# hsp-iit/online-detection

Measured on AMD Instinct MI355X. Metric: FALKON fit+infer samples/sec (N=1e6 D=1024 M=1e4), higher is better.
Workload: dtype f32-accurate K_nM (X Z' as a two-term f16 split on the f16 MFMA, f32 accumulate) stored as 24-bit fixed point (step 2^-24) + f64 solver (preconditioner: K_MM, T and T^-1 in f64; the products of the A factor, which only preconditions, at f32 accuracy on the f16 MFMA)

## Files before the change

include/odx.h:

```cpp
#ifndef ODX_H
#define ODX_H
#include <stdint.h>
#ifdef __cplusplus
extern "C" {
#endif

#define ODX_OK 0
#define ODX_ERR_INVALID (-1)
#define ODX_ERR_HIP (-2)
#define ODX_ERR_UNSUPPORTED (-3)
#define ODX_ERR_WORKSPACE (-4)

typedef void* odx_stream_t;

const char* odx_last_error_string(void);
int odx_version(void);
int odx_device_cus(void);
int odx_set_option(const char* name, int value);
int odx_get_option(const char* name, int* value);
int odx_option_default(const char* name, int* value);
int odx_release_helper_streams(void);
int odx_set_helper_streams(odx_stream_t s0, odx_stream_t s1);
int odx_stream_create_cu_mask(const uint32_t* mask, int words, odx_stream_t* stream);
int odx_stream_destroy(odx_stream_t stream);
// ... 63 lines not shown
int64_t odx_knm_bytes(int64_t n, int64_t M, int fmt);
int odx_gauss_knm_h2_store(const void* PX, int64_t ldpx, const float* metax, const float* xsq, int64_t n,
                           const void* PZ, int64_t ldpz, const float* metaz, const float* zsq, int64_t M, int D,
                           double sigma, int fmt, void* K, int64_t ldk, void* Klo, int64_t ldlo, const double* w,
                           double* ktw, void* workspace, int64_t workspace_bytes, odx_stream_t stream);
int64_t odx_knm_fwd_bwd_q_workspace_bytes(int64_t n, int64_t M, int fmt);
int odx_knm_fwd_bwd_q(const void* K, int64_t ldk, const void* Klo, int64_t ldlo, int fmt, int64_t n, int64_t M,
                      const double* v, const double* w, double* out, void* workspace, int64_t workspace_bytes,
                      odx_stream_t stream);
int64_t odx_knm_fwd_bwd2_q_workspace_bytes(int64_t n, int64_t M, int fmt);
int odx_knm_fwd_bwd2_q(const void* K, int64_t ldk, const void* Klo, int64_t ldlo, int fmt, int64_t n, int64_t M,
                       const double* v, const double* v2, double* out, double* out2, void* workspace,
                       int64_t workspace_bytes, odx_stream_t stream);
int odx_knm_fwd_bwd_q_t(const void* K, int64_t ldk, const void* Klo, int64_t ldlo, int fmt, int64_t n, int64_t M,
                        const double* v, const double* w, double* out, double* t_out, void* workspace,
                        int64_t workspace_bytes, odx_stream_t stream);
int odx_knm_fwd_bwd2_q_t(const void* K, int64_t ldk, const void* Klo, int64_t ldlo, int fmt, int64_t n, int64_t M,
                         const double* v, const double* v2, double* out, double* out2, double* t_out, void* workspace,
                         int64_t workspace_bytes, odx_stream_t stream);
int odx_knm_fwd_bwd_q_cols_t(const void* K, int64_t ldk, const void* Klo, int64_t ldlo, int fmt, int64_t n, int64_t M,
                             const double* v, const double* w, double* out, double* t_out, void* workspace,
                             int64_t workspace_bytes, int64_t Mv, const int32_t* col_of, const int32_t* start,
                             const int32_t* pos, odx_stream_t stream);
int odx_knm_fwd_bwd2_q_cols_t(const void* K, int64_t ldk, const void* Klo, int64_t ldlo, int fmt, int64_t n, int64_t M,
                              const double* v, const double* v2, double* out, double* out2, double* t_out, void* workspace,
                              int64_t workspace_bytes, int64_t Mv, const int32_t* col_of, const int32_t* start,
                              const int32_t* pos, odx_stream_t stream);
int odx_cols_fold_f64(const double* v, int64_t Mv, const int32_t* start, const int32_t* pos, int64_t M, double* out,
                      odx_stream_t stream);
int odx_cols_expand_f64(const double* x, int64_t M, const int32_t* col_of, int64_t Mv, double* out, odx_stream_t stream);
int64_t odx_knm_fwd_bwdn_q_workspace_bytes(int64_t n, int64_t M, int fmt, int nv);
int odx_knm_fwd_bwdn_q(const void* K, int64_t ldk, const void* Klo, int64_t ldlo, int fmt, int64_t n, int64_t M, int nv,
                       const double* V, int64_t ldv, double* out, int64_t ldo, void* workspace, int64_t workspace_bytes,
                       odx_stream_t stream);
int64_t odx_knm_bwdn_q_workspace_bytes(int64_t n, int64_t M, int fmt, int nv);
int odx_knm_bwdn_q(const void* K, int64_t ldk, const void* Klo, int64_t ldlo, int fmt, int64_t n, int64_t M, int nv,
                   const double* W, int64_t ldw, double* out, int64_t ldo, void* workspace, int64_t workspace_bytes,
                   odx_stream_t stream);
int64_t odx_knm_fwdn_q_workspace_bytes(int64_t n, int64_t M, int fmt, int nv);
int odx_knm_fwdn_q(const void* K, int64_t ldk, const void* Klo, int64_t ldlo, int fmt, int64_t n, int64_t M, int nv,
                   const double* V, int64_t ldv, double* T, int64_t ldt, void* workspace, int64_t workspace_bytes,
                   odx_stream_t stream);
int odx_knm_mv(const void* K, int64_t ldk, const void* Klo, int64_t ldlo, int fmt, int64_t n, int64_t M, const double* alpha,
               float* out, int64_t ldo, odx_stream_t stream);
int64_t odx_gauss_ktk_stream_h2_rows(int64_t M, int D);
int64_t odx_gauss_ktk_stream_h2_workspace_bytes(int64_t n, int64_t M, int D);
int odx_gauss_ktk_stream_h2(const void* PX, int64_t ldpx, const float* metax, const float* xsq, int64_t n,
                            const void* PZ, int64_t ldpz, const float* metaz, const float* zsq, int64_t M, int D,
                            double sigma, const double* v, const double* v2, const double* w, double* out, double* out2,
                            void* workspace, int64_t workspace_bytes, odx_stream_t stream);
#define ODX_STREAM_MAX_VECTORS 16
int64_t odx_gauss_ktk_stream_h2n_rows(int64_t M, int D);
int64_t odx_gauss_ktk_stream_h2n_workspace_bytes(int64_t n, int64_t M, int D, int nv);
int odx_gauss_ktk_stream_h2n(const void* PX, int64_t ldpx, const float* metax, const float* xsq, int64_t n,
                             const void* PZ, int64_t ldpz, const float* metaz, const float* zsq, int64_t M, int D,
                             double sigma, int nv, const double* V, int64_t ldv, double* out, int64_t ldo,
                             void* workspace, int64_t workspace_bytes, odx_stream_t stream);

int odx_split_f8(const float* X, int64_t ldx, int64_t n, int D, void* P8, int64_t ldp8, float* meta, float* qsq,
                 odx_stream_t stream);
int odx_gauss_knm_f8_store(const void* PX, int64_t ldpx8, const float* metax, const float* xsq, int64_t n,
                           const void* PZ, int64_t ldpz8, const float* metaz, const float* zsq, int64_t M, int D,
                           double sigma, int fmt, void* K, int64_t ldk, void* Klo, int64_t ldlo, const double* w,
                           double* ktw, void* workspace, int64_t workspace_bytes, odx_stream_t stream);
int odx_gauss_mmv_f8(const void* PX, int64_t ldpx8, const float* metax, const float* xsq, int64_t n,
                     const void* PZ, int64_t ldpz8, const float* metaz, const float* zsq, int64_t max_range, int D,
                     double sigma, const double* V, int64_t ldv, const int32_t* ranges, int T,
                     float* out, int64_t ldo, void* workspace, int64_t workspace_bytes, odx_stream_t stream);

int64_t odx_falkon_precond_workspace_bytes(int64_t M, int D);
int odx_falkon_precond_f64(const float* Z, int64_t ldz, int64_t M, int D, double sigma,
                           double lam, double eps, double* LTi, double* LTit, double* LAi,
                           double* LAit, int64_t ld, int32_t* info,
                           void* workspace, int64_t workspace_bytes, odx_stream_t stream);
int64_t odx_falkon_precond_path_workspace_bytes(int64_t M, int D, int L);
int odx_falkon_precond_path_f64(const float* Z, int64_t ldz, int64_t M, int D, double sigma, const double* lams, int L,
                                double eps, double* LTi, double* LTit, double* LA, int64_t ld, int32_t* info,
                                void* workspace, int64_t workspace_bytes, odx_stream_t stream);
int64_t odx_falkon_precond_batched_workspace_bytes(int64_t Mmax, int D, int B);
int odx_falkon_precond_batched_f64(const float* const* Z, const int64_t* ldz, const int64_t* M, int B,
                                   int64_t Mmax, int D, double sigma, double lam, double eps,
                                   double* out, int64_t ld, int64_t out_stride, int32_t* info,
                                   void* workspace, int64_t workspace_bytes, odx_stream_t stream);

int odx_trmv_f64(const double* Tri, int64_t ld, int64_t M, int uplo, const double* x,
                 double alpha, double beta, const double* z, double* y, odx_stream_t stream);

int odx_trmvn_f64(const double* Tri, int64_t ld, int64_t M, int uplo, int nv, const double* X, int64_t ldx,
                  double alpha, double beta, const double* Z, int64_t ldz, double* Y, int64_t ldy, odx_stream_t stream);

int odx_cg_init(const double* B, double* X, double* R, double* P, double* state, int64_t M,
                odx_stream_t stream);
int odx_cg_step(double* X, double* R, const double* P, const double* AP, double* state,
                double cg_eps, int full_grad, int64_t M, odx_stream_t stream);
int odx_cg_finish(const double* R, double* P, double* state, double cg_eps, double tol,
                  int64_t M, odx_stream_t stream);
int odx_cg_residual(const double* B, const double* AX, const double* AP, const double* state,
                    double* R, int64_t M, odx_stream_t stream);
int odx_cg_scores_axpy_f64(const double* state, const double* t, double* S, int64_t n, odx_stream_t stream);
int odx_cg_scores_store_f32(const double* S, int64_t n, float* out, int64_t ldo, odx_stream_t stream);
int odx_axpby_f64(double a, const double* x, double b, double* y, int64_t M, odx_stream_t stream);

int64_t odx_falkon_cg_workspace_bytes(int64_t n, int64_t M);
int odx_falkon_cg_f64(const float* K, int64_t ldk, int64_t n, int64_t M, const double* LTi, const double* LTit,
                      const double* LAi, const double* LAit, int64_t ldp, const double* b0, double n_total,
                      double lam, int maxiter, int full_gradient_every, double cg_epsilon, double cg_tolerance,
                      double* alpha, void* workspace, int64_t workspace_bytes, odx_stream_t stream);
int64_t odx_falkon_cg_batched_workspace_bytes(int B, const int64_t* n, const int64_t* M);
int odx_falkon_cg_batched_f64(int B, const float* const* K, const int64_t* ldk, const int64_t* n, const int64_t* M,
                              const double* P, int64_t ldp, int64_t p_rows, int64_t p_stride,
                              const double* b0, int64_t vstride, const double* n_total, double lam,
                              int maxiter, int full_gradient_every, double cg_epsilon, double cg_tolerance,
                              double* alpha, void* workspace, int64_t workspace_bytes, odx_stream_t stream);
int64_t odx_falkon_cg_batched_q_workspace_bytes(int B, const int64_t* n, const int64_t* M, int fmt);
int odx_falkon_cg_batched_q_f64(int B, const void* const* Khi, const int64_t* ldk, const void* const* Klo, const int64_t* ldlo,
                                int fmt, const int64_t* n, const int64_t* M, const double* P, int64_t ldp, int64_t p_rows,
                                int64_t p_stride, const double* b0, int64_t vstride, const double* n_total, double lam,
                                int maxiter, int full_gradient_every, double cg_epsilon, double cg_tolerance, double* alpha,
                                void* workspace, int64_t workspace_bytes, odx_stream_t stream);

#define ODX_GEMM_LOWER_ONLY 1
#define ODX_GEMM_A_UPPER 2
#define ODX_GEMM_B_UPPER 4
#define ODX_GEMM_A_LOWER 8
#define ODX_GEMM_B_LOWER 16
#define ODX_GEMM_STORE_T 32
int odx_gemm_nt_f64(const double* A, int64_t lda, const double* B, int64_t ldb, double* C,
                    int64_t ldc, int64_t m, int64_t n, int64_t k, double alpha, double beta,
                    int flags, odx_stream_t stream);
int odx_gemm_nt_f32(const float* A, int64_t lda, const float* B, int64_t ldb, float* C,
                    int64_t ldc, int64_t m, int64_t n, int64_t k, float alpha, float beta,
                    int flags, odx_stream_t stream);
int64_t odx_potrf_workspace_bytes(int64_t M);
int odx_potrf_f64(double* A, int64_t lda, int64_t M, int32_t* info, void* workspace,
                  int64_t workspace_bytes, odx_stream_t stream);
int64_t odx_trtri_workspace_bytes(int64_t M);
int odx_trtri_f64(const double* L, int64_t ldl, int64_t M, double* Li, double* Lit, int64_t ld,
                  void* workspace, int64_t workspace_bytes, odx_stream_t stream);
int odx_convert_f32_f64(const float* src, int64_t lds, double* dst, int64_t ldd, int64_t rows,
                        int64_t cols, odx_stream_t stream);
int odx_convert_f64_f32(const double* src, int64_t lds, float* dst, int64_t ldd, int64_t rows,
                        int64_t cols, odx_stream_t stream);

int64_t odx_rls_gram_workspace_bytes(int64_t nc, int D);
int odx_rls_gram_f64(const float* X, int64_t ldx, int D, const int64_t* idx, int64_t nc,
                     const double* Yt, int64_t ldy, double* G, int64_t ldg, double* XtY,
                     int64_t ldxy, void* workspace, int64_t workspace_bytes, odx_stream_t stream);
int64_t odx_rls_solve_workspace_bytes(int D);
int odx_rls_solve_f64(double* G, int64_t ldg, int D, double lam, const double* XtY, int64_t ldxy,
                      double* W, int64_t ldw, int32_t* info, void* workspace,
                      int64_t workspace_bytes, odx_stream_t stream);

int odx_rls_predict_rows_f64(const float* X, int64_t ldx, int D, const int64_t* idx, int64_t nc,
                             const double* W, int64_t ldw, double* P, int64_t ldp, odx_stream_t stream);
int odx_rls_predict_rows_batched_f64(const float* X, int64_t ldx, int D, const int64_t* idx, const int64_t* seg_start, int C,
                                     int64_t total, const double* W, int64_t ldw, int64_t w_stride, double* P, int64_t ldp,
                                     odx_stream_t stream);

int64_t odx_rls_gram_batched_workspace_bytes(int64_t npad, int D);
int odx_rls_rows_form(const float* X, int64_t ldx, int D);
int odx_rls_xty_batched_f64(const float* X, int64_t ldx, int D, const int64_t* idx_pad, int64_t npad,
                            const int64_t* seg_off, const int64_t* seg_len, int C, const double* Yt, int64_t ldy,
                            double* G, int64_t ldg, int64_t g_stride, double* XtY, int64_t ldxy, int64_t xy_stride,
                            void* workspace, int64_t workspace_bytes, odx_stream_t stream);
int odx_rls_gram_batched_f64(const float* X, int64_t ldx, int D, const int64_t* idx_pad, int64_t npad,
                             const int64_t* seg_off, const int64_t* seg_len, int C,
                             const double* Yt, int64_t ldy, double* G, int64_t ldg, int64_t g_stride,
                             double* XtY, int64_t ldxy, int64_t xy_stride,
                             void* workspace, int64_t workspace_bytes, odx_stream_t stream);
int odx_rls_pad_index(const int64_t* run, int64_t total, const int64_t* seg_off, const int64_t* seg_len, int C, int64_t npad,
                      int64_t* idx_pad, int64_t* gid, int64_t* pos, int64_t* dest, int64_t* lens, odx_stream_t stream);
int odx_rls_gram_raw_batched_f64(const float* X, int64_t ldx, int D, const int64_t* idx_pad, int64_t npad,
                                 const int64_t* seg_off, const int64_t* seg_len, int C, const float* Yraw, int64_t ldyr,
                                 double* G, int64_t ldg, int64_t g_stride, double* O5, int64_t ldo, odx_stream_t stream);
int odx_rls_fold_whitened_f64(const double* O5, int64_t ldo, int D, int C, const double* stats, const double* cnt,
                              double* G, int64_t ldg, int64_t g_stride, double* XtY, int64_t ldxy, int64_t xy_stride,
                              odx_stream_t stream);
int64_t odx_rls_solve_batched_workspace_bytes(int D, int C);
int odx_rls_solve_batched_f64(double* G, int64_t ldg, int64_t g_stride, int D, int C, double lam,
                              const double* XtY, int64_t ldxy, int64_t xy_stride,
                              double* W, int64_t ldw, int64_t w_stride, int32_t* info,
                              void* workspace, int64_t workspace_bytes, odx_stream_t stream);

int odx_roi_align_fwd_f32(const float* feat, int N, int C, int H, int W, const float* rois, int R,
                          float spatial_scale, int PH, int PW, int sampling_ratio, float* out,
                          odx_stream_t stream);
int odx_split_f16_taps3x3(const float* Y, int64_t ldy, int64_t R, int H, int W, int C, void* P, int64_t ldp,
                          float* meta, odx_stream_t stream);
int odx_gemm_h2_f32(const void* PA, int64_t ldpa, const float* metaa, int64_t m, const void* PB, int64_t ldpb,
                    const float* metab, int64_t n, int K, const float* bias, const float* residual, int64_t ldr,
                    int relu, float* out, int64_t ldo, odx_stream_t stream);
int odx_gemm_h2_max_f32(const void* PA, int64_t ldpa, const float* metaa, int64_t m, const void* PB, int64_t ldpb,
                        const float* metab, int64_t n, int K, const float* bias, const float* residual, int64_t ldr,
                        int relu, float* out, int64_t ldo, float* out_meta, odx_stream_t stream);
int odx_split_f16_taps3x3_premax(const float* Y, int64_t ldy, int64_t R, int H, int W, int C, void* P, int64_t ldp,
                                 float* meta, odx_stream_t stream);
int odx_gemm_h2_taps_supported(int64_t m, int64_t n, int C, int64_t ldpy);
int odx_gemm_h2_taps_f32(const void* PY, int64_t ldpy, const float* metay, int64_t R, int H, int W, int C,
                         const void* PB, int64_t ldpb, const float* metab, int64_t n, const float* bias,
                         const float* residual, int64_t ldr, int relu, float* out, int64_t ldo, float* out_meta,
                         void* out_packed, int64_t ldop, float bound_w, float bound_add, const float* residual_meta,
                         odx_stream_t stream);
int odx_upsample_add_rows_f32(float* lat, int64_t ldl, const float* top, int64_t ldt, int B, int H, int W, int Hp, int Wp, int C,
                              float* meta, odx_stream_t stream);
int odx_upsample_add_rows_16(void* lat, int64_t ldl, const void* top, int64_t ldt, int is_bf16, int B, int H, int W, int Hp, int Wp,
                             int C, odx_stream_t stream);
int odx_gemm_h2_chain_f32(const void* PA, int64_t ldpa, const float* metaa, int64_t m, const void* PB, int64_t ldpb,
                          const float* metab, int64_t n, int K, const float* bias, const float* residual, int64_t ldr,
                          int relu, float* out, int64_t ldo, float* out_meta, void* out_packed, int64_t ldop,
                          float bound_w, float bound_add, const float* residual_meta, odx_stream_t stream);
int odx_taps3x3_packed(const void* PY, int64_t ldpy, int64_t R, int H, int W, int C, void* P, int64_t ldp,
                       odx_stream_t stream);
int odx_gemm_b16(const void* A, int64_t lda, int64_t m, const void* B, int64_t ldb, int64_t n, int K, int is_bf16,
                 const float* bias, const void* residual, int64_t ldr, int relu, void* out, int64_t ldo, int out_16,
                 odx_stream_t stream);
int odx_taps3x3_16(const void* Y, int64_t ldy, int64_t R, int H, int W, int C, void* P, int64_t ldp, odx_stream_t stream);
int odx_debug_gemm_h2_mf32(const void* PA, int64_t ldpa, const float* metaa, int64_t m, const void* PB, int64_t ldpb,
                           const float* metab, int64_t n, int K, float* out, int64_t ldo, odx_stream_t stream);
int odx_gemm_b16_taps_supported(int64_t m, int64_t n, int C, int64_t ldy);
int odx_gemm_b16_taps(const void* Y, int64_t ldy, int64_t R, int H, int W, int C, const void* B, int64_t ldb, int64_t n,
                      int is_bf16, const float* bias, const void* residual, int64_t ldr, int relu, void* out, int64_t ldo,
// ... 59 lines not shown
```

online-detection_amd/csrc/api.cpp:

```cpp
#include "odx_common.h"
#include <string.h>

namespace odx {
static thread_local char g_error[512] = "";

void set_error(const char* fmt, ...) {
  va_list ap;
  va_start(ap, fmt);
  vsnprintf(g_error, sizeof(g_error), fmt, ap);
  va_end(ap);
}
}

extern "C" const char* odx_last_error_string(void) { return odx::g_error; }

#include "odx_internal.h"
namespace odx {
struct OptSpec {
  const char* name;
  int def, lo, hi;
};
static const OptSpec g_opt_spec[OPT_COUNT] = {
    {"h2_tile", 0, 0, 256}, {"precond", 0, 0, 2}, {"chain_helpers", -1, -1, 1}, {"rls_force_nt_gram", 0, 0, 1},
    {"rls_force_inverse_solve", 0, 0, 1}};
static int g_opt[OPT_COUNT] = {0, 0, -1, 0, 0};
int lib_option(int which) { return g_opt[which]; }
static int opt_index(const char* name) {
  if (name)
    for (int i = 0; i < OPT_COUNT; ++i)
      if (strcmp(name, g_opt_spec[i].name) == 0) return i;
  return -1;
}
}

extern "C" int odx_set_option(const char* name, int value) {
  const int i = odx::opt_index(name);
  ODX_REQUIRE(i >= 0, "odx_set_option: unknown option '%s'", name ? name : "(null)");
  const odx::OptSpec& sp = odx::g_opt_spec[i];
  ODX_REQUIRE(value >= sp.lo && value <= sp.hi && (i != odx::OPT_H2_TILE || value == 0 || value == 128 || value == 256),
              "odx_set_option: %s = %d out of range", name, value);
  odx::g_opt[i] = value;
  return ODX_OK;
}

extern "C" int odx_get_option(const char* name, int* value) {
  const int i = odx::opt_index(name);
  ODX_REQUIRE(i >= 0 && value, "odx_get_option: unknown option '%s'", name ? name : "(null)");
  *value = odx::g_opt[i];
  return ODX_OK;
}

extern "C" int odx_option_default(const char* name, int* value) {
  const int i = odx::opt_index(name);
  ODX_REQUIRE(i >= 0 && value, "odx_option_default: unknown option '%s'", name ? name : "(null)");
  *value = odx::g_opt_spec[i].def;
  return ODX_OK;
}

extern "C" int odx_version(void) { return 100; }

extern "C" int odx_device_cus(void) {
  int dev = 0;
  if (hipGetDevice(&dev) != hipSuccess) {
    odx::set_error("odx_device_cus: no HIP device");
    return ODX_ERR_HIP;
  }
  int cus = 0;
  if (hipDeviceGetAttribute(&cus, hipDeviceAttributeMultiprocessorCount, dev) != hipSuccess) {
    odx::set_error("odx_device_cus: attribute query failed");
    return ODX_ERR_HIP;
  }
  return cus;
}

extern "C" int odx_stream_create_cu_mask(const uint32_t* mask, int words, odx_stream_t* stream) {
  ODX_REQUIRE(mask && words > 0 && stream, "odx_stream_create_cu_mask: bad argument");
  hipStream_t s = nullptr;
  ODX_CHECK_HIP(hipExtStreamCreateWithCUMask(&s, (uint32_t)words, mask));
  *stream = reinterpret_cast<odx_stream_t>(s);
  return ODX_OK;
}

extern "C" int odx_stream_destroy(odx_stream_t stream) {
  if (stream) ODX_CHECK_HIP(hipStreamDestroy(reinterpret_cast<hipStream_t>(stream)));
  return ODX_OK;
}

namespace odx {
__global__ __launch_bounds__(64) void placement_kernel(int32_t* __restrict__ out, int32_t* __restrict__ counter, int spin) {
  if (threadIdx.x == 0) {
    const unsigned xcc = __builtin_amdgcn_s_getreg((3 << 11) | 20);
    const unsigned hw = __builtin_amdgcn_s_getreg((31 << 11) | 4);
    out[3 * blockIdx.x] = (int32_t)xcc;
    out[3 * blockIdx.x + 1] = (int32_t)hw;
    out[3 * blockIdx.x + 2] = atomicAdd(counter, 1);
    const long long t0 = wall_clock64();
    while (wall_clock64() - t0 < spin) __builtin_amdgcn_s_sleep(8);
  }
}
}

extern "C" int odx_debug_placement(int32_t* out, int blocks, int spin, odx_stream_t stream) {
  ODX_REQUIRE(out && blocks > 0 && spin >= 0, "odx_debug_placement: bad argument");
  hipStream_t s = reinterpret_cast<hipStream_t>(stream);
  ODX_CHECK_HIP(hipMemsetAsync(out, 0, (size_t)(3 * blocks + 1) * sizeof(int32_t), s));
  hipLaunchKernelGGL(odx::placement_kernel, dim3((unsigned)blocks), dim3(64), 0, s, out, out + 3 * blocks, spin);
  ODX_CHECK_LAUNCH("odx_debug_placement");
  return ODX_OK;
// ... 2 lines not shown
```

online-detection_amd/csrc/dense_f64.hip:

```cpp
#include "odx_internal.h"
#include <vector>

namespace odx {

typedef double f64x2 __attribute__((ext_vector_type(2)));
typedef double f64x4v __attribute__((ext_vector_type(4)));

constexpr int DB_NB = POTRF_NB;
constexpr int DB_LD = DB_NB + 1;
constexpr int DB_XLD = 33;
constexpr int DB_NT = 512;
constexpr int DB_PQ = 3072 / DB_NT;

__device__ __forceinline__ double readlane_f64(double v, int src) {
  const long long b = __double_as_longlong(v);
  const unsigned lo = (unsigned)__builtin_amdgcn_readlane((int)(b & 0xffffffffll), src);
  const unsigned hi = (unsigned)__builtin_amdgcn_readlane((int)(b >> 32), src);
  return __longlong_as_double((long long)(((unsigned long long)hi << 32) | lo));
}

__device__ __forceinline__ void chol32_wave(double* s, double* rd, int J, int jb, int32_t* info, int info_base,
                                            int lane) {
  const int l = lane & 31;
  double row[32];
// ... 298 lines not shown
    }
    __builtin_amdgcn_wave_barrier();
#pragma unroll
    for (int q = 0; q < 4; ++q) {
      const int r = wave * 16 + (lane >> 4) + 4 * q;
      T[r * TS_TLD + 32 * J + bc] = y0[q];
      T[r * TS_TLD + 32 * J + 16 + bc] = y1[q];
    }
    __builtin_amdgcn_s_waitcnt(0xC07F);
    __builtin_amdgcn_wave_barrier();
  }
  __syncthreads();
#pragma unroll
  for (int q = 0; q < 16; ++q) {
    const int e = tid + 256 * q, r = e >> 6, c = (e & 63) * 2;
    if (r < rows) *reinterpret_cast<f64x2*>(A21 + (r0 + r) * lda + c) = *reinterpret_cast<const f64x2*>(&T[r * TS_TLD + c]);
  }
}
constexpr int TS_LDS_BYTES = (TS_R * TS_TLD + 10 * 32 * TS_BLD) * (int)sizeof(double);

__global__ __launch_bounds__(256) void transpose_f64_kernel(const double* __restrict__ src, int64_t lds_,
                                                            double* __restrict__ dst, int64_t ldd, int64_t rows,
                                                            int64_t cols, int64_t zstride_src, int64_t zstride_dst) {
  __shared__ double tile[32][33];
  src += (int64_t)blockIdx.z * zstride_src;
  dst += (int64_t)blockIdx.z * zstride_dst;
  const int tx = threadIdx.x & 31, ty = threadIdx.x >> 5;
  const int64_t r0 = (int64_t)blockIdx.y * 32, c0 = (int64_t)blockIdx.x * 32;
#pragma unroll
  for (int q = 0; q < 4; ++q) {
    const int64_t r = r0 + ty + q * 8, c = c0 + tx;
    tile[ty + q * 8][tx] = (r < rows && c < cols) ? src[r * lds_ + c] : 0.0;
  }
  __syncthreads();
#pragma unroll
  for (int q = 0; q < 4; ++q) {
    const int64_t r = c0 + ty + q * 8, c = r0 + tx;
    if (r < cols && c < rows) dst[r * ldd + c] = tile[tx][ty + q * 8];
  }
}

__global__ __launch_bounds__(256) void add_diag_f64_kernel(double* A, int64_t lda, int64_t M, double value,
                                                           int64_t zstride) {
  A += (int64_t)blockIdx.y * zstride;
  const int64_t i = (int64_t)blockIdx.x * 256 + threadIdx.x;
  if (i < M) A[i * lda + i] += value;
}

__global__ __launch_bounds__(256) void fill_f64_kernel(double* A, int64_t lda, int64_t rows, int64_t cols,
                                                       double value) {
  const int64_t c = (int64_t)blockIdx.x * 256 + threadIdx.x;
  const int64_t r = blockIdx.y;
  if (c < cols && r < rows) A[r * lda + c] = value;
}

template <typename S, typename Dt>
__global__ __launch_bounds__(256) void convert_kernel(const S* __restrict__ src, int64_t lds_, Dt* __restrict__ dst,
                                                      int64_t ldd, int64_t rows, int64_t cols) {
  const int64_t c = (int64_t)blockIdx.x * 256 + threadIdx.x;
  const int64_t r = blockIdx.y;
  if (c < cols && r < rows) dst[r * ldd + c] = (Dt)src[r * lds_ + c];
}

__global__ __launch_bounds__(256) void place_diag_inverses_kernel(const double* __restrict__ Dinv, int nb,
                                                                  int64_t M, double* __restrict__ Li,
                                                                  double* __restrict__ Lit, int64_t ld,
                                                                  int64_t zstrideD, int64_t zstrideO) {
  Dinv += (int64_t)blockIdx.z * zstrideD;
  Li += (int64_t)blockIdx.z * zstrideO;
  Lit += (int64_t)blockIdx.z * zstrideO;
  const int b = blockIdx.y;
  const int64_t r0 = (int64_t)b * nb;
  const double* D = Dinv + (int64_t)b * nb * nb;
  for (int e = blockIdx.x * 256 + threadIdx.x; e < nb * nb; e += gridDim.x * 256) {
    const int i = e / nb, j = e % nb;
    if (r0 + i < M && r0 + j < M && j <= i) {
      const double v = D[e];
      Li[(r0 + i) * ld + r0 + j] = v;
      Lit[(r0 + j) * ld + r0 + i] = v;
    }
  }
}

__device__ __forceinline__ void trmv_row(const double* __restrict__ Tri, int64_t ld, int64_t M, int uplo,
                                         const double* __restrict__ x, double alpha, double beta,
                                         const double* __restrict__ z, double* __restrict__ y) {
  const int lane = threadIdx.x & 63;
  int64_t i = (int64_t)blockIdx.x * 4 + (threadIdx.x >> 6);
  if (i >= M) return;
  if (!uplo) i = M - 1 - i;
  const int64_t jlo = uplo ? i : 0, jhi = uplo ? M : i + 1;
  const double* row = Tri + i * ld;
  const int64_t q0 = (jlo + 1) >> 1, q1 = jhi >> 1;
  double s0 = 0.0, s1 = 0.0, s2 = 0.0, s3 = 0.0;
  if (lane == 0) {
    if (jlo & 1) s0 = row[jlo] * x[jlo];
    if (jhi & 1) s1 = row[jhi - 1] * x[jhi - 1];
  }
  int64_t p = q0 + lane;
  for (; p + 192 < q1; p += 256) {
    const f64x2 a0 = *reinterpret_cast<const f64x2*>(row + 2 * p), a1 = *reinterpret_cast<const f64x2*>(row + 2 * (p + 64));
    const f64x2 a2 = *reinterpret_cast<const f64x2*>(row + 2 * (p + 128)), a3 = *reinterpret_cast<const f64x2*>(row + 2 * (p + 192));
    const f64x2 b0 = *reinterpret_cast<const f64x2*>(x + 2 * p), b1 = *reinterpret_cast<const f64x2*>(x + 2 * (p + 64));
    const f64x2 b2 = *reinterpret_cast<const f64x2*>(x + 2 * (p + 128)), b3 = *reinterpret_cast<const f64x2*>(x + 2 * (p + 192));
    s0 = fma(a0[1], b0[1], fma(a0[0], b0[0], s0));
    s1 = fma(a1[1], b1[1], fma(a1[0], b1[0], s1));
    s2 = fma(a2[1], b2[1], fma(a2[0], b2[0], s2));
    s3 = fma(a3[1], b3[1], fma(a3[0], b3[0], s3));
  }
  for (; p < q1; p += 64) {
    const f64x2 a = *reinterpret_cast<const f64x2*>(row + 2 * p);
    const f64x2 b = *reinterpret_cast<const f64x2*>(x + 2 * p);
    s0 = fma(a[1], b[1], fma(a[0], b[0], s0));
  }
  double s = (s0 + s1) + (s2 + s3);
#pragma unroll
  for (int off = 32; off > 0; off >>= 1) s += __shfl_xor(s, off);
  if (lane == 0) {
    double r = alpha * s;
    if (beta != 0.0) r += beta * z[i];
    y[i] = r;
  }
}

__global__ __launch_bounds__(256) void trmv_f64_kernel(const double* __restrict__ Tri, int64_t ld, int64_t M,
                                                       int uplo, const double* __restrict__ x, double alpha,
                                                       double beta, const double* __restrict__ z,
                                                       double* __restrict__ y) {
  trmv_row(Tri, ld, M, uplo, x, alpha, beta, z, y);
}

template <int NV>
__global__ __launch_bounds__(256) void trmvn_f64_kernel(const double* __restrict__ Tri, int64_t ld, int64_t M, int uplo, int nv,
                                                        const double* __restrict__ X, int64_t ldx, double alpha, double beta,
                                                        const double* Z, int64_t ldz, double* Y, int64_t ldy) {
  constexpr int RB = 4, N = RB * NV;
  static_assert((N & (N - 1)) == 0 && N <= 64, "the transposing reduction needs a power-of-two count of sums");
  const int lane = threadIdx.x & 63;
  const int64_t nrb = (M + RB - 1) / RB;
  int64_t rb = (int64_t)blockIdx.x * 4 + (threadIdx.x >> 6);
  if (rb >= nrb) return;
  if (!uplo) rb = nrb - 1 - rb;
  const int64_t i0 = rb * RB, i1 = i0 + RB < M ? i0 + RB : M;
  const int64_t q0 = uplo ? i1 >> 1 : 0, q1 = uplo ? M >> 1 : (i0 + 1) >> 1;
  const double* row[RB];
  const double* xq[NV];
#pragma unroll
  for (int k = 0; k < RB; ++k) row[k] = Tri + (i0 + k < M ? i0 + k : M - 1) * ld;
#pragma unroll
  for (int q = 0; q < NV; ++q) xq[q] = X + (int64_t)(q < nv ? q : nv - 1) * ldx;
  double acc[RB][NV];
#pragma unroll
  for (int k = 0; k < RB; ++k)
#pragma unroll
    for (int q = 0; q < NV; ++q) acc[k][q] = 0.0;
  if (lane < 16) {
    const int64_t j = lane < 8 ? 2 * q1 + lane : 2 * q0 - 1 - (lane - 8);
#pragma unroll
    for (int k = 0; k < RB; ++k) {
      const int64_t i = i0 + k;
      const int64_t jlo = uplo ? i : 0, jhi = uplo ? M : i + 1;
      if (i < M && j >= jlo && j < jhi) {
        const double a = row[k][j];
#pragma unroll
        for (int q = 0; q < NV; ++q) acc[k][q] = a * xq[q][j];
      }
    }
  }
  for (int64_t p = q0 + lane; p < q1; p += 64) {
    f64x2 a[RB];
#pragma unroll
    for (int k = 0; k < RB; ++k) a[k] = *reinterpret_cast<const f64x2*>(row[k] + 2 * p);
#pragma unroll
    for (int q = 0; q < NV; ++q) {
      const f64x2 b = *reinterpret_cast<const f64x2*>(xq[q] + 2 * p);
#pragma unroll
      for (int k = 0; k < RB; ++k) acc[k][q] = fma(a[k][1], b[1], fma(a[k][0], b[0], acc[k][q]));
    }
  }
  double* s = &acc[0][0];
  int off = 32;
#pragma unroll
  for (int half = N / 2; half >= 1; half >>= 1, off >>= 1) {
    const bool up = (lane & off) != 0;
#pragma unroll
    for (int i = 0; i < half; ++i) {
      const double give = up ? s[i] : s[half + i], keep = up ? s[half + i] : s[i];
      s[i] = keep + __shfl_xor(give, off);
    }
  }
#pragma unroll
  for (; off > 0; off >>= 1) s[0] += __shfl_xor(s[0], off);
  int idx = 0, bit = 32;
#pragma unroll
  for (int half = N / 2; half >= 1; half >>= 1, bit >>= 1) idx += (lane & bit) ? half : 0;
  if ((lane & (64 / N - 1)) == 0 || N == 64) {
    const int k = idx / NV, q = idx % NV;
    const int64_t i = i0 + k;
    if (i < M && q < nv) {
      double r = alpha * s[0];
      if (beta != 0.0) r += beta * Z[(int64_t)q * ldz + i];
      Y[(int64_t)q * ldy + i] = r;
    }
  }
}

__global__ __launch_bounds__(256) void trmv_batched_kernel(const double* __restrict__ Tri, int64_t ld, int64_t tri_stride,
                                                           int uplo, VecBatch vb, const double* __restrict__ x,
                                                           int64_t xstride, int scaled, double beta,
                                                           const double* __restrict__ z, int64_t zstride,
                                                           double* __restrict__ y, int64_t ystride) {
  const int b = blockIdx.y;
// ... 177 lines not shown
      double* D = Dinv + (k0 / NB) * NB * NB;
      hipLaunchKernelGGL((potrf_diag_kernel<NB, false>), dim3((unsigned)Z), dim3(DB_NT), 0, stream, A + k0 * lda + k0, lda,
                         jb, D, info, (int)k0, zb.strideA, zb.strideD);
      ODX_CHECK_LAUNCH("potrf_diag");
      const int64_t m = M - k0 - jb;
      if (m <= 0) break;
      double* A21 = A + (k0 + jb) * lda + k0;
      hipLaunchKernelGGL(trsm128_kernel, dim3((unsigned)ceil_div(m, TS_R), (unsigned)Z), dim3(256), TS_LDS_BYTES, stream,
                         A21, lda, m, A + k0 * lda + k0, D + NB * NB - 4096, zb.strideA, zb.strideD);
      ODX_CHECK_LAUNCH("trsm128");
      const int64_t pc = (K0 + kbo) - (k0 + jb);
      if (pc > 0) {
        GemmParams<double> u;
        u.A = A21; u.lda = lda; u.B = A21; u.ldb = lda; u.C = A + (k0 + jb) * lda + (k0 + jb); u.ldc = lda;
        u.m = m; u.n = pc; u.k = jb; u.alpha = -1.0; u.beta = 1.0; u.flags = ODX_GEMM_LOWER_ONLY;
        zgemm(u);
        ODX_PROPAGATE(launch_gemm_f64(u, stream));
      }
    }
    const int64_t mt = M - K0 - kbo;
    if (mt > 0) {
      double* P = A + (K0 + kbo) * lda + K0;
      const int64_t nw = mt < POTRF_NBO ? mt : POTRF_NBO;
      if (pending) {
        ODX_CHECK_HIP(hipStreamWaitEvent(stream, look->join, 0));
        pending = false;
      }
      const int64_t mr = mt - nw;
      double minus1[ODX_MAX_ZBATCH];
      for (int z = 0; z < Z; ++z) minus1[z] = -1.0;
      uint32_t* Pk = pk ? pk + ((K0 / POTRF_NBO) & 1) * pk_buf : nullptr;
      if (Pk) {
        ODX_PROPAGATE(split_f64(P, lda, zb.strideA, mt, kbo, pk_scale, Pk, POTRF_NBO, pk_z, Z, stream));
        ODX_PROPAGATE(gemm_h2_f64(Pk, POTRF_NBO, pk_z, pk_scale, Pk, POTRF_NBO, pk_z, pk_scale, A + (K0 + kbo) * (lda + 1), lda,
                                  zb.strideA, mt, nw, kbo, minus1, 1.0, ODX_GEMM_LOWER_ONLY, Z, stream));
      } else {
        GemmParams<double> u;
        u.A = P; u.lda = lda; u.B = P; u.ldb = lda; u.C = A + (K0 + kbo) * (lda + 1); u.ldc = lda;
        u.m = mt; u.n = nw; u.k = kbo; u.alpha = -1.0; u.beta = 1.0; u.flags = ODX_GEMM_LOWER_ONLY;
        zgemm(u);
        ODX_PROPAGATE(launch_gemm_f64(u, stream));
      }
      if (mr > 0) {
        ODX_CHECK_HIP(hipEventRecord(look->fork, stream));
        ODX_CHECK_HIP(hipStreamWaitEvent(look->stream, look->fork, 0));
        if (Pk) {
          ODX_PROPAGATE(gemm_h2_f64(Pk + nw * POTRF_NBO, POTRF_NBO, pk_z, pk_scale, Pk + nw * POTRF_NBO, POTRF_NBO, pk_z, pk_scale,
                                    A + (K0 + kbo + nw) * (lda + 1), lda, zb.strideA, mr, mr, kbo, minus1, 1.0, ODX_GEMM_LOWER_ONLY, Z,
                                    look->stream));
        } else {
          double* P2 = P + nw * lda;
          GemmParams<double> r;
          r.A = P2; r.lda = lda; r.B = P2; r.ldb = lda; r.C = A + (K0 + kbo + nw) * (lda + 1); r.ldc = lda;
          r.m = mr; r.n = mr; r.k = kbo; r.alpha = -1.0; r.beta = 1.0; r.flags = ODX_GEMM_LOWER_ONLY;
          zgemm(r);
          ODX_PROPAGATE(launch_gemm_f64(r, look->stream));
        }
        ODX_CHECK_HIP(hipEventRecord(look->join, look->stream));
        pending = true;
      }
    }
  }
  if (pending) ODX_CHECK_HIP(hipStreamWaitEvent(stream, look->join, 0));
  hipLaunchKernelGGL(trtri_diag_kernel, dim3((unsigned)ceil_div(M, NB), (unsigned)Z), dim3(DB_NT), 0, stream, A, lda, M,
                     Dinv, zb.strideA, zb.strideD);
  ODX_CHECK_LAUNCH("trtri_diag");
  return ODX_OK;
}

int trmv_batched_f64(const double* Tri, int64_t ld, int64_t tri_stride, int uplo, const VecBatch& vb, const double* x,
                     int64_t xstride, bool scaled, double beta, const double* z, int64_t zstride, double* y,
                     int64_t ystride, hipStream_t stream) {
  int mm = 0;
  for (int b = 0; b < vb.B; ++b) mm = vb.M[b] > mm ? vb.M[b] : mm;
  if (mm <= 0) return ODX_OK;
  hipLaunchKernelGGL(trmv_batched_kernel, dim3((unsigned)ceil_div(mm, 4), (unsigned)vb.B), dim3(256), 0, stream, Tri, ld,
                     tri_stride, uplo, vb, x, xstride, scaled ? 1 : 0, beta, z, zstride, y, ystride);
  ODX_CHECK_LAUNCH("trmv_batched_f64");
  return ODX_OK;
}

int trtri_from_diag_f64(const double* L, int64_t ldl, int64_t M, const double* Dinv, double* Li, double* Lit,
                        int64_t ld, double* WT, hipStream_t stream, const ZBatch& zb, uint32_t* pk, int64_t pk_cap, int64_t pk_z,
                        double bound_l, double bound_inv) {
  constexpr int NB = POTRF_NB;
  ODX_REQUIRE(ld % 2 == 0 && ldl % 2 == 0, "trtri_f64: leading dimensions must be even");
  const int Z = zb.count;
  ODX_REQUIRE(Z >= 1 && Z <= ODX_MAX_ZBATCH && zb.strideA % 2 == 0 && zb.strideO % 2 == 0 && zb.strideW % 2 == 0,
              "trtri_f64: class batch of 1..%d matrices, even strides", ODX_MAX_ZBATCH);
  const int nblk = (int)ceil_div(M, NB);
  hipLaunchKernelGGL(place_diag_inverses_kernel, dim3(16, (unsigned)nblk, (unsigned)Z), dim3(256), 0, stream, Dinv, NB, M,
                     Li, Lit, ld, zb.strideD, zb.strideO);
  ODX_CHECK_LAUNCH("place_diag_inverses");
  for (int64_t s = NB; s < M; s *= 2) {
    const int nb = (int)ceil_div(M, 2 * s);
    const int nbe = (int)ceil_div(M - s, 2 * s);
    const int64_t m2l = M - s - (int64_t)(nbe - 1) * 2 * s;
    const int64_t szr = (int64_t)(nbe - 1) * s * s + (m2l < s ? m2l : s) * s;
    if (pk != nullptr && s >= 512 && 2 * szr + 2 * (int64_t)nbe * s * s <= pk_cap) {
      const float sl = split_scale_for(bound_l), si = split_scale_for(bound_inv), sw = split_scale_for(bound_l * bound_inv);
      uint32_t *pL21 = pk, *pX11 = pL21 + szr, *pX22 = pX11 + (int64_t)nbe * s * s, *pWT = pX22 + szr;
      double one[ODX_MAX_ZBATCH], mone[ODX_MAX_ZBATCH];
      for (int z = 0; z < Z; ++z) { one[z] = 1.0; mone[z] = -1.0; }
      SplitBlocksArgs k1;
      k1.X = L + s * ldl; k1.ldx = ldl; k1.bsx = 2 * s * (ldl + 1); k1.zsx = zb.strideA;
      k1.P = pL21; k1.ldp = s; k1.bsp = s * s; k1.zsp = pk_z; k1.rows = s; k1.cols = s;
      k1.rg_total = M; k1.rg_off = s; k1.rg_step = 2 * s; k1.rows_ragged = 1; k1.nb = nbe; k1.Z = Z; k1.scale = sl;
      ODX_PROPAGATE(split_f64_blocks(k1, stream));
      SplitBlocksArgs k2;
      k2.X = Lit; k2.ldx = ld; k2.bsx = 2 * s * (ld + 1); k2.zsx = zb.strideO;
      k2.P = pX11; k2.ldp = s; k2.bsp = s * s; k2.zsp = pk_z; k2.rows = s; k2.cols = s; k2.nb = nbe; k2.Z = Z; k2.scale = si;
      ODX_PROPAGATE(split_f64_blocks(k2, stream));
      H2F64Args a1;
      a1.PA = pL21; a1.ldpa = s; a1.zsa = pk_z; a1.bsa = s * s; a1.sa = sl;
      a1.PB = pX11; a1.ldpb = s; a1.zsb = pk_z; a1.bsb = s * s; a1.sb = si;
      a1.C = WT; a1.ldc = s; a1.zsc = zb.strideW; a1.bsc = s * s;
      a1.m = s; a1.n = s; a1.k = s; a1.rg_total = M; a1.rg_off = s; a1.rg_step = 2 * s;
      a1.flags = ODX_GEMM_B_UPPER | ODX_GEMM_STORE_T; a1.zcount = Z; a1.nb = nbe; a1.beta = 0.0;
      for (int z = 0; z < Z; ++z) a1.alpha[z] = one[z];
      ODX_PROPAGATE(gemm_h2_f64_ex(a1, stream));
      SplitBlocksArgs k3;
      k3.X = Li + s * (ld + 1); k3.ldx = ld; k3.bsx = 2 * s * (ld + 1); k3.zsx = zb.strideO;
      k3.P = pX22; k3.ldp = s; k3.bsp = s * s; k3.zsp = pk_z; k3.rows = s; k3.cols = s;
      k3.rg_total = M; k3.rg_off = s; k3.rg_step = 2 * s; k3.rows_ragged = 1; k3.cols_ragged = 1; k3.nb = nbe; k3.Z = Z; k3.scale = si;
      ODX_PROPAGATE(split_f64_blocks(k3, stream));
      SplitBlocksArgs k4;
      k4.X = WT; k4.ldx = s; k4.bsx = s * s; k4.zsx = zb.strideW;
      k4.P = pWT; k4.ldp = s; k4.bsp = s * s; k4.zsp = pk_z; k4.rows = s; k4.cols = s;
      k4.rg_total = M; k4.rg_off = s; k4.rg_step = 2 * s; k4.cols_ragged = 1; k4.nb = nbe; k4.Z = Z; k4.scale = sw;
      ODX_PROPAGATE(split_f64_blocks(k4, stream));
      H2F64Args a2;
      a2.PA = pX22; a2.ldpa = s; a2.zsa = pk_z; a2.bsa = s * s; a2.sa = si;
      a2.PB = pWT; a2.ldpb = s; a2.zsb = pk_z; a2.bsb = s * s; a2.sb = sw;
      a2.C = Li + s * ld; a2.ldc = ld; a2.zsc = zb.strideO; a2.bsc = 2 * s * (ld + 1);
      a2.C2 = Lit + s; a2.ldc2 = ld; a2.zsc2 = zb.strideO; a2.bsc2 = 2 * s * (ld + 1);
      a2.m = s; a2.n = s; a2.k = s; a2.rg_total = M; a2.rg_off = s; a2.rg_step = 2 * s; a2.k_is_m = 1;
      a2.flags = ODX_GEMM_A_LOWER; a2.zcount = Z; a2.nb = nbe; a2.beta = 0.0;
      for (int z = 0; z < Z; ++z) a2.alpha[z] = mone[z];
      ODX_PROPAGATE(gemm_h2_f64_ex(a2, stream));
      continue;
    }
    GemmParams<double> g1;
    g1.A = L + s * ldl; g1.lda = ldl;
    g1.B = Lit; g1.ldb = ld;
    g1.C = WT; g1.ldc = s;
    g1.m = s; g1.n = s; g1.k = s; g1.alpha = 1.0; g1.beta = 0.0;
    g1.flags = ODX_GEMM_B_UPPER | ODX_GEMM_STORE_T;
    g1.batches = nb;
    g1.strideA = 2 * s * (ldl + 1); g1.strideB = 2 * s * (ld + 1); g1.strideC = s * s;
    g1.ragged_total = M; g1.ragged_off = s; g1.ragged_step = 2 * s;
    g1.zbatches = Z; g1.zstrideA = zb.strideA; g1.zstrideB = zb.strideO; g1.zstrideC = zb.strideW;
    ODX_PROPAGATE(launch_gemm_f64(g1, stream));
    GemmParams<double> g2;
    g2.A = Li + s * (ld + 1); g2.lda = ld;
    g2.B = WT; g2.ldb = s;
    g2.C = Li + s * ld; g2.ldc = ld;
    g2.C2 = Lit + s; g2.ldc2 = ld;
    g2.m = s; g2.n = s; g2.k = s; g2.alpha = -1.0; g2.beta = 0.0;
    g2.flags = ODX_GEMM_A_LOWER;
    g2.batches = nb;
    g2.strideA = 2 * s * (ld + 1); g2.strideB = s * s; g2.strideC = 2 * s * (ld + 1); g2.strideC2 = 2 * s * (ld + 1);
    g2.ragged_total = M; g2.ragged_off = s; g2.ragged_step = 2 * s; g2.ragged_k_is_m = 1;
    g2.zbatches = Z; g2.zstrideA = zb.strideO; g2.zstrideB = zb.strideW; g2.zstrideC = zb.strideO; g2.zstrideC2 = zb.strideO;
    ODX_PROPAGATE(launch_gemm_f64(g2, stream));
  }
  return ODX_OK;
}

}

using namespace odx;

extern "C" int odx_trmv_f64(const double* Tri, int64_t ld, int64_t M, int uplo, const double* x, double alpha,
                            double beta, const double* z, double* y, odx_stream_t stream) {
  if (M <= 0) return ODX_OK;
  ODX_REQUIRE(Tri && x && y && (beta == 0.0 || z), "odx_trmv_f64: null pointer");
  ODX_REQUIRE(ld % 2 == 0 && ld >= M && aligned16(Tri) && aligned16(x), "odx_trmv_f64: Tri/x must be 16-byte aligned, ld even, ld >= M");
  ODX_REQUIRE(x != y, "odx_trmv_f64: x and y must not alias");
  hipLaunchKernelGGL(trmv_f64_kernel, dim3((unsigned)ceil_div(M, 4)), dim3(256), 0, as_stream(stream), Tri, ld, M,
                     uplo, x, alpha, beta, z, y);
  ODX_CHECK_LAUNCH("odx_trmv_f64");
  return ODX_OK;
}

extern "C" int odx_trmvn_f64(const double* Tri, int64_t ld, int64_t M, int uplo, int nv, const double* X, int64_t ldx, double alpha,
                             double beta, const double* Z, int64_t ldz, double* Y, int64_t ldy, odx_stream_t stream) {
  ODX_REQUIRE(nv >= 1 && nv <= 8, "odx_trmvn_f64: 1 .. 8 vectors per call (got %d)", nv);
  if (M <= 0) return ODX_OK;
  ODX_REQUIRE(Tri && X && Y && (beta == 0.0 || Z), "odx_trmvn_f64: null pointer");
  ODX_REQUIRE(ld % 2 == 0 && ld >= M && aligned16(Tri) && aligned16(X) && ldx % 2 == 0,
              "odx_trmvn_f64: Tri/X must be 16-byte aligned, ld and ldx even, ld >= M");
  ODX_REQUIRE(nv == 1 || (ldx >= M && ldy >= M && (beta == 0.0 || ldz >= M)), "odx_trmvn_f64: rows of X, Z and Y must be M apart or more");
  ODX_REQUIRE(X != Y, "odx_trmvn_f64: X and Y must not alias");
  const dim3 grid((unsigned)ceil_div(ceil_div(M, (int64_t)4), (int64_t)4));
#define ODX_TRMVN(NV_)                                                                                                            \
  hipLaunchKernelGGL(trmvn_f64_kernel<NV_>, grid, dim3(256), 0, as_stream(stream), Tri, ld, M, uplo, nv, X, ldx, alpha, beta, Z, ldz, \
                     Y, ldy)
  if (nv <= 2) ODX_TRMVN(2);
  else if (nv <= 4) ODX_TRMVN(4);
  else ODX_TRMVN(8);
#undef ODX_TRMVN
  ODX_CHECK_LAUNCH("odx_trmvn_f64");
  return ODX_OK;
}

extern "C" int odx_convert_f32_f64(const float* src, int64_t lds_, double* dst, int64_t ldd, int64_t rows,
                                   int64_t cols, odx_stream_t stream) {
  if (rows <= 0 || cols <= 0) return ODX_OK;
  ODX_REQUIRE(src && dst, "odx_convert_f32_f64: null pointer");
  for (int64_t r0 = 0; r0 < rows; r0 += 65535) {
    const int64_t nr = rows - r0 < 65535 ? rows - r0 : 65535;
    hipLaunchKernelGGL((convert_kernel<float, double>), dim3((unsigned)ceil_div(cols, 256), (unsigned)nr), dim3(256),
                       0, as_stream(stream), src + r0 * lds_, lds_, dst + r0 * ldd, ldd, nr, cols);
  }
  ODX_CHECK_LAUNCH("odx_convert_f32_f64");
  return ODX_OK;
}

extern "C" int odx_convert_f64_f32(const double* src, int64_t lds_, float* dst, int64_t ldd, int64_t rows,
                                   int64_t cols, odx_stream_t stream) {
  if (rows <= 0 || cols <= 0) return ODX_OK;
  ODX_REQUIRE(src && dst, "odx_convert_f64_f32: null pointer");
  for (int64_t r0 = 0; r0 < rows; r0 += 65535) {
    const int64_t nr = rows - r0 < 65535 ? rows - r0 : 65535;
    hipLaunchKernelGGL((convert_kernel<double, float>), dim3((unsigned)ceil_div(cols, 256), (unsigned)nr), dim3(256),
                       0, as_stream(stream), src + r0 * lds_, lds_, dst + r0 * ldd, ldd, nr, cols);
  }
  ODX_CHECK_LAUNCH("odx_convert_f64_f32");
  return ODX_OK;
}

extern "C" int64_t odx_potrf_workspace_bytes(int64_t M) {
  if (M <= 0) return 0;
  return ceil_div(M, POTRF_NB) * POTRF_NB * POTRF_NB * (int64_t)sizeof(double);
}

extern "C" int odx_potrf_f64(double* A, int64_t lda, int64_t M, int32_t* info, void* workspace,
                             int64_t workspace_bytes, odx_stream_t stream) {
  if (M <= 0) return ODX_OK;
  ODX_REQUIRE(A && info && workspace, "odx_potrf_f64: null pointer");
  if (workspace_bytes < odx_potrf_workspace_bytes(M)) {
    set_error("odx_potrf_f64: workspace too small");
    return ODX_ERR_WORKSPACE;
  }
  ODX_CHECK_HIP(hipMemsetAsync(info, 0, sizeof(int32_t), as_stream(stream)));
  const int rc = potrf_f64(A, lda, M, static_cast<double*>(workspace), info, as_stream(stream));
  return rc;
}

extern "C" int64_t odx_trtri_workspace_bytes(int64_t M) {
  if (M <= 0) return 0;
  return odx_potrf_workspace_bytes(M) + M * M * (int64_t)sizeof(double);
}

extern "C" int odx_trtri_f64(const double* L, int64_t ldl, int64_t M, double* Li, double* Lit, int64_t ld,
                             void* workspace, int64_t workspace_bytes, odx_stream_t stream) {
  if (M <= 0) return ODX_OK;
  ODX_REQUIRE(L && Li && Lit && workspace, "odx_trtri_f64: null pointer");
  ODX_REQUIRE(ld >= M && ldl >= M && aligned16(L) && aligned16(Li) && aligned16(Lit), "odx_trtri_f64: bad ld / alignment");
  if (workspace_bytes < odx_trtri_workspace_bytes(M)) {
    set_error("odx_trtri_f64: workspace too small");
    return ODX_ERR_WORKSPACE;
  }
  hipStream_t s = as_stream(stream);
  double* Dinv = static_cast<double*>(workspace);
  double* WT = Dinv + ceil_div(M, POTRF_NB) * POTRF_NB * POTRF_NB;
  hipLaunchKernelGGL(trtri_diag_kernel, dim3((unsigned)ceil_div(M, POTRF_NB)), dim3(DB_NT), 0, s, L, ldl, M, Dinv,
                     (int64_t)0, (int64_t)0);
  ODX_CHECK_LAUNCH("trtri_diag");
  ODX_PROPAGATE(fill_f64(Li, ld, M, M, 0.0, s));
  ODX_PROPAGATE(fill_f64(Lit, ld, M, M, 0.0, s));
  return trtri_from_diag_f64(L, ldl, M, Dinv, Li, Lit, ld, WT, s);
}

static int64_t precond_ld(int64_t M) { return round_up(M, 2); }
static int64_t precond_ldz(int D) { const int64_t l = round_up(D, 2); return l % 128 == 0 ? l + 64 : l; }

extern "C" int64_t odx_falkon_precond_workspace_bytes(int64_t M, int D) {
  if (M <= 0 || D <= 0) return 0;
  const int64_t ld = precond_ld(M), ldzd = precond_ldz(D);
  int64_t dbl = M * ldzd + round_up(M, 2) + 4 * M * ld + 2 * ceil_div(M, POTRF_NB) * POTRF_NB * POTRF_NB + precond_split_doubles(M);
  return dbl * (int64_t)sizeof(double);
}

static int falkon_precond_f64_impl(const float* Z, int64_t ldz, int64_t M, int D, double sigma, const double* lams, int L,
                                   double eps, double* LTi, double* LTit, double* const* LAi, double* const* LAit, int64_t ld,
                                   int32_t* info, void* workspace, int64_t workspace_bytes, odx_stream_t stream);

extern "C" int odx_falkon_precond_f64(const float* Z, int64_t ldz, int64_t M, int D, double sigma, double lam,
                                      double eps, double* LTi, double* LTit, double* LAi, double* LAit, int64_t ld,
                                      int32_t* info, void* workspace, int64_t workspace_bytes, odx_stream_t stream) {
  ODX_REQUIRE(LAi && LAit, "odx_falkon_precond_f64: null pointer");
  const int rc = falkon_precond_f64_impl(Z, ldz, M, D, sigma, &lam, 1, eps, LTi, LTit, &LAi, &LAit, ld, info, workspace, workspace_bytes, stream);
  return rc;
}

extern "C" int64_t odx_falkon_precond_path_workspace_bytes(int64_t M, int D, int L) {
  if (M <= 0 || D <= 0 || L <= 0) return 0;
  return round_up(odx_falkon_precond_workspace_bytes(M, D), 16) + (L > 1 ? M * precond_ld(M) * (int64_t)sizeof(double) : 0);
}

extern "C" int odx_falkon_precond_path_f64(const float* Z, int64_t ldz, int64_t M, int D, double sigma, const double* lams, int L,
                                           double eps, double* LTi, double* LTit, double* LA, int64_t ld, int32_t* info,
                                           void* workspace, int64_t workspace_bytes, odx_stream_t stream) {
  ODX_REQUIRE(lams && LA && L >= 1 && L <= ODX_MAX_ZBATCH, "odx_falkon_precond_path_f64: 1 <= L <= %d lambdas, non-null lams / LA",
              ODX_MAX_ZBATCH);
  ODX_REQUIRE(M > 0 && ld >= M, "odx_falkon_precond_path_f64: bad sizes");
  double* lai[ODX_MAX_ZBATCH];
  double* lait[ODX_MAX_ZBATCH];
  for (int l = 0; l < L; ++l) {
    lai[l] = LA + (int64_t)(2 * l) * M * ld;
    lait[l] = lai[l] + M * ld;
  }
  return falkon_precond_f64_impl(Z, ldz, M, D, sigma, lams, L, eps, LTi, LTit, lai, lait, ld, info, workspace, workspace_bytes, stream);
}

static int falkon_precond_f64_impl(const float* Z, int64_t ldz, int64_t M, int D, double sigma, const double* lams, int L,
                                   double eps, double* LTi, double* LTit, double* const* LAi, double* const* LAit, int64_t ld,
                                   int32_t* info, void* workspace, int64_t workspace_bytes, odx_stream_t stream) {
  ODX_REQUIRE(M > 0 && D > 0 && sigma > 0, "odx_falkon_precond_f64: bad sizes");
  ODX_REQUIRE(Z && LTi && LTit && info && workspace, "odx_falkon_precond_f64: null pointer");
  ODX_REQUIRE(ld % 2 == 0 && ld >= M && aligned16(LTi) && aligned16(LTit), "odx_falkon_precond_f64: outputs must be 16-byte aligned with even ld >= M");
  for (int l = 0; l < L; ++l)
    ODX_REQUIRE(LAi[l] && LAit[l] && aligned16(LAi[l]) && aligned16(LAit[l]),
                "odx_falkon_precond_f64: outputs must be 16-byte aligned with even ld >= M");
  ODX_REQUIRE(aligned16(workspace), "odx_falkon_precond_f64: workspace must be 16-byte aligned");
  if (workspace_bytes < odx_falkon_precond_path_workspace_bytes(M, D, L)) {
    set_error("odx_falkon_precond_f64: workspace too small");
    return ODX_ERR_WORKSPACE;
  }
  hipStream_t s = as_stream(stream);
  SideStream* side = nullptr;
  ODX_PROPAGATE(side_stream(&side, 0, s, M));
  hipStream_t s2 = side->stream;
  const int64_t wld = precond_ld(M), ldzd = precond_ldz(D);
  const int64_t dsz = ceil_div(M, POTRF_NB) * POTRF_NB * POTRF_NB;
  double* Zd = static_cast<double*>(workspace);
  double* zsq = Zd + M * ldzd;
  double* W0 = zsq + round_up(M, 2);
  double* W1 = W0 + M * wld;
  double* W2 = W1 + M * wld;
  double* W3 = W2 + M * wld;
  double* DinvT = W3 + M * wld;
  double* DinvA = DinvT + dsz;
  const bool split = precond_split(M);
  const int64_t ldpt = h2_f64_packed_ld(M);
  uint32_t* Tk = reinterpret_cast<uint32_t*>(DinvA + dsz);
  uint32_t* Pk = Tk + precond_pack_units(M);
  double* WA = L > 1 ? static_cast<double*>(workspace) + round_up(odx_falkon_precond_workspace_bytes(M, D), 16) / (int64_t)sizeof(double) : W2;

  ODX_CHECK_HIP(hipMemsetAsync(info, 0, (size_t)L * sizeof(int32_t), s));
  ODX_CHECK_HIP(hipMemsetAsync(Zd, 0, (size_t)(M * ldzd) * sizeof(double), s));
  ODX_PROPAGATE(odx_convert_f32_f64(Z, ldz, Zd, ldzd, M, D, stream));
  ODX_CHECK_HIP(hipMemsetAsync(W0, 0, (size_t)(M * wld) * sizeof(double), s));
  ODX_PROPAGATE(gauss_kmm_f64(Zd, ldzd, M, D, sigma, eps * (double)M, W0, wld, zsq, s));
  ODX_PROPAGATE(potrf_f64(W0, wld, M, DinvT, info, s));
  for (int l = 1; l < L; ++l)
    ODX_CHECK_HIP(hipMemcpyAsync(info + l, info, sizeof(int32_t), hipMemcpyDeviceToDevice, s));
  ODX_CHECK_HIP(hipEventRecord(side->fork, s));
  ODX_CHECK_HIP(hipStreamWaitEvent(s2, side->fork, 0));
  ODX_PROPAGATE(fill_f64(LTi, ld, M, M, 0.0, s2));
  ODX_PROPAGATE(fill_f64(LTit, ld, M, M, 0.0, s2));
  ODX_PROPAGATE(trtri_from_diag_f64(W0, wld, M, DinvT, LTi, LTit, ld, W3, s2));
  ODX_CHECK_HIP(hipEventRecord(side->join, s2));
  ODX_CHECK_HIP(hipMemsetAsync(W1, 0, (size_t)(M * wld) * sizeof(double), s));
  ODX_PROPAGATE(transpose_f64(W0, wld, W1, wld, M, M, s));
  ODX_CHECK_HIP(hipMemsetAsync(W2, 0, (size_t)(M * wld) * sizeof(double), s));
  if (split) {
    const float st = split_scale_for(sqrt(1.0 + eps * 65536.0));
    const double a1 = 1.0 / (double)M;
    ODX_PROPAGATE(split_f64(W1, wld, 0, M, M, st, Tk, ldpt, 0, 1, s));
    ODX_PROPAGATE(gemm_h2_f64(Tk, ldpt, 0, st, Tk, ldpt, 0, st, W2, wld, 0, M, M, M, &a1, 0.0,
                              ODX_GEMM_LOWER_ONLY | ODX_GEMM_A_UPPER | ODX_GEMM_B_UPPER, 1, s));
  } else {
    GemmParams<double> g;
    g.A = W1; g.lda = wld; g.B = W1; g.ldb = wld; g.C = W2; g.ldc = wld;
    g.m = M; g.n = M; g.k = M; g.alpha = 1.0 / (double)M; g.beta = 0.0;
    g.flags = ODX_GEMM_LOWER_ONLY | ODX_GEMM_A_UPPER | ODX_GEMM_B_UPPER;
    ODX_PROPAGATE(launch_gemm_f64(g, s));
  }
  for (int l = 0; l < L; ++l) {
    const double lam = lams[l];
    if (WA != W2) ODX_CHECK_HIP(hipMemcpyAsync(WA, W2, (size_t)(M * wld) * sizeof(double), hipMemcpyDeviceToDevice, s));
    ODX_PROPAGATE(add_diag_f64(WA, wld, M, lam, s));
    if (split) ODX_PROPAGATE(potrf_f64(WA, wld, M, DinvA, info + l, s, ZBatch(), Pk, M * POTRF_NBO, 0, split_scale_for(sqrt(1.0 + eps + lam))));
    else ODX_PROPAGATE(potrf_f64(WA, wld, M, DinvA, info + l, s));
    if (l == 0) ODX_CHECK_HIP(hipStreamWaitEvent(s, side->join, 0));
    ODX_PROPAGATE(fill_f64(LAi[l], ld, M, M, 0.0, s));
    ODX_PROPAGATE(fill_f64(LAit[l], ld, M, M, 0.0, s));
    if (split && eps + lam > 0.0)
      ODX_PROPAGATE(trtri_from_diag_f64(WA, wld, M, DinvA, LAi[l], LAit[l], ld, W1, s, ZBatch(), Tk, precond_pack_units(M), 0,
                                        sqrt(1.0 + eps + lam), 1.0 / sqrt(eps + lam)));
    else
      ODX_PROPAGATE(trtri_from_diag_f64(WA, wld, M, DinvA, LAi[l], LAit[l], ld, W1, s));
  }
  return ODX_OK;
}

extern "C" int64_t odx_falkon_precond_batched_workspace_bytes(int64_t Mmax, int D, int B) {
  if (Mmax <= 0 || D <= 0 || B <= 0) return 0;
  const int64_t ld = precond_ld(Mmax), ldzd = precond_ldz(D);
  const int64_t per = Mmax * ldzd + round_up(Mmax, 2) + 4 * Mmax * ld + 2 * ceil_div(Mmax, POTRF_NB) * POTRF_NB * POTRF_NB +
                      precond_split_doubles(Mmax);
  return per * B * (int64_t)sizeof(double);
}

static int falkon_precond_batched_f64_impl(const float* const* Z, const int64_t* ldz, const int64_t* M, int B,
                                           int64_t Mmax, int D, double sigma, double lam, double eps, double* out,
                                           int64_t ld, int64_t out_stride, int32_t* info, void* workspace,
                                           int64_t workspace_bytes, odx_stream_t stream);

extern "C" int odx_falkon_precond_batched_f64(const float* const* Z, const int64_t* ldz, const int64_t* M, int B,
                                              int64_t Mmax, int D, double sigma, double lam, double eps, double* out,
                                              int64_t ld, int64_t out_stride, int32_t* info, void* workspace,
                                              int64_t workspace_bytes, odx_stream_t stream) {
  const int rc = falkon_precond_batched_f64_impl(Z, ldz, M, B, Mmax, D, sigma, lam, eps, out, ld, out_stride, info, workspace, workspace_bytes, stream);
  return rc;
}

static int falkon_precond_batched_f64_impl(const float* const* Z, const int64_t* ldz, const int64_t* M, int B,
                                           int64_t Mmax, int D, double sigma, double lam, double eps, double* out,
                                           int64_t ld, int64_t out_stride, int32_t* info, void* workspace,
                                           int64_t workspace_bytes, odx_stream_t stream) {
  ODX_REQUIRE(B >= 1 && B <= ODX_MAX_ZBATCH, "odx_falkon_precond_batched_f64: 1 <= B <= %d classes per call", ODX_MAX_ZBATCH);
  ODX_REQUIRE(Z && ldz && M && out && info && workspace && Mmax > 0 && D > 0 && sigma > 0,
              "odx_falkon_precond_batched_f64: null pointer or bad size");
  ODX_REQUIRE(ld % 2 == 0 && ld >= Mmax && aligned16(out) && out_stride % 2 == 0 && out_stride >= 4 * Mmax * ld,
              "odx_falkon_precond_batched_f64: out must be 16-byte aligned, ld even >= Mmax, out_stride >= 4 Mmax ld");
  ODX_REQUIRE(aligned16(workspace), "odx_falkon_precond_batched_f64: workspace must be 16-byte aligned");
  for (int b = 0; b < B; ++b)
    ODX_REQUIRE(Z[b] && M[b] > 0 && M[b] <= Mmax, "odx_falkon_precond_batched_f64: class %d: need 0 < M <= Mmax", b);
  if (workspace_bytes < odx_falkon_precond_batched_workspace_bytes(Mmax, D, B)) {
    set_error("odx_falkon_precond_batched_f64: workspace too small");
    return ODX_ERR_WORKSPACE;
  }
  hipStream_t s = as_stream(stream);
  SideStream* side = nullptr;
  ODX_PROPAGATE(side_stream(&side, 0, s, Mmax));
  hipStream_t s2 = side->stream;
  const int64_t wld = precond_ld(Mmax), ldzd = precond_ldz(D);
  const int64_t dsz = ceil_div(Mmax, POTRF_NB) * POTRF_NB * POTRF_NB;
  const int64_t zper = Mmax * ldzd + round_up(Mmax, 2), wsz = Mmax * wld;
  double* Zd0 = static_cast<double*>(workspace);
  double* W0 = Zd0 + (int64_t)B * zper;
  double* W1 = W0 + (int64_t)B * wsz;
  double* W2 = W1 + (int64_t)B * wsz;
  double* W3 = W2 + (int64_t)B * wsz;
  double* DinvT = W3 + (int64_t)B * wsz;
  double* DinvA = DinvT + (int64_t)B * dsz;
  double* LTi = out, *LTit = out + Mmax * ld, *LAi = out + 2 * Mmax * ld, *LAit = out + 3 * Mmax * ld;
  const bool split = precond_split(Mmax);
  const int64_t ldpt = h2_f64_packed_ld(Mmax);
  uint32_t* Tk = reinterpret_cast<uint32_t*>(DinvA + (int64_t)B * dsz);
  uint32_t* Pk = Tk + (int64_t)B * precond_pack_units(Mmax);

  ODX_CHECK_HIP(hipMemsetAsync(info, 0, (size_t)B * sizeof(int32_t), s));
  ODX_CHECK_HIP(hipMemsetAsync(Zd0, 0, (size_t)((int64_t)B * zper) * sizeof(double), s));
  ODX_CHECK_HIP(hipMemsetAsync(W0, 0, (size_t)(3 * (int64_t)B * wsz) * sizeof(double), s));
  if (out_stride == 4 * Mmax * ld) {
    ODX_CHECK_HIP(hipMemsetAsync(out, 0, (size_t)((int64_t)B * out_stride) * sizeof(double), s));
  } else {
    for (int b = 0; b < B; ++b)
      ODX_CHECK_HIP(hipMemsetAsync(out + (int64_t)b * out_stride, 0, (size_t)(4 * Mmax * ld) * sizeof(double), s));
  }
  VecBatch kb;
  kb.B = B;
  for (int b = 0; b < B; ++b) {
    ODX_PROPAGATE(odx_convert_f32_f64(Z[b], ldz[b], Zd0 + (int64_t)b * zper, ldzd, M[b], D, stream));
    kb.M[b] = (int)M[b];
    kb.scale[b] = eps * (double)M[b];
  }
  ODX_PROPAGATE(gauss_kmm_f64_batched(Zd0, ldzd, zper, Mmax * ldzd, kb, D, sigma, W0, wld, wsz, s));
  for (int b = 0; b < B; ++b)
    if (M[b] < Mmax) ODX_PROPAGATE(add_diag_f64(W0 + (int64_t)b * wsz + M[b] * (wld + 1), wld, Mmax - M[b], 1.0, s));
  ZBatch zt;
  zt.count = B; zt.strideA = wsz; zt.strideD = dsz; zt.strideO = out_stride; zt.strideW = wsz;
  ODX_PROPAGATE(potrf_f64(W0, wld, Mmax, DinvT, info, s, zt));
  ODX_CHECK_HIP(hipEventRecord(side->fork, s));
  ODX_CHECK_HIP(hipStreamWaitEvent(s2, side->fork, 0));
  ODX_PROPAGATE(trtri_from_diag_f64(W0, wld, Mmax, DinvT, LTi, LTit, ld, W3, s2, zt));
  ODX_CHECK_HIP(hipEventRecord(side->join, s2));
  ODX_PROPAGATE(transpose_f64(W0, wld, W1, wld, Mmax, Mmax, s, B, wsz, wsz));
  if (split) {
    const float st = split_scale_for(sqrt(1.0 + eps * 65536.0)), sa = split_scale_for(sqrt(1.0 + eps + lam));
    double a1[ODX_MAX_ZBATCH];
    for (int b = 0; b < B; ++b) a1[b] = 1.0 / (double)M[b];
    ODX_PROPAGATE(split_f64(W1, wld, wsz, Mmax, Mmax, st, Tk, ldpt, precond_pack_units(Mmax), B, s));
    ODX_PROPAGATE(gemm_h2_f64(Tk, ldpt, precond_pack_units(Mmax), st, Tk, ldpt, precond_pack_units(Mmax), st, W2, wld, wsz, Mmax, Mmax, Mmax, a1, 0.0,
                              ODX_GEMM_LOWER_ONLY | ODX_GEMM_A_UPPER | ODX_GEMM_B_UPPER, B, s));
    ODX_PROPAGATE(add_diag_f64(W2, wld, Mmax, lam, s, B, wsz));
    ODX_PROPAGATE(potrf_f64(W2, wld, Mmax, DinvA, info, s, zt, Pk, (int64_t)B * Mmax * POTRF_NBO, Mmax * POTRF_NBO, sa));
  } else {
    GemmParams<double> g;
    g.A = W1; g.lda = wld; g.B = W1; g.ldb = wld; g.C = W2; g.ldc = wld;
    g.m = Mmax; g.n = Mmax; g.k = Mmax; g.beta = 0.0;
    g.flags = ODX_GEMM_LOWER_ONLY | ODX_GEMM_A_UPPER | ODX_GEMM_B_UPPER;
    g.zbatches = B; g.zstrideA = wsz; g.zstrideB = wsz; g.zstrideC = wsz;
    g.zalpha_on = 1;
    for (int b = 0; b < B; ++b) g.zalpha[b] = 1.0 / (double)M[b];
    ODX_PROPAGATE(launch_gemm_f64(g, s));
    ODX_PROPAGATE(add_diag_f64(W2, wld, Mmax, lam, s, B, wsz));
    ODX_PROPAGATE(potrf_f64(W2, wld, Mmax, DinvA, info, s, zt));
  }
  ODX_CHECK_HIP(hipStreamWaitEvent(s, side->join, 0));
  if (split && eps + lam > 0.0)
    return trtri_from_diag_f64(W2, wld, Mmax, DinvA, LAi, LAit, ld, W1, s, zt, Tk, precond_pack_units(Mmax), precond_pack_units(Mmax),
                               sqrt(1.0 + eps + lam), 1.0 / sqrt(eps + lam));
  return trtri_from_diag_f64(W2, wld, Mmax, DinvA, LAi, LAit, ld, W1, s, zt);
}

extern "C" int odx_set_side_stream_cu_mask(const uint32_t* mask, int words) {
  ODX_REQUIRE(words >= 0 && words <= 64 && (words == 0 || mask != nullptr), "odx_set_side_stream_cu_mask: bad argument");
  g_side_mask.assign(mask, mask + words);
  return ODX_OK;
}

extern "C" int odx_set_helper_streams(odx_stream_t s0, odx_stream_t s1) {
  g_given_helper[0] = reinterpret_cast<hipStream_t>(s0);
  g_given_helper[1] = reinterpret_cast<hipStream_t>(s1);
  return ODX_OK;
}

extern "C" int odx_release_helper_streams(void) {
  return odx::release_side_streams(false);
}
```

online-detection_amd/csrc/odx_internal.h:

```cpp
#pragma once
#include "odx_common.h"

namespace odx {
enum LibOpt {
  OPT_H2_TILE = 0,
  OPT_PRECOND,
  OPT_CHAIN_HELPERS,
  OPT_RLS_FORCE_NT_GRAM,
  OPT_RLS_FORCE_INVERSE_SOLVE,
  OPT_COUNT
};
int lib_option(int which);


constexpr int ODX_MAX_ZBATCH = 32;

template <typename T>
struct GemmParams {
  const T* A = nullptr; int64_t lda = 0;
  const T* B = nullptr; int64_t ldb = 0;
  T* C = nullptr; int64_t ldc = 0;
  T* C2 = nullptr; int64_t ldc2 = 0;
  int64_t m = 0, n = 0, k = 0;
  T alpha = T(1), beta = T(0);
  int flags = 0;
  int batches = 1;
  int64_t strideA = 0, strideB = 0, strideC = 0, strideC2 = 0;
  int64_t ragged_total = 0, ragged_off = 0, ragged_step = 0;
  int ragged_k_is_m = 0;
  int vec_epilogue = 0;
  int zbatches = 1;
  int64_t zstrideA = 0, zstrideB = 0, zstrideC = 0, zstrideC2 = 0;
  int zalpha_on = 0;
  T zalpha[ODX_MAX_ZBATCH] = {};
  int zk_on = 0;
  int64_t zkoff[ODX_MAX_ZBATCH] = {};
  int64_t zklen[ODX_MAX_ZBATCH] = {};
};

int launch_gemm_f64(const GemmParams<double>& p, hipStream_t stream);
int launch_gemm_f32(const GemmParams<float>& p, hipStream_t stream);

constexpr int POTRF_NB = 128;
struct ZBatch {
  int count = 1;
  int64_t strideA = 0;
  int64_t strideD = 0;
  int64_t strideO = 0;
  int64_t strideW = 0;
};
int potrf_f64(double* A, int64_t lda, int64_t M, double* Dinv , int32_t* info ,
              hipStream_t stream, const ZBatch& zb = ZBatch(), uint32_t* pk = nullptr, int64_t pk_buf = 0, int64_t pk_z = 0,
              float pk_scale = 1.f);
int trtri_from_diag_f64(const double* L, int64_t ldl, int64_t M, const double* Dinv, double* Li, double* Lit,
                        int64_t ld, double* WT, hipStream_t stream, const ZBatch& zb = ZBatch(), uint32_t* pk = nullptr,
                        int64_t pk_cap = 0, int64_t pk_z = 0, double bound_l = 1.0, double bound_inv = 1.0);
int transpose_f64(const double* src, int64_t lds, double* dst, int64_t ldd, int64_t rows, int64_t cols,
                  hipStream_t stream, int zcount = 1, int64_t zstride_src = 0, int64_t zstride_dst = 0);
int add_diag_f64(double* A, int64_t lda, int64_t M, double value, hipStream_t stream, int zcount = 1, int64_t zstride = 0);
int fill_f64(double* A, int64_t lda, int64_t rows, int64_t cols, double value, hipStream_t stream);

int slab_reduce_f64(const double* slab, int64_t slab_ld, int nslab, int64_t M, double* out, hipStream_t stream);
int slab_reduce2_f64(const double* slab, int64_t slab_ld, int nslab, int64_t M, double* out, double* out2, hipStream_t stream);

int slab_reduce_cols_f64(const double* slab, int64_t slab_ld, int nslab, int nv, int64_t M, int64_t Mv, const int* col_of, double* out,
                         double* out2, hipStream_t stream);

int slab_reduce_batched_f64(int B, const int64_t* M, const int* nslab, const double* slab, int64_t slab_ld, int64_t slab_stride,
                            double* out, int64_t ostride, hipStream_t stream);
int64_t knm_passq_batched_workspace_bytes(int B, const int64_t* n, const int64_t* M, int fmt);
int knm_passq_batched(int B, const void* const* Khi, const int64_t* ldk, const void* const* Klo, const int64_t* ldlo, int fmt,
                      const int64_t* n, const int64_t* M, const double* v, int64_t vstride, double* out, int64_t ostride,
                      void* workspace, int64_t workspace_bytes, hipStream_t stream);

int pass_cus();
int check_q_block(const char* who, const void* K, int64_t ldk, const void* Klo, int64_t ldlo, int fmt, int64_t M);

bool knm_pass_batch_cfg(int B, const int64_t* M, int* nt, int* ch, int* r);
int64_t knm_pass_batched_workspace_bytes(int B, const int64_t* n, const int64_t* M);
int knm_pass_batched(int B, const float* const* K, const int64_t* ldk, const int64_t* n, const int64_t* M, const double* v,
                     int64_t vstride, double* out, int64_t ostride, void* workspace, int64_t workspace_bytes,
                     hipStream_t stream);

struct VecBatch {
  int B = 1;
  int M[ODX_MAX_ZBATCH] = {};
  double scale[ODX_MAX_ZBATCH] = {};
};
int trmv_batched_f64(const double* Tri, int64_t ld, int64_t tri_stride, int uplo, const VecBatch& vb, const double* x,
                     int64_t xstride, bool scaled, double beta, const double* z, int64_t zstride, double* y,
                     int64_t ystride, hipStream_t stream);
int cg_init_batched(const VecBatch& vb, const double* Bv, double* X, double* R, double* P, double* state, int64_t vstride,
                    hipStream_t stream);
int cg_step_batched(const VecBatch& vb, double* X, double* R, const double* P, const double* AP, double* state,
                    double cg_eps, int full_grad, int64_t vstride, hipStream_t stream);
int cg_finish_batched(const VecBatch& vb, const double* R, double* P, double* state, double cg_eps, double tol,
                      int64_t vstride, hipStream_t stream);
int cg_full_residual_batched(const VecBatch& vb, const double* Bv, const double* AX, double* R, int64_t vstride,
                             hipStream_t stream);

int64_t h2_f64_packed_ld(int64_t cols);
int split_f64(const double* X, int64_t ldx, int64_t zsx, int64_t rows, int64_t cols, float scale, uint32_t* P, int64_t ldp,
              int64_t zsp, int z, hipStream_t stream);
struct SplitBlocksArgs {
  const double* X = nullptr; int64_t ldx = 0, bsx = 0, zsx = 0;
  uint32_t* P = nullptr; int64_t ldp = 0, bsp = 0, zsp = 0;
  int64_t rows = 0, cols = 0;
  int64_t rg_total = 0, rg_off = 0, rg_step = 0;
  int rows_ragged = 0, cols_ragged = 0, nb = 1, Z = 1;
  float scale = 1.f;
};
int split_f64_blocks(const SplitBlocksArgs& a, hipStream_t stream);
struct H2F64Args {
  const uint32_t* PA = nullptr; int64_t ldpa = 0, zsa = 0, bsa = 0; float sa = 1.f;
  const uint32_t* PB = nullptr; int64_t ldpb = 0, zsb = 0, bsb = 0; float sb = 1.f;
  double* C = nullptr; int64_t ldc = 0, zsc = 0, bsc = 0;
  double* C2 = nullptr; int64_t ldc2 = 0, zsc2 = 0, bsc2 = 0;
  int64_t m = 0, n = 0, k = 0;
  int64_t rg_total = 0, rg_off = 0, rg_step = 0;
  int k_is_m = 0, flags = 0, zcount = 1, nb = 1;
  double beta = 0.0;
  double alpha[ODX_MAX_ZBATCH] = {};
};
int gemm_h2_f64_ex(const H2F64Args& a, hipStream_t stream);
int gemm_h2_f64(const uint32_t* PA, int64_t ldpa, int64_t zsa, float sa, const uint32_t* PB, int64_t ldpb, int64_t zsb, float sb,
                double* C, int64_t ldc, int64_t zsc, int64_t m, int64_t n, int64_t k, const double* alpha, double beta, int flags,
                int zcount, hipStream_t stream);

int gauss_kmm_f64(const double* Zd, int64_t ldz, int64_t M, int D, double sigma, double diag_add, double* Kmm,
                  int64_t ldk, double* zsq , hipStream_t stream);

int gauss_kmm_f64_batched(const double* Zd, int64_t ldz, int64_t z_stride, int64_t zsq_off, const VecBatch& vb, int D,
                          double sigma, double* Kmm, int64_t ldk, int64_t k_stride, hipStream_t stream);

}
```

online-detection_amd/odx/backend.py:

```python
import ctypes
import os

import torch

from . import hip
from .knm_path import PathOps, _p


class Features:
    __slots__ = ("X", "sq", "n", "D", "ld", "P", "meta", "own_pack", "P8", "meta8", "sq8", "zero_row", "cmap")

    def __init__(self, X, sq, D, P=None, meta=None):
        self.X, self.sq, self.n, self.D, self.ld = X, sq, X.shape[0], D, X.stride(0) if X.shape[0] else X.shape[1]
        self.P, self.meta = P, meta
        self.zero_row = False
        self.own_pack = P is None
        self.P8 = self.meta8 = self.sq8 = None
        self.cmap = None


class Rows16:
    __slots__ = ("buf", "n", "K", "zero_row")

    def __init__(self, buf, K, zero_row=False):
        self.buf, self.n, self.K = buf, buf.shape[0], K
        self.zero_row = zero_row

    @property
    def dense(self):
        return self.buf[:, :self.K]


class PackedRows:
    __slots__ = ("X", "n", "D", "P", "meta", "zero_row")

    def __init__(self, X, n, D, P, meta, zero_row=False):
        self.X, self.n, self.D, self.P, self.meta, self.zero_row = X, n, D, P, meta, zero_row


class Precond:
    __slots__ = ("LTi", "LTit", "LAi", "LAit", "M", "ld", "info", "block_rows")


class Knm:
    __slots__ = ("K", "n", "M", "ld", "fmt", "lo", "cmap", "Mv")

    def __init__(self):
        self.fmt, self.lo, self.cmap, self.Mv = "f32", None, None, None

    def dense(self):
        if self.fmt == "f32":
            return self.K[:, :self.M]
        if self.fmt == "u24":
            q = ((self.K[:, :self.M].to(torch.int32) & 0xFFFF) << 8) | self.lo[:, :self.M].to(torch.int32)
            return q.to(torch.float32) * (2.0 ** -24)
        return ((self.K[:, :self.M].to(torch.int32) & 0xFFFF) << 16).view(torch.float32)

    def rows(self, lo, hi):
        sub = Knm()
        sub.n, sub.M, sub.ld, sub.fmt = hi - lo, self.M, self.ld, self.fmt
        sub.K = self.K[lo:hi]
        sub.lo = self.lo[lo:hi] if self.lo is not None else None
        sub.cmap, sub.Mv = self.cmap, self.Mv
        return sub


class KnmStream:
    __slots__ = ("F", "Zf", "sigma", "n", "M", "ring", "K", "fmt", "lo")

    def __init__(self, F, Zf, sigma, ring=None):
        self.F, self.Zf, self.sigma, self.n, self.M, self.ring = F, Zf, float(sigma), F.n, Zf.n, ring
        self.K, self.fmt, self.lo = F.P, "stream", None


class HipBackend(PathOps):
    name = "hip-gfx950"
    shared_mmv_min = 2

    def __init__(self, device=None):
        self.lib = hip.require_gpu()
        self.device = torch.device("cuda", torch.cuda.current_device()) if device is None else torch.device(device)
        self._ws = {}
        self._meta_pools = {}
        self._capture_meta_pool = None
        from . import options as _options
        opts = _options.load()
        self.gauss = opts.gauss
        self.knm_storage = opts.knm_storage
        _options.apply()
        self.helper_streams = []
        try:
            from . import streams as _streams
            own = _streams.of_default(3, self.device)
            if len(own) >= 3:
                self.helper_streams = own[1:3]
                hip.check(self.lib.odx_set_helper_streams(ctypes.c_void_p(own[1].cuda_stream), ctypes.c_void_p(own[2].cuda_stream)),
                          "odx_set_helper_streams")
        except hip.OdxError:
            raise
        except Exception:
            pass

    def _stream(self):
        return ctypes.c_void_p(torch.cuda.current_stream(self.device).cuda_stream)

    def _workspace(self, key, nbytes):
        nbytes = max(int(nbytes), 16)
        if torch.cuda.is_current_stream_capturing():
            return torch.empty(nbytes, dtype=torch.uint8, device=self.device)
        cur = torch.cuda.current_stream(self.device)
        if cur != torch.cuda.default_stream(self.device):
            key = (key, cur.cuda_stream)
        buf = self._ws.get(key)
        if buf is None or buf.numel() < nbytes:
            buf = None
            self._ws.pop(key, None)
            buf = torch.empty(nbytes, dtype=torch.uint8, device=self.device)
            self._ws[key] = buf
        return buf

    def release_workspaces(self):
        self._ws.clear()
        self.release_helper_streams()

# ... 68 lines not shown

    def _meta_slot(self):
        if torch.cuda.is_current_stream_capturing():
            pool = self._capture_meta_pool
            if pool is None or pool[1] + 2 > pool[0].numel():
                pool = self._capture_meta_pool = [torch.zeros(1024, dtype=torch.float32, device=self.device), 0]
            at = pool[1]
            pool[1] = at + 4
            return pool[0][at:at + 2]
        cur = torch.cuda.current_stream(self.device)
        key = cur.cuda_stream
        pool = self._meta_pools.get(key)
        if pool is None or pool[1] + 2 > pool[0].numel():
            pool = self._meta_pools[key] = [torch.zeros(8192, dtype=torch.float32, device=self.device), 0]
        at = pool[1]
        pool[1] = at + 4
        return pool[0][at:at + 2]

    def reset_capture_pools(self):
        self._capture_meta_pool = None

    def rows(self, F, idx):
        idx = torch.as_tensor(idx, dtype=torch.int64, device=self.device).reshape(-1)
        ld = (F.D + 3) // 4 * 4
        buf = torch.zeros((idx.numel(), ld), dtype=torch.float32, device=self.device)
        buf[:, :F.D] = F.X.index_select(0, idx)
        P = F.P.index_select(0, idx) if F.P is not None else None
        Z = Features(buf[:, :F.D], F.sq.index_select(0, idx), F.D, P, F.meta if P is not None else None)
        if F.P8 is not None:
            Z.P8, Z.meta8, Z.sq8 = F.P8.index_select(0, idx), F.meta8, F.sq8.index_select(0, idx)
        return Z

    def pack8(self, F):
        if F.P8 is None:
            ldp8 = (F.D + 127) // 128 * 128
            F.P8 = torch.empty((F.n, ldp8), dtype=torch.uint8, device=self.device)
            F.meta8 = torch.zeros(2, dtype=torch.float32, device=self.device)
            F.sq8 = torch.empty(F.n, dtype=torch.float32, device=self.device)
            hip.check(self.lib.odx_split_f8(_p(F.X), F.ld, F.n, F.D, _p(F.P8), ldp8, _p(F.meta8), _p(F.sq8), self._stream()),
                      "odx_split_f8")
        return F

    def pack(self, F, zero_row=False):
        if F.P is not None and zero_row and not F.zero_row:
            if not F.own_pack:
                raise ValueError("pack(zero_row=True): the packed rows were gathered from another matrix and have no zero row behind them")
            F.P = None
        if F.P is None:
            ldp = (F.D + 63) // 64 * 64
            if zero_row:
                buf = torch.empty((F.n + 1, ldp), dtype=torch.int32, device=self.device)
                buf[F.n].zero_()
                F.P = buf[:F.n]
                F.zero_row = True
            else:
                F.P = torch.empty((F.n, ldp), dtype=torch.int32, device=self.device)
            if F.meta is not None and F.n:
                hip.check(self.lib.odx_split_f16_premax(_p(F.X), F.ld, F.n, F.D, _p(F.P), ldp, _p(F.meta), self._stream()),
                          "odx_split_f16_premax")
            else:
                F.meta = torch.zeros(2, dtype=torch.float32, device=self.device)
                hip.check(self.lib.odx_split_f16(_p(F.X), F.ld, F.n, F.D, _p(F.P), ldp, _p(F.meta), self._stream()),
                          "odx_split_f16")
        return F

    def precond(self, Zf, sigma, lam, eps, out=None, ws_key="precond"):
        M, D = Zf.n, Zf.D
        ld = (M + 1) // 2 * 2
        P = Precond()
        P.M, P.ld = M, ld
        mats = out if out is not None else torch.empty((4, M, ld), dtype=torch.float64, device=self.device)
        P.LTi, P.LTit, P.LAi, P.LAit = mats[0], mats[1], mats[2], mats[3]
        P.block_rows = M
        P.info = torch.zeros(1, dtype=torch.int32, device=self.device)
        nbytes = self.lib.odx_falkon_precond_workspace_bytes(M, D)
        ws = self._workspace(ws_key, nbytes)
        hip.check(self.lib.odx_falkon_precond_f64(_p(Zf.X), Zf.ld, M, D, float(sigma), float(lam), float(eps),
                                                  _p(P.LTi), _p(P.LTit), _p(P.LAi), _p(P.LAit), ld, _p(P.info),
                                                  _p(ws), ws.numel(), self._stream()), "odx_falkon_precond_f64")
        return P

    MAX_CLASS_BATCH = 32

    def precond_batched(self, Zfs, sigma, lam, eps, out=None, ws_key="precond_batched", Mmax=None):
        B = len(Zfs)
        if not 1 <= B <= self.MAX_CLASS_BATCH:
            raise ValueError("precond_batched: 1..%d classes per call, got %d" % (self.MAX_CLASS_BATCH, B))
        D = Zfs[0].D
        if any(z.D != D for z in Zfs):
            raise ValueError("precond_batched: every class needs the same feature dimension")
        Ms = [int(z.n) for z in Zfs]
        if Mmax is not None and int(Mmax) < max(Ms):
            raise ValueError("precond_batched: Mmax (%d) below the largest class (%d)" % (int(Mmax), max(Ms)))
        Mmax = max(Ms) if Mmax is None else int(Mmax)
        ld = (Mmax + 1) // 2 * 2
        if out is None:
            out = torch.empty((B, 4, Mmax, ld), dtype=torch.float64, device=self.device)
        if out.dtype != torch.float64 or out.dim() != 4 or out.shape[0] < B or tuple(out.shape[1:]) != (4, Mmax, ld) or not out.is_contiguous():
            raise ValueError("precond_batched: out must be a contiguous (>= %d, 4, %d, %d) f64 tensor" % (B, Mmax, ld))
        info = torch.zeros(B, dtype=torch.int32, device=self.device)
        ws = self._workspace(ws_key, self.lib.odx_falkon_precond_batched_workspace_bytes(Mmax, D, B))
        zp = (ctypes.c_void_p * B)(*[z.X.data_ptr() for z in Zfs])
        zl = (ctypes.c_int64 * B)(*[int(z.ld) for z in Zfs])
        zm = (ctypes.c_int64 * B)(*Ms)
        hip.check(self.lib.odx_falkon_precond_batched_f64(zp, zl, zm, B, Mmax, D, float(sigma), float(lam), float(eps), _p(out), ld,
                                                          4 * Mmax * ld, _p(info), _p(ws), ws.numel(), self._stream()),
                  "odx_falkon_precond_batched_f64")
        Ps = []
        for b, M in enumerate(Ms):
            P = Precond()
            P.M, P.ld = M, ld
            P.LTi, P.LTit, P.LAi, P.LAit = (out[b, k, :M] for k in range(4))
            P.info = info[b:b + 1]
            P.block_rows = Mmax
            Ps.append(P)
        return Ps

    def check_precond(self, P):
        self.check_info(P.info)

    def check_info(self, info):
        info = int(info.item())
        if info != 0:
            raise hip.OdxError("FALKON preconditioner: non-positive pivot at index %d (Cholesky failed)" % (info - 1))

    def knm_format(self, n, M):
        if self.knm_storage == "stream":
            if self.gauss != "h2":
                raise ValueError("knm_storage 'stream' needs gauss 'h2' (the streamed pass recomputes K on the split-f16 tile core); "
                                 "gauss is %r" % (self.gauss,))
            return "stream"
        if self.gauss not in ("h2", "f8") or n <= 0 or M <= 0:
            return "f32"
        if self.knm_storage in ("u24", "bf16"):
            return self.knm_storage if self.lib.odx_knm_fwd_bwd_q_workspace_bytes(n, M, hip.KNM_CODE[self.knm_storage]) >= 0 else "f32"
        if self.knm_storage == "auto" and n * M >= (1 << 27) and M >= 1024 and (self.gauss == "f8" or self.lib.odx_gauss_h2_tile(n, M) == 256) \
                and self.lib.odx_knm_fwd_bwd_q_workspace_bytes(n, M, hip.KNM_U24) >= 0:
            return "u24"
        return "f32"

    def knm_bytes(self, n, M, D=None):
        if self.knm_format(n, M) == "stream":
            return max(0, int(self._stream_bytes(max(n, 1), M, 64 if D is None else D)))
        return int(self.lib.odx_knm_bytes(max(n, 0), M, hip.KNM_CODE[self.knm_format(n, M)]))

    def _knm_block(self, n, M, fmt, out):
        K = Knm()
        K.n, K.M, K.fmt = n, M, fmt
        K.ld = ld = int(self.lib.odx_knm_ld(M, hip.KNM_CODE[fmt]))
        per = {"f32": 4, "u24": 3, "bf16": 2}[fmt]
        need = n * ld * per
        if out is not None:
            raw = out.view(-1).view(torch.uint8)
            if raw.numel() < need or raw.data_ptr() % 16:
                raise ValueError("knm: out buffer too small (%d < %d bytes) or not 16-byte aligned" % (raw.numel(), need))
        else:
            raw = torch.empty(max(need, 16), dtype=torch.uint8, device=self.device)
        if fmt == "f32":
            K.K = raw[: n * ld * 4].view(torch.float32).view(n, ld)
        else:
            K.K = raw[: n * ld * 2].view(torch.int16).view(n, ld)
            if fmt == "u24":
                K.lo = raw[n * ld * 2: n * ld * 3].view(n, ld)
        return K

    def knm(self, F, Zf, sigma, out=None):
        n, M = F.n, Zf.n
        fmt = self.knm_format(n, M)
        if fmt == "stream":
            raise ValueError("knm: knm_storage 'stream' stores no K_nM block (knm_rhs hands out a streamed shard)")
        if fmt != "f32" or self.gauss == "f8":
            return self._knm_store(F, Zf, sigma, fmt, None, out, None)[0]
        K = self._knm_block(n, M, "f32", out)
        ld = K.ld
        if self.direct_small(n, M, F.D):
            hip.check(self.lib.odx_gauss_knm_direct_f32(_p(F.X), F.ld, n, _p(Zf.X), Zf.ld, M, F.D, float(sigma), _p(K.K), ld,
                                                        self._stream()), "odx_gauss_knm_direct_f32")
            return K
        if self.gauss == "h2":
            self.pack(F), self.pack(Zf)
            hip.check(self.lib.odx_gauss_knm_h2(_p(F.P), F.P.stride(0), _p(F.meta), _p(F.sq), n, _p(Zf.P), Zf.P.stride(0),
                                                _p(Zf.meta), _p(Zf.sq), M, F.D, float(sigma), _p(K.K), ld, self._stream()),
                      "odx_gauss_knm_h2")
        else:
            hip.check(self.lib.odx_gauss_knm_f32(_p(F.X), F.ld, _p(F.sq), n, _p(Zf.X), Zf.ld, _p(Zf.sq), M, F.D,
                                                 float(sigma), _p(K.K), ld, self._stream()), "odx_gauss_knm_f32")
        return K

    DIRECT_MAX_MACS = 1 << 24

    def direct_small(self, n, M, D):
        from . import options as _options
        return (self.gauss == "h2" and _options.current().h2_tile == 0 and n > 0 and M > 0 and self.knm_storage in ("auto", "f32")
                and int(n) * int(M) * int(D) <= self.DIRECT_MAX_MACS)

    def _knm_store(self, F, Zf, sigma, fmt, w, out, rhs_out):
        n, M = F.n, Zf.n
        K = self._knm_block(n, M, fmt, out)
        f8 = self.gauss == "f8"
        (self.pack8(F), self.pack8(Zf)) if f8 else (self.pack(F), self.pack(Zf))
        ws = None
        if w is not None:
            w = w.to(dtype=torch.float64, device=self.device).contiguous()
            if rhs_out is None:
                rhs_out = torch.empty(M, dtype=torch.float64, device=self.device)
            ws = self._workspace("knm_rhs", self.lib.odx_gauss_knm_h2_rhs_workspace_bytes(n, M))
        fn, PX, mx, PZ, mz = ((self.lib.odx_gauss_knm_f8_store, F.P8, F.meta8, Zf.P8, Zf.meta8) if f8 else
                              (self.lib.odx_gauss_knm_h2_store, F.P, F.meta, Zf.P, Zf.meta))
        sqx, sqz = (F.sq8, Zf.sq8) if f8 else (F.sq, Zf.sq)
        hip.check(fn(_p(PX), PX.stride(0), _p(mx), _p(sqx), n, _p(PZ), PZ.stride(0), _p(mz), _p(sqz), M, F.D, float(sigma),
                     hip.KNM_CODE[fmt], _p(K.K), K.ld, _p(K.lo), K.ld, _p(w), _p(rhs_out if w is not None else None), _p(ws),
                     ws.numel() if ws is not None else 0, self._stream()), "odx_gauss_knm_f8_store" if f8 else "odx_gauss_knm_h2_store")
        return K, rhs_out

    def knm_rhs(self, F, Zf, sigma, w, out=None, rhs_out=None):
        n, M = F.n, Zf.n
        if rhs_out is None:
            rhs_out = torch.empty(M, dtype=torch.float64, device=self.device)
        fmt = self.knm_format(n, M)
        if fmt == "stream":
            self.pack(F), self.pack(Zf)
            ring = None
            if out is not None:
                raw = out.view(-1).view(torch.uint8)
                if raw.numel() >= self._stream_bytes(max(n, 1), M, F.D) and raw.data_ptr() % 16 == 0:
                    ring = raw
            K = KnmStream(F, Zf, sigma, ring)
            w = None if w is None else w.to(dtype=torch.float64, device=self.device).contiguous()
            return K, self.ktk(K, w=w, out=rhs_out)
        cmap = getattr(Zf, "cmap", None)
        if cmap is not None and fmt in ("u24", "bf16") and n > 0:
            self.pack8(Zf) if self.gauss == "f8" else self.pack(Zf)
            first, col_of = cmap.on(self.device)[:2]
            K, b_d = self._knm_store(F, self.rows(Zf, first), sigma, fmt, w, out, None)
            K.cmap, K.Mv = cmap, M
            if w is not None:
                self._call("odx_cols_expand_f64", _p(b_d), K.M, _p(col_of), M, _p(rhs_out))
            return K, rhs_out
        if (fmt != "f32" or self.gauss == "f8") and n > 0:
            return self._knm_store(F, Zf, sigma, fmt, w, out, rhs_out)
        if not (self.gauss == "h2" and n > 0 and self.lib.odx_gauss_h2_tile(n, M) == 256) or self.direct_small(n, M, F.D):
            K = self.knm(F, Zf, sigma, out=out)
            return K, self.ktk(K, w=w, out=rhs_out)
        return self._knm_store(F, Zf, sigma, "f32", w, out, rhs_out)

    def pin_gauss_tile(self, tile):
        from . import options as _options
        _options.set(h2_tile=int(tile))

    def reserve_cus_during_passes(self, cus):
        hip.check(self.lib.odx_set_pass_reserved_cus(int(cus)), "odx_set_pass_reserved_cus")

    def cg_residual(self, B, AX, AP, state, R):
        hip.check(self.lib.odx_cg_residual(_p(B), _p(AX), _p(AP), _p(state), _p(R), R.numel(), self._stream()), "odx_cg_residual")

    def cg_scores_axpy(self, state, t, S):
        if S.dtype != torch.float64 or t.dtype != torch.float64 or S.numel() != t.numel() or not (S.is_contiguous() and t.is_contiguous()):
            raise ValueError("cg_scores_axpy: t and S must be contiguous f64 vectors of the same length")
        hip.check(self.lib.odx_cg_scores_axpy_f64(_p(state), _p(t), _p(S), S.numel(), self._stream()), "odx_cg_scores_axpy_f64")

    def cg_scores_store(self, S, out):
        if out.dtype != torch.float32 or out.shape[0] != S.numel() or (out.dim() == 2 and out.shape[1] != 1) or S.dtype != torch.float64:
            raise ValueError("cg_scores_store: S must be (n,) f64 and out an (n,) or (n, 1) f32 tensor")
        hip.check(self.lib.odx_cg_scores_store_f32(_p(S), S.numel(), _p(out), out.stride(0), self._stream()), "odx_cg_scores_store_f32")
        return out

    def cg_solve(self, K, P, b0, n_total, lam, maxiter, opt):
        if K.fmt != "f32":
            raise hip.OdxError("cg_solve: the one-call CG loop needs an f32-stored K_nM block, got %r" % K.fmt)
        alpha = torch.empty(K.M, dtype=torch.float64, device=self.device)
        nbytes = self.lib.odx_falkon_cg_workspace_bytes(max(K.n, 1), K.M)
        if nbytes < 0:
            raise hip.OdxError("odx_falkon_cg_f64: M = %d is outside the supported range" % K.M)
        ws = self._workspace("cg_solve", nbytes)
        hip.check(self.lib.odx_falkon_cg_f64(_p(K.K), K.ld, K.n, K.M, _p(P.LTi), _p(P.LTit), _p(P.LAi), _p(P.LAit), P.ld, _p(b0),
                                             float(n_total), float(lam), int(maxiter), int(opt.cg_full_gradient_every),
                                             float(opt.cg_epsilon), float(opt.cg_tolerance), _p(alpha), _p(ws), ws.numel(),
                                             self._stream()), "odx_falkon_cg_f64")
        return alpha

    def cg_batched_supported(self, ns, Ms, fmt="f32"):
        B = len(ns)
        if not 1 <= B <= self.MAX_CLASS_BATCH or fmt == "stream":
            return False
        n = (ctypes.c_int64 * B)(*[int(v) for v in ns])
        M = (ctypes.c_int64 * B)(*[int(v) for v in Ms])
        if fmt == "f32":
            return self.lib.odx_falkon_cg_batched_workspace_bytes(B, n, M) >= 0
        return self.lib.odx_falkon_cg_batched_q_workspace_bytes(B, n, M, hip.KNM_CODE[fmt]) >= 0

    def cg_solve_batched(self, Ks, Ps, b0s, n_totals, lam, maxiter, opt):
        B = len(Ks)
        fmt = Ks[0].fmt
        if fmt == "stream" or any(k.fmt != fmt for k in Ks):
            return None
        n = (ctypes.c_int64 * B)(*[int(k.n) for k in Ks])
        M = (ctypes.c_int64 * B)(*[int(k.M) for k in Ks])
        if fmt == "f32":
            nbytes = self.lib.odx_falkon_cg_batched_workspace_bytes(B, n, M)
        else:
            nbytes = self.lib.odx_falkon_cg_batched_q_workspace_bytes(B, n, M, hip.KNM_CODE[fmt])
        if nbytes < 0:
            return None
        base = Ps[0].LTi
        p_rows, ldp = Ps[0].block_rows, Ps[0].ld
        p_stride = 4 * p_rows * ldp
        for b, P in enumerate(Ps):
            if P.LTi.data_ptr() != base.data_ptr() + b * p_stride * 8 or P.ld != ldp:
                raise ValueError("cg_solve_batched: the preconditioners must be consecutive members of one precond_batched block")
        kp = (ctypes.c_void_p * B)(*[k.K.data_ptr() for k in Ks])
        kl = (ctypes.c_int64 * B)(*[int(k.ld) for k in Ks])
        nt = (ctypes.c_double * B)(*[float(x) for x in n_totals])
        alpha = torch.zeros_like(b0s)
        ws = self._workspace("cg_solve_batched", nbytes)
        if fmt != "f32":
            lp = (ctypes.c_void_p * B)(*[(k.lo.data_ptr() if k.lo is not None else 0) for k in Ks])
            hip.check(self.lib.odx_falkon_cg_batched_q_f64(B, kp, kl, lp, kl, hip.KNM_CODE[fmt], n, M, _p(base), ldp, p_rows, p_stride, _p(b0s),
                                                           b0s.stride(0), nt, float(lam), int(maxiter), int(opt.cg_full_gradient_every),
                                                           float(opt.cg_epsilon), float(opt.cg_tolerance), _p(alpha), _p(ws), ws.numel(),
                                                           self._stream()), "odx_falkon_cg_batched_q_f64")
            return alpha
        hip.check(self.lib.odx_falkon_cg_batched_f64(B, kp, kl, n, M, _p(base), ldp, p_rows, p_stride, _p(b0s), b0s.stride(0), nt,
                                                     float(lam), int(maxiter), int(opt.cg_full_gradient_every), float(opt.cg_epsilon),
                                                     float(opt.cg_tolerance), _p(alpha), _p(ws), ws.numel(), self._stream()),
                  "odx_falkon_cg_batched_f64")
        return alpha

    _TRI = {"LTi": 0, "LTit": 1, "LAi": 0, "LAit": 1}

    def trmv(self, P, name, x, alpha=1.0, beta=0.0, z=None, out=None):
        if out is None:
            out = torch.empty(P.M, dtype=torch.float64, device=self.device)
        hip.check(self.lib.odx_trmv_f64(_p(getattr(P, name)), P.ld, P.M, self._TRI[name], _p(x), float(alpha),
                                        float(beta), _p(z), _p(out), self._stream()), "odx_trmv_f64")
        return out

    def cg_init(self, B, X, R, Pv, state):
        hip.check(self.lib.odx_cg_init(_p(B), _p(X), _p(R), _p(Pv), _p(state), B.numel(), self._stream()), "odx_cg_init")

    def cg_step(self, X, R, Pv, AP, state, cg_eps, full_grad):
        hip.check(self.lib.odx_cg_step(_p(X), _p(R), _p(Pv), _p(AP), _p(state), float(cg_eps), int(bool(full_grad)),
                                       X.numel(), self._stream()), "odx_cg_step")

    def cg_finish(self, R, Pv, state, cg_eps, tol):
        hip.check(self.lib.odx_cg_finish(_p(R), _p(Pv), _p(state), float(cg_eps), float(tol), R.numel(),
                                         self._stream()), "odx_cg_finish")

    def axpby(self, a, x, b, y):
        hip.check(self.lib.odx_axpby_f64(float(a), _p(x), float(b), _p(y), y.numel(), self._stream()), "odx_axpby_f64")

    def mmv(self, F, Zf, sigma, V, ranges=None, out=None, max_range=None):
        V = V.to(device=self.device, dtype=torch.float64)
        if V.dim() == 1:
            V = V[:, None]
        Vs = V
        V = V.contiguous()
        Mtot, T = V.shape
        if Mtot != Zf.n:
            raise ValueError("mmv: V has %d rows but there are %d centres" % (Mtot, Zf.n))
        shared = ranges is None and self.gauss == "h2" and self.shared_mmv_min is not None and T >= self.shared_mmv_min
        if shared and F.n > 0 and T > 0 and Mtot > 0:
            if out is None:
                out = torch.empty((F.n, T), dtype=torch.float32, device=self.device)
            self.pack(F), self.pack(Zf)
            if Vs.stride(1) == 1 and Vs.stride(0) >= T:
                V = Vs
            ws = self._workspace("mmv", self.lib.odx_gauss_mmvn_h2_workspace_bytes(F.n, Mtot, T))
            hip.check(self.lib.odx_gauss_mmvn_h2(_p(F.P), F.P.stride(0), _p(F.meta), _p(F.sq), F.n, _p(Zf.P), Zf.P.stride(0),
                                                 _p(Zf.meta), _p(Zf.sq), Mtot, F.D, float(sigma), _p(V), V.stride(0), T,
                                                 _p(out), out.stride(0), _p(ws), ws.numel(), self._stream()), "odx_gauss_mmvn_h2")
            return out
        if ranges is None:
            key = ("dense_ranges", Mtot, T)
            ranges = self._ws.get(key)
            if ranges is None:
                ranges = self._ws[key] = torch.tensor([[0, Mtot]] * T, dtype=torch.int32, device=self.device)
        ranges = ranges.to(device=self.device, dtype=torch.int32).contiguous()
        if out is None:
            out = torch.empty((F.n, T), dtype=torch.float32, device=self.device)
        if F.n == 0 or T == 0:
            return out
        if Mtot == 0:
            return out.zero_()
        if self.gauss == "f8":
            self.pack8(F), self.pack8(Zf)
            mr = Mtot if max_range is None else max(1, min(int(max_range), Mtot))
            ws = self._workspace("mmv", self.lib.odx_gauss_mmv_h2_workspace_bytes(F.n, mr, T))
            hip.check(self.lib.odx_gauss_mmv_f8(_p(F.P8), F.P8.stride(0), _p(F.meta8), _p(F.sq8), F.n, _p(Zf.P8), Zf.P8.stride(0),
                                                _p(Zf.meta8), _p(Zf.sq8), mr, F.D, float(sigma), _p(V), V.stride(0), _p(ranges), T,
                                                _p(out), out.stride(0), _p(ws), ws.numel(), self._stream()), "odx_gauss_mmv_f8")
        elif self.gauss == "h2":
            self.pack(F), self.pack(Zf)
            mr = Mtot if max_range is None else max(1, min(int(max_range), Mtot))
            ws = self._workspace("mmv", self.lib.odx_gauss_mmv_h2_workspace_bytes(F.n, mr, T))
            hip.check(self.lib.odx_gauss_mmv_h2(_p(F.P), F.P.stride(0), _p(F.meta), _p(F.sq), F.n, _p(Zf.P), Zf.P.stride(0),
                                                _p(Zf.meta), _p(Zf.sq), mr, F.D, float(sigma), _p(V), V.stride(0), _p(ranges), T,
                                                _p(out), out.stride(0), _p(ws), ws.numel(), self._stream()), "odx_gauss_mmv_h2")
        else:
            hip.check(self.lib.odx_gauss_mmv_f32(_p(F.X), F.ld, _p(F.sq), F.n, _p(Zf.X), Zf.ld, _p(Zf.sq), F.D,
                                                 float(sigma), _p(V), V.stride(0), _p(ranges), T, _p(out), out.stride(0),
                                                 self._stream()), "odx_gauss_mmv_f32")
        return out

    def rls_gram(self, F, idx, Yt, G, XtY):
        nc = idx.numel()
        if nc == 0:
            return
        nbytes = self.lib.odx_rls_gram_workspace_bytes(nc, F.D)
        ws = self._workspace("rls_gram", nbytes)
        hip.check(self.lib.odx_rls_gram_f64(_p(F.X), F.ld, F.D, _p(idx), nc, _p(Yt), Yt.stride(0), _p(G), G.stride(0),
                                            _p(XtY), XtY.stride(0), _p(ws), ws.numel(), self._stream()),
                  "odx_rls_gram_f64")

    def rls_solve(self, G, D, lam, XtY):
        D1 = D + 1
# ... 595 lines not shown
```

online-detection_amd/odx/hip.py:

```python
import ctypes
import os

_LIB = None
_LIB_PATH = os.environ.get("ODX_LIB_PATH") or os.path.join(os.path.dirname(os.path.abspath(__file__)), "lib", "libodx.so")

ODX_OK = 0
KNM_F32, KNM_U24, KNM_BF16 = 0, 1, 2
KNM_CODE = {"f32": KNM_F32, "u24": KNM_U24, "bf16": KNM_BF16}
STREAM_MAX_VECTORS = 16
GEMM_LOWER_ONLY, GEMM_A_UPPER, GEMM_B_UPPER, GEMM_A_LOWER, GEMM_B_LOWER, GEMM_STORE_T = 1, 2, 4, 8, 16, 32


class OdxUnavailable(RuntimeError):
    pass


class OdxError(RuntimeError):
    pass


_vp, _i64, _i32, _f64, _f32 = ctypes.c_void_p, ctypes.c_int64, ctypes.c_int, ctypes.c_double, ctypes.c_float

SIGNATURES = {
    "odx_last_error_string": (ctypes.c_char_p, []),
# ... 9 lines not shown
    "odx_stream_destroy": (_i32, [_vp]),
    "odx_set_pass_cus": (_i32, [_i32]),
    "odx_set_side_stream_cu_mask": (_i32, [_vp, _i32]),
    "odx_debug_placement": (_i32, [_vp, _i32, _i32, _vp]),
    "odx_row_sqnorm_f32": (_i32, [_vp, _i64, _i64, _i32, _vp, _vp]),
    "odx_row_sqnorm_absmax_f32": (_i32, [_vp, _i64, _i64, _i32, _vp, _vp, _vp]),
    "odx_split_f16_premax": (_i32, [_vp, _i64, _i64, _i32, _vp, _i64, _vp, _vp]),
    "odx_gauss_knm_f32": (_i32, [_vp, _i64, _vp, _i64, _vp, _i64, _vp, _i64, _i32, _f64, _vp, _i64, _vp]),
    "odx_gauss_knm_direct_f32": (_i32, [_vp, _i64, _i64, _vp, _i64, _i64, _i32, _f64, _vp, _i64, _vp]),
    "odx_gauss_mmv_f32": (_i32, [_vp, _i64, _vp, _i64, _vp, _i64, _vp, _i32, _f64, _vp, _i64, _vp, _i32, _vp, _i64, _vp]),
    "odx_split_f16": (_i32, [_vp, _i64, _i64, _i32, _vp, _i64, _vp, _vp]),
    "odx_gauss_h2_tile": (_i32, [_i64, _i64]),
    "odx_set_h2_tile": (_i32, [_i32]),
    "odx_gauss_knm_h2": (_i32, [_vp, _i64, _vp, _vp, _i64, _vp, _i64, _vp, _vp, _i64, _i32, _f64, _vp, _i64, _vp]),
    "odx_gauss_knm_h2_rhs_workspace_bytes": (_i64, [_i64, _i64]),
    "odx_gauss_knm_h2_rhs": (_i32, [_vp, _i64, _vp, _vp, _i64, _vp, _i64, _vp, _vp, _i64, _i32, _f64, _vp, _i64, _vp, _vp, _vp, _i64,
                                    _vp]),
    "odx_gauss_mmv_h2_workspace_bytes": (_i64, [_i64, _i64, _i32]),
    "odx_gauss_mmv_h2": (_i32, [_vp, _i64, _vp, _vp, _i64, _vp, _i64, _vp, _vp, _i64, _i32, _f64, _vp, _i64, _vp, _i32, _vp, _i64,
                                _vp, _i64, _vp]),
    "odx_gauss_mmvn_h2_workspace_bytes": (_i64, [_i64, _i64, _i32]),
    "odx_gauss_mmvn_h2": (_i32, [_vp, _i64, _vp, _vp, _i64, _vp, _i64, _vp, _vp, _i64, _i32, _f64, _vp, _i64, _i32, _vp, _i64,
                                 _vp, _i64, _vp]),
    "odx_falkon_cg_workspace_bytes": (_i64, [_i64, _i64]),
    "odx_falkon_cg_f64": (_i32, [_vp, _i64, _i64, _i64, _vp, _vp, _vp, _vp, _i64, _vp, _f64, _f64, _i32, _i32, _f64, _f64, _vp, _vp,
                                 _i64, _vp]),
    "odx_falkon_cg_batched_workspace_bytes": (_i64, [_i32, _vp, _vp]),
    "odx_falkon_cg_batched_f64": (_i32, [_i32, _vp, _vp, _vp, _vp, _vp, _i64, _i64, _i64, _vp, _i64, _vp, _f64, _i32, _i32, _f64, _f64,
                                         _vp, _vp, _i64, _vp]),
    "odx_falkon_cg_batched_q_workspace_bytes": (_i64, [_i32, _vp, _vp, _i32]),
    "odx_falkon_cg_batched_q_f64": (_i32, [_i32, _vp, _vp, _vp, _vp, _i32, _vp, _vp, _vp, _i64, _i64, _i64, _vp, _i64, _vp, _f64, _i32, _i32,
                                           _f64, _f64, _vp, _vp, _i64, _vp]),
    "odx_knm_fwd_bwd_workspace_bytes": (_i64, [_i64, _i64]),
    "odx_set_pass_reserved_cus": (_i32, [_i32]),
    "odx_knm_fwd_bwd": (_i32, [_vp, _i64, _i64, _i64, _vp, _vp, _vp, _vp, _i64, _vp]),
    "odx_knm_fwd_bwd2_workspace_bytes": (_i64, [_i64, _i64]),
    "odx_knm_fwd_bwd2": (_i32, [_vp, _i64, _i64, _i64, _vp, _vp, _vp, _vp, _vp, _i64, _vp]),
    "odx_knm_ld": (_i64, [_i64, _i32]),
    "odx_knm_bytes": (_i64, [_i64, _i64, _i32]),
    "odx_gauss_knm_h2_store": (_i32, [_vp, _i64, _vp, _vp, _i64, _vp, _i64, _vp, _vp, _i64, _i32, _f64, _i32, _vp, _i64, _vp, _i64,
                                      _vp, _vp, _vp, _i64, _vp]),
    "odx_knm_fwd_bwd_t": (_i32, [_vp, _i64, _i64, _i64, _vp, _vp, _vp, _vp, _vp, _i64, _vp]),
    "odx_knm_fwd_bwd2_t": (_i32, [_vp, _i64, _i64, _i64, _vp, _vp, _vp, _vp, _vp, _vp, _i64, _vp]),
    "odx_knm_fwd_bwd_q_t": (_i32, [_vp, _i64, _vp, _i64, _i32, _i64, _i64, _vp, _vp, _vp, _vp, _vp, _i64, _vp]),
    "odx_knm_fwd_bwd2_q_t": (_i32, [_vp, _i64, _vp, _i64, _i32, _i64, _i64, _vp, _vp, _vp, _vp, _vp, _vp, _i64, _vp]),
    "odx_knm_fwd_bwd_q_cols_t": (_i32, [_vp, _i64, _vp, _i64, _i32, _i64, _i64, _vp, _vp, _vp, _vp, _vp, _i64, _i64, _vp, _vp, _vp, _vp]),
    "odx_knm_fwd_bwd2_q_cols_t": (_i32, [_vp, _i64, _vp, _i64, _i32, _i64, _i64, _vp, _vp, _vp, _vp, _vp, _vp, _i64, _i64, _vp, _vp, _vp,
                                         _vp]),
    "odx_cols_fold_f64": (_i32, [_vp, _i64, _vp, _vp, _i64, _vp, _vp]),
    "odx_cols_expand_f64": (_i32, [_vp, _i64, _vp, _i64, _vp, _vp]),
    "odx_cg_scores_axpy_f64": (_i32, [_vp, _vp, _vp, _i64, _vp]),
    "odx_cg_scores_store_f32": (_i32, [_vp, _i64, _vp, _i64, _vp]),
    "odx_knm_fwd_bwd_q_workspace_bytes": (_i64, [_i64, _i64, _i32]),
    "odx_knm_fwd_bwd_q": (_i32, [_vp, _i64, _vp, _i64, _i32, _i64, _i64, _vp, _vp, _vp, _vp, _i64, _vp]),
    "odx_knm_fwd_bwd2_q_workspace_bytes": (_i64, [_i64, _i64, _i32]),
    "odx_knm_fwd_bwd2_q": (_i32, [_vp, _i64, _vp, _i64, _i32, _i64, _i64, _vp, _vp, _vp, _vp, _vp, _i64, _vp]),
    "odx_knm_fwd_bwdn_q_workspace_bytes": (_i64, [_i64, _i64, _i32, _i32]),
    "odx_knm_fwd_bwdn_q": (_i32, [_vp, _i64, _vp, _i64, _i32, _i64, _i64, _i32, _vp, _i64, _vp, _i64, _vp, _i64, _vp]),
    "odx_knm_bwdn_q_workspace_bytes": (_i64, [_i64, _i64, _i32, _i32]),
    "odx_knm_bwdn_q": (_i32, [_vp, _i64, _vp, _i64, _i32, _i64, _i64, _i32, _vp, _i64, _vp, _i64, _vp, _i64, _vp]),
    "odx_knm_fwdn_q_workspace_bytes": (_i64, [_i64, _i64, _i32, _i32]),
    "odx_knm_fwdn_q": (_i32, [_vp, _i64, _vp, _i64, _i32, _i64, _i64, _i32, _vp, _i64, _vp, _i64, _vp, _i64, _vp]),
    "odx_knm_mv": (_i32, [_vp, _i64, _vp, _i64, _i32, _i64, _i64, _vp, _vp, _i64, _vp]),
    "odx_gauss_ktk_stream_h2_rows": (_i64, [_i64, _i32]),
    "odx_gauss_ktk_stream_h2_workspace_bytes": (_i64, [_i64, _i64, _i32]),
    "odx_gauss_ktk_stream_h2": (_i32, [_vp, _i64, _vp, _vp, _i64, _vp, _i64, _vp, _vp, _i64, _i32, _f64, _vp, _vp, _vp, _vp, _vp, _vp,
                                       _i64, _vp]),
    "odx_gauss_ktk_stream_h2n_rows": (_i64, [_i64, _i32]),
    "odx_gauss_ktk_stream_h2n_workspace_bytes": (_i64, [_i64, _i64, _i32, _i32]),
    "odx_gauss_ktk_stream_h2n": (_i32, [_vp, _i64, _vp, _vp, _i64, _vp, _i64, _vp, _vp, _i64, _i32, _f64, _i32, _vp, _i64, _vp, _i64,
                                        _vp, _i64, _vp]),
    "odx_split_f8": (_i32, [_vp, _i64, _i64, _i32, _vp, _i64, _vp, _vp, _vp]),
    "odx_gauss_knm_f8_store": (_i32, [_vp, _i64, _vp, _vp, _i64, _vp, _i64, _vp, _vp, _i64, _i32, _f64, _i32, _vp, _i64, _vp, _i64,
                                      _vp, _vp, _vp, _i64, _vp]),
    "odx_gauss_mmv_f8": (_i32, [_vp, _i64, _vp, _vp, _i64, _vp, _i64, _vp, _vp, _i64, _i32, _f64, _vp, _i64, _vp, _i32, _vp, _i64,
                                _vp, _i64, _vp]),
    "odx_cg_residual": (_i32, [_vp, _vp, _vp, _vp, _vp, _i64, _vp]),
    "odx_falkon_precond_workspace_bytes": (_i64, [_i64, _i32]),
    "odx_falkon_precond_f64": (_i32, [_vp, _i64, _i64, _i32, _f64, _f64, _f64, _vp, _vp, _vp, _vp, _i64, _vp, _vp, _i64, _vp]),
    "odx_falkon_precond_path_workspace_bytes": (_i64, [_i64, _i32, _i32]),
    "odx_falkon_precond_path_f64": (_i32, [_vp, _i64, _i64, _i32, _f64, _vp, _i32, _f64, _vp, _vp, _vp, _i64, _vp, _vp, _i64, _vp]),
    "odx_falkon_precond_batched_workspace_bytes": (_i64, [_i64, _i32, _i32]),
    "odx_falkon_precond_batched_f64": (_i32, [_vp, _vp, _vp, _i32, _i64, _i32, _f64, _f64, _f64, _vp, _i64, _i64, _vp, _vp, _i64, _vp]),
    "odx_trmv_f64": (_i32, [_vp, _i64, _i64, _i32, _vp, _f64, _f64, _vp, _vp, _vp]),
    "odx_trmvn_f64": (_i32, [_vp, _i64, _i64, _i32, _i32, _vp, _i64, _f64, _f64, _vp, _i64, _vp, _i64, _vp]),
    "odx_cg_init": (_i32, [_vp, _vp, _vp, _vp, _vp, _i64, _vp]),
    "odx_cg_step": (_i32, [_vp, _vp, _vp, _vp, _vp, _f64, _i32, _i64, _vp]),
    "odx_cg_finish": (_i32, [_vp, _vp, _vp, _f64, _f64, _i64, _vp]),
    "odx_axpby_f64": (_i32, [_f64, _vp, _f64, _vp, _i64, _vp]),
    "odx_gemm_nt_f64": (_i32, [_vp, _i64, _vp, _i64, _vp, _i64, _i64, _i64, _i64, _f64, _f64, _i32, _vp]),
    "odx_gemm_nt_f32": (_i32, [_vp, _i64, _vp, _i64, _vp, _i64, _i64, _i64, _i64, _f32, _f32, _i32, _vp]),
    "odx_potrf_workspace_bytes": (_i64, [_i64]),
    "odx_potrf_f64": (_i32, [_vp, _i64, _i64, _vp, _vp, _i64, _vp]),
    "odx_trtri_workspace_bytes": (_i64, [_i64]),
    "odx_trtri_f64": (_i32, [_vp, _i64, _i64, _vp, _vp, _i64, _vp, _i64, _vp]),
    "odx_convert_f32_f64": (_i32, [_vp, _i64, _vp, _i64, _i64, _i64, _vp]),
    "odx_convert_f64_f32": (_i32, [_vp, _i64, _vp, _i64, _i64, _i64, _vp]),
    "odx_rls_gram_workspace_bytes": (_i64, [_i64, _i32]),
    "odx_rls_gram_f64": (_i32, [_vp, _i64, _i32, _vp, _i64, _vp, _i64, _vp, _i64, _vp, _i64, _vp, _i64, _vp]),
    "odx_rls_solve_workspace_bytes": (_i64, [_i32]),
    "odx_rls_solve_f64": (_i32, [_vp, _i64, _i32, _f64, _vp, _i64, _vp, _i64, _vp, _vp, _i64, _vp]),
    "odx_rls_gram_batched_workspace_bytes": (_i64, [_i64, _i32]),
    "odx_rls_gram_batched_f64": (_i32, [_vp, _i64, _i32, _vp, _i64, _vp, _vp, _i32, _vp, _i64, _vp, _i64, _i64, _vp, _i64, _i64, _vp, _i64, _vp]),
    "odx_rls_pad_index": (_i32, [_vp, _i64, _vp, _vp, _i32, _i64, _vp, _vp, _vp, _vp, _vp, _vp]),
    "odx_rls_gram_raw_batched_f64": (_i32, [_vp, _i64, _i32, _vp, _i64, _vp, _vp, _i32, _vp, _i64, _vp, _i64, _i64, _vp, _i64, _vp]),
    "odx_rls_fold_whitened_f64": (_i32, [_vp, _i64, _i32, _i32, _vp, _vp, _vp, _i64, _i64, _vp, _i64, _i64, _vp]),
    "odx_rls_xty_batched_f64": (_i32, [_vp, _i64, _i32, _vp, _i64, _vp, _vp, _i32, _vp, _i64, _vp, _i64, _i64, _vp, _i64, _i64, _vp, _i64, _vp]),
    "odx_rls_rows_form": (_i32, [_vp, _i64, _i32]),
    "odx_rls_solve_batched_workspace_bytes": (_i64, [_i32, _i32]),
    "odx_rls_solve_batched_f64": (_i32, [_vp, _i64, _i64, _i32, _i32, _f64, _vp, _i64, _i64, _vp, _i64, _i64, _vp, _vp, _i64, _vp]),
    "odx_rls_predict_rows_f64": (_i32, [_vp, _i64, _i32, _vp, _i64, _vp, _i64, _vp, _i64, _vp]),
    "odx_rls_predict_rows_batched_f64": (_i32, [_vp, _i64, _i32, _vp, _vp, _i32, _i64, _vp, _i64, _i64, _vp, _i64, _vp]),
    "odx_roi_align_fwd_f32": (_i32, [_vp, _i32, _i32, _i32, _i32, _vp, _i32, _f32, _i32, _i32, _i32, _vp, _vp]),
    "odx_split_f16_taps3x3": (_i32, [_vp, _i64, _i64, _i32, _i32, _i32, _vp, _i64, _vp, _vp]),
    "odx_gemm_b16": (_i32, [_vp, _i64, _i64, _vp, _i64, _i64, _i32, _i32, _vp, _vp, _i64, _i32, _vp, _i64, _i32, _vp]),
    "odx_taps3x3_16": (_i32, [_vp, _i64, _i64, _i32, _i32, _i32, _vp, _i64, _vp]),
    "odx_gemm_h2_f32": (_i32, [_vp, _i64, _vp, _i64, _vp, _i64, _vp, _i64, _i32, _vp, _vp, _i64, _i32, _vp, _i64, _vp]),
    "odx_roi_align_rows_f32": (_i32, [_vp, _i32, _i32, _i32, _i32, _vp, _i32, _f32, _i32, _i32, _i32, _i32, _vp, _vp]),
    "odx_roi_align_rows_nhwc_f32": (_i32, [_vp, _i64, _i32, _i32, _i32, _i32, _vp, _i32, _f32, _i32, _i32, _i32, _i32, _vp, _vp]),
    "odx_gemm_h2_max_f32": (_i32, [_vp, _i64, _vp, _i64, _vp, _i64, _vp, _i64, _i32, _vp, _vp, _i64, _i32, _vp, _i64, _vp, _vp]),
    "odx_split_f16_taps3x3_premax": (_i32, [_vp, _i64, _i64, _i32, _i32, _i32, _vp, _i64, _vp, _vp]),
    "odx_gemm_h2_taps_supported": (_i32, [_i64, _i64, _i32, _i64]),
    "odx_gemm_h2_taps_f32": (_i32, [_vp, _i64, _vp, _i64, _i32, _i32, _i32, _vp, _i64, _vp, _i64, _vp, _vp, _i64, _i32, _vp, _i64, _vp,
                                    _vp, _i64, _f32, _f32, _vp, _vp]),
    "odx_gemm_h2_chain_f32": (_i32, [_vp, _i64, _vp, _i64, _vp, _i64, _vp, _i64, _i32, _vp, _vp, _i64, _i32, _vp, _i64, _vp,
                                     _vp, _i64, _f32, _f32, _vp, _vp]),
    "odx_taps3x3_packed": (_i32, [_vp, _i64, _i64, _i32, _i32, _i32, _vp, _i64, _vp]),
    "odx_rpn_label_f32": (_i32, [_vp, _i32, _vp, _vp, _i32, _i32, _f32, _f32, _vp, _vp, _vp, _vp, _vp, _vp, _vp, _vp]),
    "odx_det_label_f32": (_i32, [_vp, _vp, _i32, _vp, _i32, _i32, _f32, _f32, _f32, _f32, _vp, _i32, _vp, _vp, _vp, _vp, _vp, _vp]),
    "odx_box_targets_f32": (_i32, [_vp, _vp, _i64, _vp, _vp]),
    "odx_debug_gemm_h2_mf32": (_i32, [_vp, _i64, _vp, _i64, _vp, _i64, _vp, _i64, _i32, _vp, _i64, _vp]),
    "odx_gemm_b16_taps_supported": (_i32, [_i64, _i64, _i32, _i64]),
    "odx_gemm_b16_taps": (_i32, [_vp, _i64, _i64, _i32, _i32, _i32, _vp, _i64, _i64, _i32, _vp, _vp, _i64, _i32, _vp, _i64, _i32, _vp]),
    "odx_roi_align_fpn_f32": (_i32, [_vp, _vp, _vp, _vp, _i32, _i32, _i32, _vp, _i32, _i32, _i32, _i32, _vp, _vp, _vp]),
    "odx_roi_align_fpn_nhwc_f32": (_i32, [_vp, _vp, _vp, _vp, _i32, _i32, _i32, _vp, _i32, _i32, _i32, _i32, _vp, _vp, _vp]),
    "odx_stem_pool_rows_f32": (_i32, [_vp, _vp, _i32, _i32, _i32, _i32, _vp, _i64, _vp, _vp]),
    "odx_stem_pool_rows_16": (_i32, [_vp, _vp, _i32, _i32, _i32, _i32, _i32, _vp, _i64, _vp]),
    "odx_upsample_add_rows_f32": (_i32, [_vp, _i64, _vp, _i64, _i32, _i32, _i32, _i32, _i32, _i32, _vp, _vp]),
    "odx_upsample_add_rows_16": (_i32, [_vp, _i64, _vp, _i64, _i32, _i32, _i32, _i32, _i32, _i32, _i32, _vp]),
    "odx_roi_align_fpn_nhwc_16": (_i32, [_vp, _i32, _vp, _vp, _vp, _i32, _i32, _i32, _vp, _i32, _i32, _i32, _i32, _vp, _vp, _vp]),
    "odx_nms_workspace_bytes": (_i64, [_i32]),
    "odx_nms_f32": (_i32, [_vp, _i32, _f32, _vp, _vp, _i64, _vp]),
    "odx_nms_first_f32": (_i32, [_vp, _i32, _f32, _i32, _vp, _vp, _i64, _vp]),
    "odx_nms_batched_workspace_bytes": (_i64, [_i32, _i32]),
    "odx_nms_batched_f32": (_i32, [_vp, _vp, _i32, _i32, _f32, _vp, _vp, _i64, _vp]),
    "odx_rpn_topk_decode_f32": (_i32, [_vp, _vp, _vp, _i32, _i32, _i32, _i32, _i32, _f32, _f32, _f32, _vp, _vp, _vp, _vp]),
    "odx_nms_compact_f32": (_i32, [_vp, _vp, _vp, _i32, _i32, _i32, _vp, _vp, _vp]),
    "odx_nms_batched_first_f32": (_i32, [_vp, _vp, _i32, _i32, _f32, _i32, _vp, _vp, _i64, _vp]),
    "odx_paste_masks_u8": (_i32, [_vp, _vp, _i32, _i32, _i32, _i32, _f32, _i32, _vp, _vp]),
    "odx_bias_act_nchw_f32": (_i32, [_vp, _vp, _vp, _i64, _i32, _i64, _i32, _vp]),
    "odx_bias_act_nchw_16": (_i32, [_vp, _vp, _vp, _i32, _i64, _i32, _i64, _i32, _vp]),
}


def lib_path():
    return _LIB_PATH


def load():
    global _LIB
    if _LIB is not None:
        return _LIB
    if not os.path.exists(_LIB_PATH):
        raise OdxUnavailable(
            "libodx.so not found at %s — build it with `make -C online-detection_amd/csrc` "
            "(or __graft_entry__.build()); there is no CPU fallback." % _LIB_PATH)
    lib = ctypes.CDLL(_LIB_PATH)
    for name, (res, args) in SIGNATURES.items():
        fn = getattr(lib, name)
        fn.restype = res
        fn.argtypes = args
    _LIB = lib
    return lib


def check(rc, what=""):
    if rc != ODX_OK:
        msg = load().odx_last_error_string().decode("utf-8", "replace")
# ... 9 lines not shown
```

online-detection_amd/odx/job.py:

```python
import contextlib

import torch

from . import cols as _cols
from . import plan as _plan
from . import solver
from .dist import RowShard


class _Side:

    def __init__(self, device, be=None, cus=0, index=0):
        self.cuda = torch.device(device).type == "cuda"
        self.stream = None
        if self.cuda and cus > 0 and be is not None and hasattr(be, "masked_stream"):
            self.stream = be.masked_stream(cus)
        elif self.cuda:
            from . import streams as _streams
            own = _streams.distinct(index + 1, device)
            self.stream = own[index] if len(own) > index else torch.cuda.Stream(device=device)

    def after_current(self):
        if self.cuda:
            self.stream.wait_stream(torch.cuda.current_stream())

    def __enter__(self):
        self._ctx = torch.cuda.stream(self.stream) if self.cuda else contextlib.nullcontext()
        return self._ctx.__enter__()

    def __exit__(self, *exc):
        return self._ctx.__exit__(*exc)

    def mark(self):
        if not self.cuda:
            return None
        ev = torch.cuda.Event()
        ev.record(self.stream)
        return ev


def _wait(ev):
    if ev is not None:
        torch.cuda.current_stream().wait_event(ev)


class _OnStream:

    def __init__(self, stream, inner):
        self.stream, self.inner = stream, inner

    def __enter__(self):
        self.cur = torch.cuda.current_stream()
        self.stream.wait_stream(self.cur)
        self.ctx = torch.cuda.stream(self.stream)
        self.ctx.__enter__()
        return self.inner.__enter__()

    def __exit__(self, *exc):
        r = self.inner.__exit__(*exc)
        self.ctx.__exit__(*exc)
        self.cur.wait_stream(self.stream)
        return r


precond_groups = _plan.precond_groups


class LockstepClassJob:

    def __init__(self, be, X, n_total, M, labels, centre_idx, sigma, lam, maxiter=20, opt=None, shard=None,
                 precond_batch=0, precond_depth=2, precond_after_fit=False, classes=None, precond_cus=0, batch=0,
                 hbm_bytes=None, exchange="lockstep", gauss_on_complement=False, precond_lookahead=1, precond_cus_full_only=False,
                 score_from_knm=True, scores_from_cg=True, distinct_columns="auto"):
        if exchange not in ("lockstep", "allreduce"):
            raise ValueError("LockstepClassJob: exchange must be 'lockstep' or 'allreduce', got %r" % (exchange,))
        self.exchange = exchange
        self.score_from_knm = bool(score_from_knm)
        self.scores_from_cg = bool(scores_from_cg) and self.score_from_knm
        if distinct_columns not in ("auto", False, "force"):
            raise ValueError("LockstepClassJob: distinct_columns must be 'auto', False or 'force', got %r" % (distinct_columns,))
        self.distinct_columns = distinct_columns
        if exchange == "allreduce":
            batch = 1
        self.be, self.X, self.N, self.M = be, X, int(n_total), int(M)
        self.labels, self.cidx = labels, centre_idx
        self.sigma, self.lam, self.maxiter = sigma, lam, maxiter
        self.opt = opt or solver.SolverOptions(check_pivots=False)
        self.shard = shard if shard is not None else RowShard()
        self.world, self.rank = self.shard.world, self.shard.rank
        self.lo, self.hi = self.shard.bounds(self.N)
        self.n_loc = self.hi - self.lo
        dev = X.device
        self.C = len(centre_idx) if classes is None else int(classes)
        self.ldk = (self.M + 3) // 4 * 4
        D = int(X.shape[1]) if X.dim() == 2 else 0
        self.plan = _plan.plan_lockstep(
            self.N, D, self.M, self.C, self.world, batch=batch, chain=precond_batch,
            hbm_bytes=hbm_bytes if hbm_bytes is not None else (_plan.device_hbm_bytes(dev) if dev.type == "cuda" else _plan.HBM_BYTES_MI355X),
            knm_format=(be.knm_format if hasattr(be, "knm_format") else None),
            knm_bytes=(be.knm_bytes if hasattr(be, "knm_bytes") else None), gauss=getattr(be, "gauss", "h2"),
            lookahead=max(1, int(precond_lookahead)), chain_sides=2 if (precond_cus_full_only and precond_cus > 0) else 1)
        if not self.plan.feasible:
            raise MemoryError("LockstepClassJob: this job does not fit %d rank(s): %s" % (self.world, self.plan.summary()))
        self.b, self.G = self.plan.b, self.plan.g
        self.R = self.world // self.b
        kbytes = (be.knm_bytes(self.n_loc, self.M, D) if self.plan.knm_format == "stream" else be.knm_bytes(self.n_loc, self.M)) \
            if hasattr(be, "knm_bytes") else self.n_loc * self.ldk * 4
        self.kbufs = [torch.empty(max(kbytes, 16), dtype=torch.uint8, device=dev) for _ in range(self.b)]
        self.scores = torch.empty((self.n_loc, self.C), dtype=torch.float32, device=dev)
        self.sbuf = (torch.empty(self.n_loc, dtype=torch.float64, device=dev)
                     if self.scores_from_cg and (self.shard.world == 1 or exchange == "allreduce") and hasattr(be, "cg_scores_axpy")
                     else None)
        self.depth = precond_depth if precond_depth > 0 else 2
        self.after_fit = bool(precond_after_fit)
        self.ld_p = (self.M + 1) // 2 * 2
        self.nslot = self.depth + 1
        self.sides = [_Side(dev, be, precond_cus, index=k) for k in range(self.nslot)] if self.G == 1 else []
        self.lookahead = max(1, int(precond_lookahead))
        self.precond_cus, self.full_only = int(precond_cus), bool(precond_cus_full_only and precond_cus > 0)
        grouped = self.G > 1 or exchange == "allreduce"
        self.gside = _Side(dev, be, 0 if self.full_only else precond_cus) if grouped else None
        self.cside = _Side(dev, be, precond_cus, index=1) if (grouped and self.full_only) else None
        self._cplans = {}
        self._cmaps = {}
        self.gauss_stream = (be.masked_stream(precond_cus, complement=True)
                             if gauss_on_complement and precond_cus > 0 and dev.type == "cuda" and hasattr(be, "masked_stream") else None)
        self.pbuf, self.pgroup = [], []
        self.trace = []
        if self.world > 1 and not getattr(self.shard, "emulated", False):
            for idx in self.cidx[:self.C]:
                if torch.is_tensor(idx):
                    self._centre_plan(idx)
        if (distinct_columns and hasattr(be, "knm_format") and be.knm_format(self.n_loc, self.M) in ("u24", "bf16")
                and (distinct_columns == "force" or self.n_loc * self.M >= 2 ** 27)):
            for idx in self.cidx[:self.C]:
                if torch.is_tensor(idx):
                    cmap = _cols.column_map(idx)
                    if cmap is not None:
                        cmap.on(dev)
                        self._cmaps[self._idx_key(idx)] = cmap
        if self.G > 1 and hasattr(be, "precond_batched") and hasattr(be, "lib") and dev.type == "cuda":
            while len(self.pgroup) < self.lookahead + 1:
                self.pgroup.append(torch.empty((self.G, 4, self.M, self.ld_p), dtype=torch.float64, device=dev))
            for side in (self.gside, self.cside):
                if side is not None:
                    with side:
                        be._workspace("precond_group", be.lib.odx_falkon_precond_batched_workspace_bytes(self.M, D, self.G))

    def release(self):
        self.kbufs, self.pbuf, self.pgroup, self.scores, self.sbuf = [], [], [], None, None

    @staticmethod
    def _idx_key(idx):
        return (idx.data_ptr(), int(idx.numel()))

    def _with_map(self, Zf, idx):
        cmap = self._cmaps.get(self._idx_key(idx)) if self._cmaps else None
        if cmap is not None:
            Zf.cmap = cmap
        return Zf

    def _centre_plan(self, idx):
        key = (idx.data_ptr(), int(idx.numel()))
        plan = self._cplans.get(key)
        if plan is None:
            from .dist import shard_bounds
            ih = idx.detach().cpu().to(torch.int64)
            los = torch.tensor([shard_bounds(self.N, self.world, r)[0] for r in range(self.world)], dtype=torch.int64)
            owner = torch.bucketize(ih, los, right=True) - 1
            counts = torch.bincount(owner, minlength=self.world)
            cmax = max(int(counts.max()), 1)
            order = torch.argsort(owner, stable=True)
            starts = torch.cumsum(counts, 0) - counts
            within = torch.empty_like(ih)
            within[order] = torch.arange(ih.numel(), dtype=torch.int64) - starts[owner[order]]
            mine = ih[owner == self.rank] - self.lo
            dev = self.X.device
            plan = (mine.to(dev), cmax, (owner * cmax + within).to(dev), int(counts[self.rank]))
            self._cplans[key] = plan
        return plan

    def gather_centres(self, idx):
        be, X = self.be, self.X
        if self.world == 1:
            return self._with_map(be.features(X.index_select(0, idx)), idx)
        if getattr(self.shard, "emulated", False):
            Z = X.index_select(0, idx - self.lo)
            self.shard._count("centre_gather", Z)
            return self._with_map(be.features(Z), idx)
        mine, cmax, slot, n_mine = self._centre_plan(idx)
        blk = torch.zeros((cmax, X.shape[1]), dtype=X.dtype, device=X.device)
        if n_mine:
            torch.index_select(X, 0, mine, out=blk[:n_mine])
        allb = torch.empty((self.world, cmax, X.shape[1]), dtype=X.dtype, device=X.device)
        self.shard.gather_blocks(blk, allb)
        return self._with_map(be.features(allb.view(self.world * cmax, X.shape[1]).index_select(0, slot)), idx)

    def _score(self, ph, F, Z, K, alpha, c, summed=False):
        be = self.be
        if summed:
            be.knm_mv(K, alpha, out=self.scores[:, c:c + 1], summed=self.sbuf)
        elif (self.score_from_knm and K is not None and hasattr(be, "knm_mv") and getattr(be, "gauss", None) == "h2"
                and getattr(K, "fmt", None) in ("u24", "f32")):
            with ph("ktk"):
                be.knm_mv(K, alpha, out=self.scores[:, c:c + 1])
        else:
            with ph("mmv"):
                be.mmv(F, Z, self.sigma, alpha, None, out=self.scores[:, c:c + 1])

    def _prepare(self, batch, owners, slot, ph, infos):
        be, dev = self.be, self.X.device
        while len(self.pbuf) < self.nslot:
            self.pbuf.append(torch.empty((4, self.M, self.ld_p), dtype=torch.float64, device=dev))
        Zs = [self.gather_centres(self.cidx[c]) for c in batch]
        P, ev = None, None
        if self.rank in owners:
            pos = owners.index(self.rank)
            side = self.sides[slot]
            side.after_current()
            with side:
                with ph("precond"):
                    kw = {"out": self.pbuf[slot], "ws_key": "precond%d" % slot} if hasattr(be, "precond_batched") else {}
                    P = be.precond(Zs[pos], self.sigma, self.lam, self.opt.pc_epsilon, **kw)
                ev = side.mark()
            if infos is not None and hasattr(P, "info"):
                infos.append(P.info)
            self.trace.append(("precond", (batch[pos],)))
        return Zs, P, ev

    def _prepare_group(self, group, slot, ph, infos):
        be, dev = self.be, self.X.device
        Zs_all = [[self.gather_centres(self.cidx[c]) for c in batch] for batch, _ in group]
        own = [(k, owners.index(self.rank)) for k, (_, owners) in enumerate(group) if self.rank in owners]
        Ps, ev = {}, None
        if own:
            confined = self.cside is not None and len(own) >= self.G
            side = self.cside if confined else self.gside
            if self.precond_cus > 0 and hasattr(be, "set_helper_cus"):
                be.set_helper_cus(self.precond_cus if (confined or not self.full_only) else 0)
            side.after_current()
            with side:
                with ph("precond"):
                    zf = [Zs_all[k][pos] for k, pos in own]
                    if hasattr(be, "precond_batched"):
                        while len(self.pgroup) < self.lookahead + 1:
                            self.pgroup.append(torch.empty((self.G, 4, self.M, self.ld_p), dtype=torch.float64, device=dev))
                        plist = be.precond_batched(zf, self.sigma, self.lam, self.opt.pc_epsilon,
                                                   out=self.pgroup[slot][:len(own)], ws_key="precond_group")
                    else:
                        plist = [be.precond(z, self.sigma, self.lam, self.opt.pc_epsilon) for z in zf]
                ev = side.mark()
            Ps = dict(zip((k for k, _ in own), plist))
            if infos is not None:
                infos.extend(p.info for p in plist if hasattr(p, "info"))
            self.trace.append(("precond", tuple(group[k][0][pos] for k, pos in own)))
        return [(Zs_all[k], Ps.get(k), ev) for k in range(len(group))]

    def _run_replicated(self, F, classes, ph, phases, infos, alphas_out):
        be, dev = self.be, self.X.device
        groups = precond_groups(len(classes), max(self.G, 1))

        def prepare(gi):
            cls = [classes[k] for k in groups[gi]]
            Zs = [self.gather_centres(self.cidx[c]) for c in cls]
            self.gside.after_current()
            with self.gside:
                with ph("precond"):
                    if hasattr(be, "precond_batched") and len(cls) > 1:
                        g = max(self.G, len(cls))
                        while len(self.pgroup) < 2:
                            self.pgroup.append(torch.empty((g, 4, self.M, self.ld_p), dtype=torch.float64, device=dev))
                        plist = be.precond_batched(Zs, self.sigma, self.lam, self.opt.pc_epsilon,
                                                   out=self.pgroup[gi % 2][:len(cls)], ws_key="precond_group")
                    else:
                        plist = [be.precond(z, self.sigma, self.lam, self.opt.pc_epsilon) for z in Zs]
                ev = self.gside.mark()
            if infos is not None:
                infos.extend(p.info for p in plist if hasattr(p, "info"))
            self.trace.append(("precond", tuple(cls)))
            return {c: (z, p, ev) for c, z, p in zip(cls, Zs, plist)}

        ready = prepare(0) if groups else {}
        first_of = {grp[0]: gi for gi, grp in enumerate(groups)}
        out = None
        for k, c in enumerate(classes):
            gi = first_of.get(k)
            if gi is not None and gi + 1 < len(groups):
                ready.update(prepare(gi + 1))
            Z, P, ev = ready.pop(c)
            self.trace.append(("fit", (c,)))
            Ks = []
            alpha = solver.falkon_fit(be, F, self.labels(c), Z, self.sigma, self.lam, self.maxiter, self.opt, n_total=self.N,
                                      shard=self.shard, owner=None, knm_out=self.kbufs[0],
                                      phase=(lambda name: phases[name]) if phases is not None else None,
                                      precond=P, precond_ready=(lambda ev=ev: _wait(ev)), knm_blocks=Ks, scores_out=self.sbuf)
            self.trace.extend(("distinct", (c, K.M)) for K in Ks if getattr(K, "cmap", None) is not None)
            if alphas_out is not None:
                alphas_out[c] = alpha
            self._score(ph, F, Z, Ks[0] if Ks else None, alpha, c,
                        summed=self.sbuf is not None and bool(Ks) and solver.scores_from_cg(be, Ks[0]))
            out = (alpha, Z)
        if hasattr(be, "release_helper_streams"):
            be.release_helper_streams()
        return out

    def run(self, F, classes=None, phases=None, infos=None, alphas_out=None):
        be, world, rank = self.be, self.world, self.rank
        classes = list(range(self.C)) if classes is None else list(classes)
        base = (lambda name: phases[name]) if phases is not None else (lambda name: contextlib.nullcontext())
        if self.gauss_stream is not None:
            ph = lambda name: _OnStream(self.gauss_stream, base(name)) if name in ("knm", "mmv") else base(name)
        else:
            ph = base
        if self.exchange == "allreduce":
            return self._run_replicated(F, classes, ph, phases, infos, alphas_out)
        sched = _plan.lockstep_batches(classes, world, self.b)
        out = None
        if self.G > 1:
            n_rounds = (len(sched) + self.R - 1) // self.R
            groups = [[bi for r in grp for bi in range(r * self.R, min((r + 1) * self.R, len(sched)))]
                      for grp in precond_groups(n_rounds, self.G)]
            first_of = {grp[0]: gi for gi, grp in enumerate(groups)}
            L, nb = self.lookahead, self.lookahead + 1
            ready = {}
            for g0 in range(min(L, len(groups))):
                ready.update(zip(groups[g0], self._prepare_group([sched[bi] for bi in groups[g0]], g0 % nb, ph, infos)))
        else:
            ready = {bi: self._prepare(*sched[bi], bi % self.nslot, ph, infos) for bi in range(min(self.depth, len(sched)))}
        for bi, (batch, owners) in enumerate(sched):
            if self.G > 1:
                gi = first_of.get(bi)
                if gi is not None and gi + L < len(groups):
                    ready.update(zip(groups[gi + L], self._prepare_group([sched[k] for k in groups[gi + L]], (gi + L) % nb, ph, infos)))
            elif not self.after_fit and bi + self.depth < len(sched):
                ready[bi + self.depth] = self._prepare(*sched[bi + self.depth], (bi + self.depth) % self.nslot, ph, infos)
            Zs, P, ev = ready.pop(bi)
            ys = [self.labels(c) for c in batch]
            mine = rank in owners
            self.trace.append(("fit", tuple(batch)))
            Ks = []
            alphas = solver.falkon_fit_lockstep(be, F, ys, Zs, self.sigma, self.lam, self.maxiter, self.opt, n_total=self.N,
                                                shard=self.shard, knm_outs=self.kbufs[:len(batch)],
                                                phase=ph if (phases is not None or self.gauss_stream is not None) else None,
                                                precond=P if mine else None,
                                                precond_ready=(lambda: _wait(ev)) if mine else None, owners=owners, knm_blocks=Ks,
                                                scores_out=[self.sbuf] if (self.sbuf is not None and len(batch) == 1) else None)
            if self.G == 1 and self.after_fit and bi + self.depth < len(sched):
                ready[bi + self.depth] = self._prepare(*sched[bi + self.depth], (bi + self.depth) % self.nslot, ph, infos)
            self.trace.extend(("distinct", (c, K.M)) for c, K in zip(batch, Ks) if getattr(K, "cmap", None) is not None)
            if alphas_out is not None:
                alphas_out.update((c, alphas[pos]) for pos, c in enumerate(batch))
            summed = self.sbuf is not None and len(batch) == 1 and len(Ks) == 1 and solver.scores_from_cg(be, Ks[0])
            for pos, c in enumerate(batch):
                self._score(ph, F, Zs[pos], Ks[pos] if pos < len(Ks) else None, alphas[pos], c, summed=summed)
            out = (alphas[-1], Zs[-1])
        if hasattr(be, "release_helper_streams"):
# ... 3 lines not shown
```

online-detection_amd/odx/knm_path.py:

```python
import ctypes

import torch

from . import hip


def _p(t):
    return ctypes.c_void_p(t.data_ptr()) if t is not None else ctypes.c_void_p(0)


def _compact(K):
    return K.fmt in hip.KNM_CODE and K.fmt != "f32"


def _qblock(K):
    return _p(K.K), K.ld, _p(K.lo), K.ld, hip.KNM_CODE[K.fmt]


def _mapped(K):
    return getattr(K, "cmap", None)


def _vlen(K):
    return K.Mv if _mapped(K) is not None else K.M
# ... 146 lines not shown
                l += g
        while l < L:
            g = min(width, L - l)
            plan.append(("nv" if g >= 3 else "pair" if g == 2 and self.can_ktk2(K) else "single", l, g))
            l += g
        return plan

    def ktkn_reads(self, K, L):
        if K.fmt == "stream":
            return -(-L // self.ktkn_span(K))
        return sum({"nv": 1, "wide": 2, "pair": 1, "single": g}[kind] for kind, _, g in self._ktkn_plan(K, L))

    def _nv_call(self, entry, key, K, g, A, B):
        nbytes = self._pass_bytes(entry, max(K.n, 1), K.M, hip.KNM_CODE[K.fmt], g)
        ws = self._workspace(key, nbytes) if key else None
        self._call(entry, *_qblock(K), K.n, K.M, g, _p(A[0]), A.stride(0), _p(B[0]), B.stride(0), _p(ws), ws.numel() if key else 0)

    def kvn(self, K, V, out=None):
        if not _compact(K):
            raise ValueError("kvn: compact stored blocks only (u24 / bf16), got %r" % (K.fmt,))
        _no_map("kvn", K)
        L, M, n = V.shape[0], K.M, K.n
        if out is None:
            out = torch.zeros((L, (n + 1) // 2 * 2), dtype=torch.float64, device=self.device)
        _check_matrix("kvn", "V", V, L, M)
        _check_matrix("kvn", "out", out, L, n)
        _check_aligned("kvn", V=V, out=out)
        for l, g in _groups(L if n > 0 else 0, self.WIDE_PASS_MAX):
            self._nv_call("odx_knm_fwdn_q", None, K, g, V[l:], out[l:])
        return out

    def _ktkn_wide(self, K, V, out, l, g):
        ldt = (max(K.n, 1) + 1) // 2 * 2
        T = self._workspace("ktkn_t", g * ldt * 8)[:g * ldt * 8].view(torch.float64).view(g, ldt)
        self.kvn(K, V[l:l + g], out=T)
        self._nv_call("odx_knm_bwdn_q", "ktk", K, g, T, out[l:])

    def ktkn(self, K, V, out=None):
        _no_map("ktkn", K)
        L, M = V.shape[0], K.M
        if out is None:
            out = torch.zeros((L, (M + 1) // 2 * 2), dtype=torch.float64, device=self.device)
        _check_matrix("ktkn", "V", V, L, M)
        _check_matrix("ktkn", "out", out, L, M)
        if K.fmt == "stream":
            for l, g in _groups(L, self.ktkn_span(K)):
                if g == 1:
                    self.ktk(K, v=V[l, :M], out=out[l, :M])
                    continue
                _check_aligned("ktkn", V=V, out=out)
                self._ktkn_stream(K, V, out, l, g)
            return out
        for kind, l, g in self._ktkn_plan(K, L):
            if kind in ("nv", "wide"):
                _check_aligned("ktkn", V=V, out=out)
            if kind == "wide":
                self._ktkn_wide(K, V, out, l, g)
            elif kind == "nv":
                self._nv_call("odx_knm_fwd_bwdn_q", "ktk", K, g, V[l:], out[l:])
            elif kind == "pair":
                self.ktk2(K, V[l, :M], V[l + 1, :M], out1=out[l, :M], out2=out[l + 1, :M])
            else:
                for j in range(l, l + g):
                    self.ktk(K, v=V[j, :M], out=out[j, :M])
        return out

    def ktwn(self, K, W, out=None):
        _no_map("ktwn", K)
        T, M, n = W.shape[0], K.M, K.n
        if out is None:
            out = torch.zeros((T, (M + 1) // 2 * 2), dtype=torch.float64, device=self.device)
        _check_matrix("ktwn", "W", W, T, n)
        _check_matrix("ktwn", "out", out, T, M)
        for l, g in _groups(T, self.WIDE_PASS_MAX if _compact(K) else 1):
            if g == 1:
                self.ktk(K, w=W[l, :n], out=out[l, :M])
                continue
            _check_aligned("ktwn", W=W, out=out)
            self._nv_call("odx_knm_bwdn_q", "ktk", K, g, W[l:], out[l:])
        return out

    def trmvn(self, P, name, X, alpha=1.0, beta=0.0, Z=None, out=None):
        T, M = X.shape[0], P.M
        if out is None:
            out = torch.zeros((T, P.ld), dtype=torch.float64, device=self.device)
        for nm, t in (("X", X), ("out", out)) + (() if Z is None else (("Z", Z),)):
            _check_matrix("trmvn", nm, t, T, M)
        if beta != 0.0 and Z is None:
            raise ValueError("trmvn: beta needs Z")
        for l, g in _groups(T, 8):
            if g == 1:
                self.trmv(P, name, X[l], alpha=alpha, beta=beta, z=None if Z is None else Z[l], out=out[l])
                continue
            _check_aligned("trmvn", X=X)
            self._call("odx_trmvn_f64", _p(getattr(P, name)), P.ld, M, self._TRI[name], g, _p(X[l]), X.stride(0), float(alpha),
                       float(beta), _p(None if Z is None else Z[l]), 0 if Z is None else Z.stride(0), _p(out[l]), out.stride(0))
        return out

    def knm_mv(self, K, alpha, out=None, summed=None):
        if K.fmt not in hip.KNM_CODE:
            raise ValueError("knm_mv: needs a stored K_nM block, got %r (a streamed shard is scored by mmv)" % (K.fmt,))
        if summed is not None:
            if summed.numel() != K.n:
                raise ValueError("knm_mv: summed has %d entries but the block has %d rows" % (summed.numel(), K.n))
            if out is None:
                out = torch.empty((K.n, 1), dtype=torch.float32, device=self.device)
            return self.cg_scores_store(summed, out)
        alpha = alpha.to(device=self.device, dtype=torch.float64).contiguous()
        if alpha.numel() != _vlen(K):
            raise ValueError("knm_mv: alpha has %d entries but the block has %d columns" % (alpha.numel(), _vlen(K)))
        if _mapped(K) is not None:
            _, start, pos = _cols(K, self.device)[1:]
            folded = torch.empty(K.M, dtype=torch.float64, device=self.device)
            self._call("odx_cols_fold_f64", _p(alpha), K.Mv, start, pos, K.M, _p(folded))
            alpha = folded
        if out is None:
            out = torch.empty((K.n, 1), dtype=torch.float32, device=self.device)
        if out.dtype != torch.float32 or out.shape[0] != K.n or (out.dim() == 2 and out.shape[1] != 1):
            raise ValueError("knm_mv: out must be an (n,) or (n, 1) f32 tensor")
        self._call("odx_knm_mv", *_qblock(K), K.n, K.M, _p(alpha), _p(out), out.stride(0))
        return out

    def precond_path(self, Zf, sigma, lams, eps, out=None, ws_key="precond"):
        from .backend import Precond
        lams = [float(x) for x in lams]
        L, M, D = len(lams), Zf.n, Zf.D
        if not 1 <= L <= self.MAX_CLASS_BATCH:
            raise ValueError("precond_path: 1..%d lambdas per call, got %d" % (self.MAX_CLASS_BATCH, L))
        ld = (M + 1) // 2 * 2
        shape = (2 + 2 * L, M, ld)
        mats = out if out is not None else torch.empty(shape, dtype=torch.float64, device=self.device)
        if mats.dtype != torch.float64 or tuple(mats.shape) != shape or not mats.is_contiguous():
            raise ValueError("precond_path: out must be a contiguous %r f64 tensor" % (shape,))
        info = torch.zeros(L, dtype=torch.int32, device=self.device)
        ws = self._workspace(ws_key, self.lib.odx_falkon_precond_path_workspace_bytes(M, D, L))
        hip.check(self.lib.odx_falkon_precond_path_f64(_p(Zf.X), Zf.ld, M, D, float(sigma), (ctypes.c_double * L)(*lams), L, float(eps),
                                                       _p(mats[0]), _p(mats[1]), _p(mats[2]), ld, _p(info), _p(ws), ws.numel(),
                                                       self._stream()), "odx_falkon_precond_path_f64")
        members = []
        for l in range(L):
            P = Precond()
            P.M, P.ld = M, ld
            P.LTi, P.LTit, P.LAi, P.LAit = mats[0], mats[1], mats[2 + 2 * l], mats[3 + 2 * l]
            P.block_rows = None
            P.info = info[l:l + 1]
            members.append(P)
        return members
```

online-detection_amd/odx/solver.py:

```python
import math
from dataclasses import dataclass

import torch


@dataclass
class SolverOptions:
    pc_epsilon: float = 1e-5
    cg_epsilon: float = 1e-7
    cg_tolerance: float = 1e-7
    cg_full_gradient_every: int = 10
    check_pivots: bool = True


_DEFERRED = None


class deferred_pivot_checks:

    def __enter__(self):
        global _DEFERRED
        self._prev, self.items = _DEFERRED, []
        _DEFERRED = self.items
        return self
# ... 111 lines not shown
    def W1(*pairs, rows=False):
        k = len(pairs)
        for j, (s, _) in enumerate(pairs):
            for c in cgs:
                be.trmv(c.P, "LAit", getattr(c, s), out=c.v[j])
                be.trmv(c.P, "LTit", c.v[j], out=c.io[k - 1][j][0])
        exchange(k, rows)
        for j, (_, out) in enumerate(pairs):
            for c in cgs:
                u = be.trmv(c.P, "LTi", c.io[k - 1][j][1], alpha=1.0 / n, beta=c.lam, z=c.v[j])
                be.trmv(c.P, "LAi", u, out=getattr(c, out))

    W = W1 if sh is None else Wn
    tol = opt.cg_tolerance ** 2
    for it in range(maxiter):
        full = (it + 1) % opt.cg_full_gradient_every == 0
        fold = can_fold and full and it != maxiter - 1
        if fold:
            W(("Pv", "AP"), ("X", "AX"), rows=acc)
        else:
            W(("Pv", "AP"), rows=acc)
        for c in cgs:
            be.cg_step(c.X, c.R, c.Pv, c.AP, c.state, opt.cg_epsilon, full)
        for c in cgs:
            if c.scores is not None:
                be.cg_scores_axpy(c.state, c.tk, c.scores)
        if it == maxiter - 1:
            break
        if fold:
            for c in cgs:
                be.cg_residual(c.B, c.AX, c.AP, c.state, c.R)
        elif full:
            W(("X", "AP"))
            for c in cgs:
                c.R.copy_(c.B)
                be.axpby(-1.0, c.AP, 1.0, c.R)
        for c in cgs:
            be.cg_finish(c.R, c.Pv, c.state, opt.cg_epsilon, tol)
    if sh is not None:
        be.trmvn(P, "LTit", be.trmvn(P, "LAit", sh.X, out=sh.U), out=sh.alpha)
        for l, c in enumerate(cgs):
            c.alpha = sh.alpha[l, :P.M]
    else:
        for c in cgs:
            c.alpha = be.trmv(c.P, "LTit", be.trmv(c.P, "LAit", c.X), out=c.alpha)
    if opt.check_pivots:
        for c in (cgs[:1] if sh is not None else cgs):
            _check_pivots(be, c.P)


def falkon_fit(be, F, y, Zf, sigma, lam, maxiter=20, opt=None, n_total=None, allreduce=None, knm_out=None,
               return_knm=False, phase=None, precond=None, shard=None, owner=None, precond_ready=None, knm_blocks=None,
               scores_out=None):
    opt = opt or SolverOptions()
    n = float(F.n if n_total is None else n_total)
    M = Zf.n
    if shard is not None and allreduce is None:
        allreduce = shard.allreduce
    ar = allreduce if allreduce is not None else (lambda v: v)
    ph = phase if phase is not None else (lambda name: _NoPhase())
    owned = shard is None or owner is None or shard.rank == owner
    bcast = (lambda v: shard.broadcast(v, src=owner)) if (shard is not None and owner is not None) else (lambda v: v)

    P = precond
    if owned and P is None:
        with ph("precond"):
            P = be.precond(Zf, sigma, lam, opt.pc_epsilon)
    yn = y * (1.0 / n)
    with ph("knm"):
        K, b0 = be.knm_rhs(F, Zf, sigma, yn, out=knm_out)
    if knm_blocks is not None:
        knm_blocks.append(K)
    acc = scores_out is not None and (shard is None or owner is None) and scores_from_cg(be, K)
    tk = None
    if acc:
        scores_out.zero_()
        tk = torch.empty_like(scores_out)
    if shard is not None:
        can_fold = _can_fold(be, K, M, int(n) // shard.world)
    else:
        can_fold = allreduce is None and _can_fold(be, K, M, int(n))

    b0 = ar(b0)
    one_call = shard is None and allreduce is None and phase is None and hasattr(be, "cg_solve") and not acc
    if one_call and getattr(K, "fmt", "f32") != "f32":
        one_call = bool(hasattr(be, "cg_batched_supported") and getattr(P, "block_rows", None) is not None
                        and getattr(K, "cmap", None) is None
                        and be.cg_batched_supported([K.n], [K.M], K.fmt))
    if one_call:
        if precond_ready is not None:
            precond_ready()
            precond_ready = None
        if K.fmt != "f32":
            b0s = be.zeros((M + 1) // 2 * 2).view(1, -1)
            b0s[0, :M].copy_(b0)
            got = be.cg_solve_batched([K], [P], b0s, [n], lam, maxiter, opt)
            alpha = None if got is None else got[0, :M].clone()
        else:
            alpha = be.cg_solve(K, P, b0, n, lam, maxiter, opt)
    if one_call and alpha is not None:
        if opt.check_pivots:
            _check_pivots(be, P)
        return (alpha, K) if return_knm else alpha

    k, Mp = 2 if can_fold else 1, (M + 1) // 2 * 2
    TT, CC = be.zeros(k * Mp).view(k, Mp), be.zeros(k * Mp).view(k, Mp)

    def exchange(k, rows):
        bcast(TT if k == 2 else TT[0, :M])
        _pass(be, ph, K, TT[:k], CC[:k], M, tk if rows else None)
        _sum(ar, CC if k == 2 else CC[0, :M])

    alpha = be.zeros(M)
    cgs = []
    if owned:
        if precond_ready is not None:
            precond_ready()
        cgs.append(_cg_state(be, P, lam, b0, M, _slots(TT, CC, M), can_fold, alpha, tk, scores_out if acc else None))
    _cg_run(be, cgs, exchange, n, maxiter, opt, can_fold)
    bcast(alpha)
    return (alpha, K) if return_knm else alpha


def falkon_fit_path(be, F, y, Zf, sigma, lams, maxiter=20, opt=None, n_total=None, allreduce=None, phase=None, knm_out=None,
                    knm_blocks=None):
    opt = opt or SolverOptions()
    lams = [float(x) for x in lams]
    if not lams or any(not (math.isfinite(x) and x > 0.0) for x in lams):
        raise ValueError("falkon_fit_path: lams must be a non-empty sequence of finite positive penalties, got %r" % (lams,))
    L = len(lams)
    n = float(F.n if n_total is None else n_total)
    M = Zf.n
    ar = allreduce if allreduce is not None else (lambda v: v)
    ph = phase if phase is not None else (lambda name: _NoPhase())

    with ph("precond"):
        if hasattr(be, "precond_path"):
            Ps = be.precond_path(Zf, sigma, lams, opt.pc_epsilon)
        else:
            Ps = [be.precond(Zf, sigma, lam, opt.pc_epsilon) for lam in lams]
    with ph("knm"):
        K, b0 = be.knm_rhs(F, Zf, sigma, y * (1.0 / n), out=knm_out)
    if knm_blocks is not None:
        knm_blocks.append(K)
    b0 = ar(b0)

    return _fit_members(be, K, [(P, lam, b0) for P, lam in zip(Ps, lams)], M, n, maxiter, opt, ar, ph)


def _fit_members(be, K, members, M, n, maxiter, opt, ar, ph, B0=None):
    L = len(members)
    Mp = (M + 1) // 2 * 2
    can_fold = bool(getattr(K, "fmt", None) == "stream" and hasattr(be, "ktkn") and hasattr(be, "ktkn_span")
                    and hasattr(be, "cg_residual") and 2 * L <= be.ktkn_span(K))
    rows = 2 * L if can_fold else L
    TT = be.zeros(rows * Mp).view(rows, Mp)
    CC = be.zeros(rows * Mp).view(rows, Mp)

    def exchange(k, rows):
        TTr, CCr = TT[:k * L], CC[:k * L]
        with ph("ktkn"):
            if hasattr(be, "ktkn"):
                be.ktkn(K, TTr, out=CCr)
            else:
                for l in range(k * L):
                    be.ktk(K, v=TTr[l, :M], out=CCr[l, :M])
        _sum(ar, CCr)
# ... 128 lines not shown
```

Before: 186,000.

## Stop T-inverse recursion early and apply blocked triangular solves in CG

After: 190,900, median of 6. 2.6% higher.

```diff
diff --git a/include/odx.h b/include/odx.h
--- a/include/odx.h
+++ b/include/odx.h
@@ -169,9 +169,18 @@
                                    int64_t Mmax, int D, double sigma, double lam, double eps,
                                    double* out, int64_t ld, int64_t out_stride, int32_t* info,
                                    void* workspace, int64_t workspace_bytes, odx_stream_t stream);
+int odx_falkon_precond_batched_partial_f64(const float* const* Z, const int64_t* ldz, const int64_t* M, int B,
+                                           int64_t Mmax, int D, double sigma, double lam, double eps, int64_t t_stop,
+                                           double* out, int64_t ld, int64_t out_stride, int32_t* info,
+                                           void* workspace, int64_t workspace_bytes, odx_stream_t stream);
 
 int odx_trmv_f64(const double* Tri, int64_t ld, int64_t M, int uplo, const double* x,
                  double alpha, double beta, const double* z, double* y, odx_stream_t stream);
+
+int64_t odx_tri_blocked_mv_workspace_bytes(int64_t M);
+int odx_tri_blocked_mv_f64(const double* Tri, int64_t ld, int64_t M, int uplo, const int64_t* bounds, int nblocks,
+                           const double* x, double alpha, double beta, const double* z, double* y,
+                           void* workspace, int64_t workspace_bytes, odx_stream_t stream);
 
 int odx_trmvn_f64(const double* Tri, int64_t ld, int64_t M, int uplo, int nv, const double* X, int64_t ldx,
                   double alpha, double beta, const double* Z, int64_t ldz, double* Y, int64_t ldy, odx_stream_t stream);
@@ -224,6 +233,8 @@
 int64_t odx_trtri_workspace_bytes(int64_t M);
 int odx_trtri_f64(const double* L, int64_t ldl, int64_t M, double* Li, double* Lit, int64_t ld,
                   void* workspace, int64_t workspace_bytes, odx_stream_t stream);
+int odx_trtri_partial_f64(const double* L, int64_t ldl, int64_t M, int64_t stop, double* Li, double* Lit, int64_t ld,
+                          void* workspace, int64_t workspace_bytes, odx_stream_t stream);
 int odx_convert_f32_f64(const float* src, int64_t lds, double* dst, int64_t ldd, int64_t rows,
                         int64_t cols, odx_stream_t stream);
 int odx_convert_f64_f32(const double* src, int64_t lds, float* dst, int64_t ldd, int64_t rows,
diff --git a/online-detection_amd/csrc/api.cpp b/online-detection_amd/csrc/api.cpp
--- a/online-detection_amd/csrc/api.cpp
+++ b/online-detection_amd/csrc/api.cpp
@@ -20,10 +20,11 @@
   const char* name;
   int def, lo, hi;
 };
+constexpr int T_INVERSE_UNMERGED_DEFAULT = 2;
 static const OptSpec g_opt_spec[OPT_COUNT] = {
     {"h2_tile", 0, 0, 256}, {"precond", 0, 0, 2}, {"chain_helpers", -1, -1, 1}, {"rls_force_nt_gram", 0, 0, 1},
-    {"rls_force_inverse_solve", 0, 0, 1}};
-static int g_opt[OPT_COUNT] = {0, 0, -1, 0, 0};
+    {"rls_force_inverse_solve", 0, 0, 1}, {"t_inverse_unmerged", T_INVERSE_UNMERGED_DEFAULT, 0, 2}, {"t_inverse_force_stop", 0, 0, 1 << 20}};
+static int g_opt[OPT_COUNT] = {0, 0, -1, 0, 0, T_INVERSE_UNMERGED_DEFAULT, 0};
 int lib_option(int which) { return g_opt[which]; }
 static int opt_index(const char* name) {
   if (name)
diff --git a/online-detection_amd/csrc/dense_f64.hip b/online-detection_amd/csrc/dense_f64.hip
--- a/online-detection_amd/csrc/dense_f64.hip
+++ b/online-detection_amd/csrc/dense_f64.hip
@@ -404,15 +404,34 @@
   }
 }
 
-__device__ __forceinline__ void trmv_row(const double* __restrict__ Tri, int64_t ld, int64_t M, int uplo,
-                                         const double* __restrict__ x, double alpha, double beta,
-                                         const double* __restrict__ z, double* __restrict__ y) {
-  const int lane = threadIdx.x & 63;
-  int64_t i = (int64_t)blockIdx.x * 4 + (threadIdx.x >> 6);
-  if (i >= M) return;
-  if (!uplo) i = M - 1 - i;
-  const int64_t jlo = uplo ? i : 0, jhi = uplo ? M : i + 1;
-  const double* row = Tri + i * ld;
+__global__ __launch_bounds__(256) void place_factor_blocks_kernel(const double* __restrict__ L, int64_t ldl, int64_t M,
+                                                                  int64_t stop, double* __restrict__ Li,
+                                                                  double* __restrict__ Lit, int64_t ld, int64_t zstrideA,
+                                                                  int64_t zstrideO) {
+  __shared__ double tile[32][33];
+  const int64_t r0 = stop + (int64_t)blockIdx.y * 32, c0 = (int64_t)blockIdx.x * 32;
+  if (c0 >= r0 / stop * stop) return;
+  L += (int64_t)blockIdx.z * zstrideA;
+  Li += (int64_t)blockIdx.z * zstrideO;
+  Lit += (int64_t)blockIdx.z * zstrideO;
+  const int tx = threadIdx.x & 31, ty = threadIdx.x >> 5;
+#pragma unroll
+  for (int q = 0; q < 4; ++q) {
+    const int64_t r = r0 + ty + q * 8, c = c0 + tx;
+    const double v = r < M ? L[r * ldl + c] : 0.0;
+    tile[ty + q * 8][tx] = v;
+    if (r < M) Li[r * ld + c] = v;
+  }
+  __syncthreads();
+#pragma unroll
+  for (int q = 0; q < 4; ++q) {
+    const int64_t r = c0 + ty + q * 8, c = r0 + tx;
+    if (c < M) Lit[r * ld + c] = tile[tx][ty + q * 8];
+  }
+}
+
+__device__ __forceinline__ double row_dot(const double* __restrict__ row, const double* __restrict__ x, int64_t jlo, int64_t jhi,
+                                          int lane) {
   const int64_t q0 = (jlo + 1) >> 1, q1 = jhi >> 1;
   double s0 = 0.0, s1 = 0.0, s2 = 0.0, s3 = 0.0;
   if (lane == 0) {
@@ -438,10 +457,22 @@
   double s = (s0 + s1) + (s2 + s3);
 #pragma unroll
   for (int off = 32; off > 0; off >>= 1) s += __shfl_xor(s, off);
+  return s;
+}
+
+__device__ __forceinline__ void trmv_row(const double* __restrict__ Tri, int64_t ld, int64_t M, int uplo,
+                                         const double* __restrict__ x, double alpha, double beta,
+                                         const double* __restrict__ z, double* __restrict__ y, double* __restrict__ yraw = nullptr) {
+  const int lane = threadIdx.x & 63;
+  int64_t i = (int64_t)blockIdx.x * 4 + (threadIdx.x >> 6);
+  if (i >= M) return;
+  if (!uplo) i = M - 1 - i;
+  const double s = row_dot(Tri + i * ld, x, uplo ? i : 0, uplo ? M : i + 1, lane);
   if (lane == 0) {
     double r = alpha * s;
     if (beta != 0.0) r += beta * z[i];
     y[i] = r;
+    if (yraw) yraw[i] = s;
   }
 }
 
@@ -450,6 +481,23 @@
                                                        double beta, const double* __restrict__ z,
                                                        double* __restrict__ y) {
   trmv_row(Tri, ld, M, uplo, x, alpha, beta, z, y);
+}
+
+__global__ __launch_bounds__(256) void trmv_block_f64_kernel(const double* __restrict__ Tri, int64_t ld, int64_t M,
+                                                             int uplo, const double* __restrict__ x, double alpha,
+                                                             double beta, const double* __restrict__ z,
+                                                             double* __restrict__ y, double* __restrict__ yraw) {
+  trmv_row(Tri, ld, M, uplo, x, alpha, beta, z, y, yraw);
+}
+
+__global__ __launch_bounds__(256) void rect_dot_f64_kernel(const double* __restrict__ A, int64_t ld, int64_t r0, int64_t r1,
+                                                           int64_t c0, int64_t c1, const double* __restrict__ t,
+                                                           const double* __restrict__ x, double* __restrict__ u) {
+  const int lane = threadIdx.x & 63;
+  const int64_t i = r0 + (int64_t)blockIdx.x * 4 + (threadIdx.x >> 6);
+  if (i >= r1) return;
+  const double s = row_dot(A + i * ld, t, c0, c1, lane);
+  if (lane == 0) u[i] = x[i] - s;
 }
 
 template <int NV>
@@ -793,9 +841,11 @@
 
 int trtri_from_diag_f64(const double* L, int64_t ldl, int64_t M, const double* Dinv, double* Li, double* Lit,
                         int64_t ld, double* WT, hipStream_t stream, const ZBatch& zb, uint32_t* pk, int64_t pk_cap, int64_t pk_z,
-                        double bound_l, double bound_inv) {
+                        double bound_l, double bound_inv, int64_t stop) {
   constexpr int NB = POTRF_NB;
   ODX_REQUIRE(ld % 2 == 0 && ldl % 2 == 0, "trtri_f64: leading dimensions must be even");
+  ODX_REQUIRE(stop == 0 || (stop >= NB && stop % NB == 0 && (stop / NB & (stop / NB - 1)) == 0),
+              "trtri_f64: the stop level must be %d 2^k", NB);
   const int Z = zb.count;
   ODX_REQUIRE(Z >= 1 && Z <= ODX_MAX_ZBATCH && zb.strideA % 2 == 0 && zb.strideO % 2 == 0 && zb.strideW % 2 == 0,
               "trtri_f64: class batch of 1..%d matrices, even strides", ODX_MAX_ZBATCH);
@@ -804,6 +854,12 @@
                      Li, Lit, ld, zb.strideD, zb.strideO);
   ODX_CHECK_LAUNCH("place_diag_inverses");
   for (int64_t s = NB; s < M; s *= 2) {
+    if (stop > 0 && s >= stop) {
+      hipLaunchKernelGGL(place_factor_blocks_kernel, dim3((unsigned)ceil_div(M, 32), (unsigned)ceil_div(M - stop, 32), (unsigned)Z),
+                         dim3(256), 0, stream, L, ldl, M, stop, Li, Lit, ld, zb.strideA, zb.strideO);
+      ODX_CHECK_LAUNCH("place_factor_blocks");
+      break;
+    }
     const int nb = (int)ceil_div(M, 2 * s);
     const int nbe = (int)ceil_div(M - s, 2 * s);
     const int64_t m2l = M - s - (int64_t)(nbe - 1) * 2 * s;
@@ -964,13 +1020,13 @@
   return odx_potrf_workspace_bytes(M) + M * M * (int64_t)sizeof(double);
 }
 
-extern "C" int odx_trtri_f64(const double* L, int64_t ldl, int64_t M, double* Li, double* Lit, int64_t ld,
-                             void* workspace, int64_t workspace_bytes, odx_stream_t stream) {
+static int trtri_f64_impl(const char* who, const double* L, int64_t ldl, int64_t M, int64_t stop, double* Li, double* Lit,
+                          int64_t ld, void* workspace, int64_t workspace_bytes, odx_stream_t stream) {
   if (M <= 0) return ODX_OK;
-  ODX_REQUIRE(L && Li && Lit && workspace, "odx_trtri_f64: null pointer");
-  ODX_REQUIRE(ld >= M && ldl >= M && aligned16(L) && aligned16(Li) && aligned16(Lit), "odx_trtri_f64: bad ld / alignment");
+  ODX_REQUIRE(L && Li && Lit && workspace, "%s: null pointer", who);
+  ODX_REQUIRE(ld >= M && ldl >= M && aligned16(L) && aligned16(Li) && aligned16(Lit), "%s: bad ld / alignment", who);
   if (workspace_bytes < odx_trtri_workspace_bytes(M)) {
-    set_error("odx_trtri_f64: workspace too small");
+    set_error("%s: workspace too small", who);
     return ODX_ERR_WORKSPACE;
   }
   hipStream_t s = as_stream(stream);
@@ -981,7 +1037,54 @@
   ODX_CHECK_LAUNCH("trtri_diag");
   ODX_PROPAGATE(fill_f64(Li, ld, M, M, 0.0, s));
   ODX_PROPAGATE(fill_f64(Lit, ld, M, M, 0.0, s));
-  return trtri_from_diag_f64(L, ldl, M, Dinv, Li, Lit, ld, WT, s);
+  return trtri_from_diag_f64(L, ldl, M, Dinv, Li, Lit, ld, WT, s, ZBatch(), nullptr, 0, 0, 1.0, 1.0, stop);
+}
+
+extern "C" int odx_trtri_f64(const double* L, int64_t ldl, int64_t M, double* Li, double* Lit, int64_t ld,
+                             void* workspace, int64_t workspace_bytes, odx_stream_t stream) {
+  return trtri_f64_impl("odx_trtri_f64", L, ldl, M, 0, Li, Lit, ld, workspace, workspace_bytes, stream);
+}
+
+extern "C" int odx_trtri_partial_f64(const double* L, int64_t ldl, int64_t M, int64_t stop, double* Li, double* Lit, int64_t ld,
+                                     void* workspace, int64_t workspace_bytes, odx_stream_t stream) {
+  return trtri_f64_impl("odx_trtri_partial_f64", L, ldl, M, stop, Li, Lit, ld, workspace, workspace_bytes, stream);
+}
+
+extern "C" int64_t odx_tri_blocked_mv_workspace_bytes(int64_t M) {
+  return M <= 0 ? 0 : 2 * round_up(M, 2) * (int64_t)sizeof(double);
+}
+
+extern "C" int odx_tri_blocked_mv_f64(const double* Tri, int64_t ld, int64_t M, int uplo, const int64_t* bounds, int nblocks,
+                                      const double* x, double alpha, double beta, const double* z, double* y, void* workspace,
+                                      int64_t workspace_bytes, odx_stream_t stream) {
+  if (M <= 0) return ODX_OK;
+  ODX_REQUIRE(Tri && x && y && bounds && workspace && (beta == 0.0 || z), "odx_tri_blocked_mv_f64: null pointer");
+  ODX_REQUIRE(ld % 2 == 0 && ld >= M && aligned16(Tri) && aligned16(x) && aligned16(workspace),
+              "odx_tri_blocked_mv_f64: Tri/x/workspace must be 16-byte aligned, ld even, ld >= M");
+  ODX_REQUIRE(x != y, "odx_tri_blocked_mv_f64: x and y must not alias");
+  ODX_REQUIRE(nblocks >= 1 && bounds[0] == 0 && bounds[nblocks] == M, "odx_tri_blocked_mv_f64: bounds must run from 0 to M");
+  for (int b = 0; b < nblocks; ++b)
+    ODX_REQUIRE(bounds[b] < bounds[b + 1] && bounds[b] % 2 == 0, "odx_tri_blocked_mv_f64: bounds must ascend, interior ones even");
+  if (workspace_bytes < odx_tri_blocked_mv_workspace_bytes(M)) {
+    set_error("odx_tri_blocked_mv_f64: workspace too small");
+    return ODX_ERR_WORKSPACE;
+  }
+  hipStream_t s = as_stream(stream);
+  double* t = static_cast<double*>(workspace);
+  double* u = t + round_up(M, 2);
+  for (int k = 0; k < nblocks; ++k) {
+    const int b = uplo ? nblocks - 1 - k : k;
+    const int64_t r0 = bounds[b], r1 = bounds[b + 1];
+    if (k > 0) {
+      hipLaunchKernelGGL(rect_dot_f64_kernel, dim3((unsigned)ceil_div(r1 - r0, 4)), dim3(256), 0, s, Tri, ld, r0, r1,
+                         uplo ? r1 : (int64_t)0, uplo ? M : r0, t, x, u);
+      ODX_CHECK_LAUNCH("odx_tri_blocked_mv_f64 (rect)");
+    }
+    hipLaunchKernelGGL(trmv_block_f64_kernel, dim3((unsigned)ceil_div(r1 - r0, 4)), dim3(256), 0, s, Tri + r0 * (ld + 1), ld,
+                       r1 - r0, uplo, (k > 0 ? u : x) + r0, alpha, beta, z ? z + r0 : nullptr, y + r0, t + r0);
+    ODX_CHECK_LAUNCH("odx_tri_blocked_mv_f64 (block)");
+  }
+  return ODX_OK;
 }
 
 static int64_t precond_ld(int64_t M) { return round_up(M, 2); }
@@ -1117,7 +1220,7 @@
 }
 
 static int falkon_precond_batched_f64_impl(const float* const* Z, const int64_t* ldz, const int64_t* M, int B,
-                                           int64_t Mmax, int D, double sigma, double lam, double eps, double* out,
+                                           int64_t Mmax, int D, double sigma, double lam, double eps, int64_t t_stop, double* out,
                                            int64_t ld, int64_t out_stride, int32_t* info, void* workspace,
                                            int64_t workspace_bytes, odx_stream_t stream);
 
@@ -1125,12 +1228,20 @@
                                               int64_t Mmax, int D, double sigma, double lam, double eps, double* out,
                                               int64_t ld, int64_t out_stride, int32_t* info, void* workspace,
                                               int64_t workspace_bytes, odx_stream_t stream) {
-  const int rc = falkon_precond_batched_f64_impl(Z, ldz, M, B, Mmax, D, sigma, lam, eps, out, ld, out_stride, info, workspace, workspace_bytes, stream);
+  const int rc = falkon_precond_batched_f64_impl(Z, ldz, M, B, Mmax, D, sigma, lam, eps, 0, out, ld, out_stride, info, workspace, workspace_bytes, stream);
   return rc;
 }
 
+extern "C" int odx_falkon_precond_batched_partial_f64(const float* const* Z, const int64_t* ldz, const int64_t* M, int B,
+                                                      int64_t Mmax, int D, double sigma, double lam, double eps, int64_t t_stop,
+                                                      double* out, int64_t ld, int64_t out_stride, int32_t* info, void* workspace,
+                                                      int64_t workspace_bytes, odx_stream_t stream) {
+  ODX_REQUIRE(t_stop >= 0, "odx_falkon_precond_batched_partial_f64: negative stop level");
+  return falkon_precond_batched_f64_impl(Z, ldz, M, B, Mmax, D, sigma, lam, eps, t_stop, out, ld, out_stride, info, workspace, workspace_bytes, stream);
+}
+
 static int falkon_precond_batched_f64_impl(const float* const* Z, const int64_t* ldz, const int64_t* M, int B,
-                                           int64_t Mmax, int D, double sigma, double lam, double eps, double* out,
+                                           int64_t Mmax, int D, double sigma, double lam, double eps, int64_t t_stop, double* out,
                                            int64_t ld, int64_t out_stride, int32_t* info, void* workspace,
                                            int64_t workspace_bytes, odx_stream_t stream) {
   ODX_REQUIRE(B >= 1 && B <= ODX_MAX_ZBATCH, "odx_falkon_precond_batched_f64: 1 <= B <= %d classes per call", ODX_MAX_ZBATCH);
@@ -1189,7 +1300,7 @@
   ODX_PROPAGATE(potrf_f64(W0, wld, Mmax, DinvT, info, s, zt));
   ODX_CHECK_HIP(hipEventRecord(side->fork, s));
   ODX_CHECK_HIP(hipStreamWaitEvent(s2, side->fork, 0));
-  ODX_PROPAGATE(trtri_from_diag_f64(W0, wld, Mmax, DinvT, LTi, LTit, ld, W3, s2, zt));
+  ODX_PROPAGATE(trtri_from_diag_f64(W0, wld, Mmax, DinvT, LTi, LTit, ld, W3, s2, zt, nullptr, 0, 0, 1.0, 1.0, t_stop));
   ODX_CHECK_HIP(hipEventRecord(side->join, s2));
   ODX_PROPAGATE(transpose_f64(W0, wld, W1, wld, Mmax, Mmax, s, B, wsz, wsz));
   if (split) {
diff --git a/online-detection_amd/csrc/odx_internal.h b/online-detection_amd/csrc/odx_internal.h
--- a/online-detection_amd/csrc/odx_internal.h
+++ b/online-detection_amd/csrc/odx_internal.h
@@ -8,6 +8,8 @@
   OPT_CHAIN_HELPERS,
   OPT_RLS_FORCE_NT_GRAM,
   OPT_RLS_FORCE_INVERSE_SOLVE,
+  OPT_T_INVERSE_UNMERGED,
+  OPT_T_INVERSE_FORCE_STOP,
   OPT_COUNT
 };
 int lib_option(int which);
@@ -54,7 +56,7 @@
               float pk_scale = 1.f);
 int trtri_from_diag_f64(const double* L, int64_t ldl, int64_t M, const double* Dinv, double* Li, double* Lit,
                         int64_t ld, double* WT, hipStream_t stream, const ZBatch& zb = ZBatch(), uint32_t* pk = nullptr,
-                        int64_t pk_cap = 0, int64_t pk_z = 0, double bound_l = 1.0, double bound_inv = 1.0);
+                        int64_t pk_cap = 0, int64_t pk_z = 0, double bound_l = 1.0, double bound_inv = 1.0, int64_t stop = 0);
 int transpose_f64(const double* src, int64_t lds, double* dst, int64_t ldd, int64_t rows, int64_t cols,
                   hipStream_t stream, int zcount = 1, int64_t zstride_src = 0, int64_t zstride_dst = 0);
 int add_diag_f64(double* A, int64_t lda, int64_t M, double value, hipStream_t stream, int zcount = 1, int64_t zstride = 0);
diff --git a/online-detection_amd/odx/backend.py b/online-detection_amd/odx/backend.py
--- a/online-detection_amd/odx/backend.py
+++ b/online-detection_amd/odx/backend.py
@@ -39,7 +39,15 @@
 
 
 class Precond:
-    __slots__ = ("LTi", "LTit", "LAi", "LAit", "M", "ld", "info", "block_rows")
+    __slots__ = ("LTi", "LTit", "LAi", "LAit", "M", "ld", "info", "block_rows", "blocks")
+
+    def __init__(self):
+        self.blocks = ()
+
+
+def require_merged(P, who):
+    if getattr(P, "blocks", ()):
+        raise ValueError("%s: this preconditioner holds a partial inverse of T (blocks %r); only trmv multiplies by it" % (who, P.blocks))
 
 
 class Knm:
@@ -274,7 +282,7 @@
 
     MAX_CLASS_BATCH = 32
 
-    def precond_batched(self, Zfs, sigma, lam, eps, out=None, ws_key="precond_batched", Mmax=None):
+    def precond_batched(self, Zfs, sigma, lam, eps, out=None, ws_key="precond_batched", Mmax=None, t_stop=0):
         B = len(Zfs)
         if not 1 <= B <= self.MAX_CLASS_BATCH:
             raise ValueError("precond_batched: 1..%d classes per call, got %d" % (self.MAX_CLASS_BATCH, B))
@@ -295,9 +303,15 @@
         zp = (ctypes.c_void_p * B)(*[z.X.data_ptr() for z in Zfs])
         zl = (ctypes.c_int64 * B)(*[int(z.ld) for z in Zfs])
         zm = (ctypes.c_int64 * B)(*Ms)
-        hip.check(self.lib.odx_falkon_precond_batched_f64(zp, zl, zm, B, Mmax, D, float(sigma), float(lam), float(eps), _p(out), ld,
-                                                          4 * Mmax * ld, _p(info), _p(ws), ws.numel(), self._stream()),
-                  "odx_falkon_precond_batched_f64")
+        t_stop = int(t_stop) if int(t_stop) < Mmax else 0
+        if t_stop:
+            hip.check(self.lib.odx_falkon_precond_batched_partial_f64(zp, zl, zm, B, Mmax, D, float(sigma), float(lam), float(eps), t_stop,
+                                                                      _p(out), ld, 4 * Mmax * ld, _p(info), _p(ws), ws.numel(),
+                                                                      self._stream()), "odx_falkon_precond_batched_partial_f64")
+        else:
+            hip.check(self.lib.odx_falkon_precond_batched_f64(zp, zl, zm, B, Mmax, D, float(sigma), float(lam), float(eps), _p(out), ld,
+                                                              4 * Mmax * ld, _p(info), _p(ws), ws.numel(), self._stream()),
+                      "odx_falkon_precond_batched_f64")
         Ps = []
         for b, M in enumerate(Ms):
             P = Precond()
@@ -305,6 +319,8 @@
             P.LTi, P.LTit, P.LAi, P.LAit = (out[b, k, :M] for k in range(4))
             P.info = info[b:b + 1]
             P.block_rows = Mmax
+            if t_stop and M > t_stop:
+                P.blocks = tuple(range(0, M, t_stop)) + (M,)
             Ps.append(P)
         return Ps
 
@@ -458,6 +474,7 @@
         return out
 
     def cg_solve(self, K, P, b0, n_total, lam, maxiter, opt):
+        require_merged(P, "cg_solve")
         if K.fmt != "f32":
             raise hip.OdxError("cg_solve: the one-call CG loop needs an f32-stored K_nM block, got %r" % K.fmt)
         alpha = torch.empty(K.M, dtype=torch.float64, device=self.device)
@@ -483,6 +500,8 @@
 
     def cg_solve_batched(self, Ks, Ps, b0s, n_totals, lam, maxiter, opt):
         B = len(Ks)
+        for P in Ps:
+            require_merged(P, "cg_solve_batched")
         fmt = Ks[0].fmt
         if fmt == "stream" or any(k.fmt != fmt for k in Ks):
             return None
@@ -519,10 +538,20 @@
         return alpha
 
     _TRI = {"LTi": 0, "LTit": 1, "LAi": 0, "LAit": 1}
+    _bounds = {}
 
     def trmv(self, P, name, x, alpha=1.0, beta=0.0, z=None, out=None):
         if out is None:
             out = torch.empty(P.M, dtype=torch.float64, device=self.device)
+        if P.blocks and name in ("LTi", "LTit"):
+            bounds = self._bounds.get(P.blocks)
+            if bounds is None:
+                bounds = self._bounds[P.blocks] = (ctypes.c_int64 * len(P.blocks))(*P.blocks)
+            ws = self._workspace("tri_blocked_mv", self.lib.odx_tri_blocked_mv_workspace_bytes(P.M))
+            hip.check(self.lib.odx_tri_blocked_mv_f64(_p(getattr(P, name)), P.ld, P.M, self._TRI[name], bounds, len(P.blocks) - 1,
+                                                      _p(x), float(alpha), float(beta), _p(z), _p(out), _p(ws), ws.numel(),
+                                                      self._stream()), "odx_tri_blocked_mv_f64")
+            return out
         hip.check(self.lib.odx_trmv_f64(_p(getattr(P, name)), P.ld, P.M, self._TRI[name], _p(x), float(alpha),
                                         float(beta), _p(z), _p(out), self._stream()), "odx_trmv_f64")
         return out
diff --git a/online-detection_amd/odx/hip.py b/online-detection_amd/odx/hip.py
--- a/online-detection_amd/odx/hip.py
+++ b/online-detection_amd/odx/hip.py
@@ -115,6 +115,9 @@
     "odx_falkon_precond_path_f64": (_i32, [_vp, _i64, _i64, _i32, _f64, _vp, _i32, _f64, _vp, _vp, _vp, _i64, _vp, _vp, _i64, _vp]),
     "odx_falkon_precond_batched_workspace_bytes": (_i64, [_i64, _i32, _i32]),
     "odx_falkon_precond_batched_f64": (_i32, [_vp, _vp, _vp, _i32, _i64, _i32, _f64, _f64, _f64, _vp, _i64, _i64, _vp, _vp, _i64, _vp]),
+    "odx_falkon_precond_batched_partial_f64": (_i32, [_vp, _vp, _vp, _i32, _i64, _i32, _f64, _f64, _f64, _i64, _vp, _i64, _i64, _vp, _vp, _i64, _vp]),
+    "odx_tri_blocked_mv_workspace_bytes": (_i64, [_i64]),
+    "odx_tri_blocked_mv_f64": (_i32, [_vp, _i64, _i64, _i32, _vp, _i32, _vp, _f64, _f64, _vp, _vp, _vp, _i64, _vp]),
     "odx_trmv_f64": (_i32, [_vp, _i64, _i64, _i32, _vp, _f64, _f64, _vp, _vp, _vp]),
     "odx_trmvn_f64": (_i32, [_vp, _i64, _i64, _i32, _i32, _vp, _i64, _f64, _f64, _vp, _i64, _vp, _i64, _vp]),
     "odx_cg_init": (_i32, [_vp, _vp, _vp, _vp, _vp, _i64, _vp]),
@@ -127,6 +130,7 @@
     "odx_potrf_f64": (_i32, [_vp, _i64, _i64, _vp, _vp, _i64, _vp]),
     "odx_trtri_workspace_bytes": (_i64, [_i64]),
     "odx_trtri_f64": (_i32, [_vp, _i64, _i64, _vp, _vp, _i64, _vp, _i64, _vp]),
+    "odx_trtri_partial_f64": (_i32, [_vp, _i64, _i64, _i64, _vp, _vp, _i64, _vp, _i64, _vp]),
     "odx_convert_f32_f64": (_i32, [_vp, _i64, _vp, _i64, _i64, _i64, _vp]),
     "odx_convert_f64_f32": (_i32, [_vp, _i64, _vp, _i64, _i64, _i64, _vp]),
     "odx_rls_gram_workspace_bytes": (_i64, [_i64, _i32]),
diff --git a/online-detection_amd/odx/job.py b/online-detection_amd/odx/job.py
--- a/online-detection_amd/odx/job.py
+++ b/online-detection_amd/odx/job.py
@@ -37,6 +37,18 @@
         ev = torch.cuda.Event()
         ev.record(self.stream)
         return ev
+
+
+def t_inverse_stop(M, unmerged, force=0):
+    M, unmerged, force = int(M), int(unmerged), int(force)
+    if force > 0:
+        return force if M > force else 0
+    if unmerged <= 0 or M <= 8192:
+        return 0
+    top = 128
+    while 2 * top < M:
+        top *= 2
+    return max(top >> (unmerged - 1), 4096)
 
 
 def _wait(ev):
@@ -147,6 +159,19 @@
                     with side:
                         be._workspace("precond_group", be.lib.odx_falkon_precond_batched_workspace_bytes(self.M, D, self.G))
 
+    def _t_stop(self):
+        lib = getattr(self.be, "lib", None)
+        if lib is None or not hasattr(lib, "odx_get_option"):
+            return 0
+        import ctypes
+        got = {}
+        for name in ("t_inverse_unmerged", "t_inverse_force_stop"):
+            v = ctypes.c_int(0)
+            if lib.odx_get_option(name.encode(), ctypes.byref(v)) != 0:
+                raise RuntimeError("odx_get_option(%s) failed" % name)
+            got[name] = v.value
+        return t_inverse_stop(self.M, got["t_inverse_unmerged"], got["t_inverse_force_stop"])
+
     def release(self):
         self.kbufs, self.pbuf, self.pgroup, self.scores, self.sbuf = [], [], [], None, None
 
@@ -246,7 +271,7 @@
                         while len(self.pgroup) < self.lookahead + 1:
                             self.pgroup.append(torch.empty((self.G, 4, self.M, self.ld_p), dtype=torch.float64, device=dev))
                         plist = be.precond_batched(zf, self.sigma, self.lam, self.opt.pc_epsilon,
-                                                   out=self.pgroup[slot][:len(own)], ws_key="precond_group")
+                                                   out=self.pgroup[slot][:len(own)], ws_key="precond_group", t_stop=self._t_stop())
                     else:
                         plist = [be.precond(z, self.sigma, self.lam, self.opt.pc_epsilon) for z in zf]
                 ev = side.mark()
@@ -271,7 +296,7 @@
                         while len(self.pgroup) < 2:
                             self.pgroup.append(torch.empty((g, 4, self.M, self.ld_p), dtype=torch.float64, device=dev))
                         plist = be.precond_batched(Zs, self.sigma, self.lam, self.opt.pc_epsilon,
-                                                   out=self.pgroup[gi % 2][:len(cls)], ws_key="precond_group")
+                                                   out=self.pgroup[gi % 2][:len(cls)], ws_key="precond_group", t_stop=self._t_stop())
                     else:
                         plist = [be.precond(z, self.sigma, self.lam, self.opt.pc_epsilon) for z in Zs]
                 ev = self.gside.mark()
diff --git a/online-detection_amd/odx/knm_path.py b/online-detection_amd/odx/knm_path.py
--- a/online-detection_amd/odx/knm_path.py
+++ b/online-detection_amd/odx/knm_path.py
@@ -252,6 +252,8 @@
 
     def trmvn(self, P, name, X, alpha=1.0, beta=0.0, Z=None, out=None):
         T, M = X.shape[0], P.M
+        from .backend import require_merged
+        require_merged(P, "trmvn")
         if out is None:
             out = torch.zeros((T, P.ld), dtype=torch.float64, device=self.device)
         for nm, t in (("X", X), ("out", out)) + (() if Z is None else (("Z", Z),)):
diff --git a/online-detection_amd/odx/solver.py b/online-detection_amd/odx/solver.py
--- a/online-detection_amd/odx/solver.py
+++ b/online-detection_amd/odx/solver.py
@@ -217,7 +217,8 @@
         can_fold = allreduce is None and _can_fold(be, K, M, int(n))
 
     b0 = ar(b0)
-    one_call = shard is None and allreduce is None and phase is None and hasattr(be, "cg_solve") and not acc
+    one_call = (shard is None and allreduce is None and phase is None and hasattr(be, "cg_solve") and not acc
+                and not getattr(P, "blocks", ()))
     if one_call and getattr(K, "fmt", "f32") != "f32":
         one_call = bool(hasattr(be, "cg_batched_supported") and getattr(P, "block_rows", None) is not None
                         and getattr(K, "cmap", None) is None
```
